# rcedgar/muscle

Measured on AMD Instinct MI355X. Metric: sequence-pairs/sec (fwd+bwd+posterior+relax), higher is better.
Workload: dtype f32

## Files before the change

### include/mpcgpu.h

```cpp
#ifndef MPCGPU_H
#define MPCGPU_H

#include <stdint.h>

#ifdef __cplusplus
extern "C" {
#endif

typedef struct mpcgpu_ctx mpcgpu_ctx;

int mpcgpu_create(mpcgpu_ctx **out, int device_ordinal);
void mpcgpu_destroy(mpcgpu_ctx *ctx);
const char *mpcgpu_last_error(const mpcgpu_ctx *ctx);
const char *mpcgpu_version(void);

int mpcgpu_set_hmm(mpcgpu_ctx *ctx, const float start[5], const float trans[25],
                   const float match[256 * 256], const float ins[256],
                   float min_sparse_score, int expf_variant);

int mpcgpu_set_seqs(mpcgpu_ctx *ctx, uint32_t n, const uint8_t *const *seqs, const uint32_t *lens);

int mpcgpu_set_mega(mpcgpu_ctx *ctx, uint32_t nfeat, const uint32_t *alpha, const float *weight,
                    const float *const *logprobs, const float *const *logprob_mx,
                    const uint8_t *const *profiles);
// ... 10 lines not shown
int mpcgpu_plan_store_segments(uint32_t n, const uint32_t *sizes, uint64_t limit_blocks, uint32_t max_segs, uint32_t *z_first,
                               uint64_t *blocks, uint32_t *nsegs);

int mpcgpu_calc_posteriors(mpcgpu_ctx *ctx, uint64_t k0, uint64_t k1);

int mpcgpu_build_store(mpcgpu_ctx *ctx);

int mpcgpu_shard_info(mpcgpu_ctx *ctx, uint64_t *bytes, void **dev_ptr);
int mpcgpu_shard_entries(mpcgpu_ctx *ctx, uint64_t *entries);
int mpcgpu_shard_export(mpcgpu_ctx *ctx, void *dev_dst);
int mpcgpu_store_import(mpcgpu_ctx *ctx, uint32_t nshards, const uint64_t *k0, const uint64_t *k1,
                        const uint64_t *bytes, void *dev_all);
int mpcgpu_store_import_part(mpcgpu_ctx *ctx, uint32_t nshards, const uint64_t *k0, const uint64_t *k1, const uint64_t *bytes,
                             const uint64_t *offsets, void *dev_all, uint64_t own_k0, uint64_t own_k1);
int mpcgpu_store_complete(mpcgpu_ctx *ctx);
int mpcgpu_values_info(mpcgpu_ctx *ctx, void **dev_ptr, uint64_t *total_count);
int mpcgpu_values_slice(mpcgpu_ctx *ctx, uint64_t k0, uint64_t k1, uint64_t *first, uint64_t *count);
int mpcgpu_values_export(mpcgpu_ctx *ctx, uint64_t first, uint64_t count, void *dev_dst);
int mpcgpu_values_import(mpcgpu_ctx *ctx, uint64_t first, uint64_t count, const void *dev_src);

int mpcgpu_cons_iter(mpcgpu_ctx *ctx, uint64_t k0, uint64_t k1);
int mpcgpu_cons_commit(mpcgpu_ctx *ctx);
int mpcgpu_cons_commit_range(mpcgpu_ctx *ctx, uint64_t first, uint64_t count);

int mpcgpu_get_ea(mpcgpu_ctx *ctx, uint64_t k0, uint64_t k1, float *ea);
int mpcgpu_get_nnz(mpcgpu_ctx *ctx, uint64_t k0, uint64_t k1, uint32_t *nnz);
int mpcgpu_get_sparse(mpcgpu_ctx *ctx, uint64_t k, uint32_t *offsets, void *values);
int mpcgpu_get_sparse_range(mpcgpu_ctx *ctx, uint64_t k0, uint64_t k1, uint32_t *offsets, void *values);

int mpcgpu_post_scores(mpcgpu_ctx *ctx, uint32_t LX, uint32_t LY, uint32_t ncand, const uint32_t *rows,
                       const uint32_t *cols, const float *scores, int kernel, uint32_t batch, float *ea, uint32_t *nnz,
                       uint32_t *offsets, void *values);

int mpcgpu_calc_aln(mpcgpu_ctx *ctx, const float *post, uint32_t LX, uint32_t LY,
                    char *path, uint32_t *pathlen, float *score);

int mpcgpu_align_alns(mpcgpu_ctx *ctx, uint32_t n1, const uint32_t *seq1, uint32_t n2, const uint32_t *seq2,
                      uint32_t C1, uint32_t C2, const uint32_t *pos2col1, const uint32_t *pos2col2,
                      char *path, uint32_t *pathlen, float *score);
int mpcgpu_align_alns_w(mpcgpu_ctx *ctx, uint32_t n1, const uint32_t *seq1, uint32_t n2, const uint32_t *seq2,
                        uint32_t C1, uint32_t C2, const uint32_t *pos2col1, const uint32_t *pos2col2,
                        const float *w1, const float *w2, char *path, uint32_t *pathlen, float *score);

int mpcgpu_align_alns_batch(mpcgpu_ctx *ctx, uint32_t njoins, const uint32_t *n1, const uint32_t *n2, const uint32_t *C1,
                            const uint32_t *C2, const uint32_t *seqs, const uint32_t *pos2col, uint32_t path_stride,
                            char *paths, uint32_t *pathlens, float *scores);

int mpcgpu_build_post(mpcgpu_ctx *ctx, uint32_t n1, const uint32_t *seq1, uint32_t n2, const uint32_t *seq2, uint32_t C1,
                      uint32_t C2, const uint32_t *pos2col1, const uint32_t *pos2col2, const float *w1, const float *w2,
                      float *post);
int mpcgpu_get_last_post(mpcgpu_ctx *ctx, uint32_t C1, uint32_t C2, float *post);

int mpcgpu_set_seqs_registry(mpcgpu_ctx *ctx, uint32_t n, const uint8_t *const *seqs, const uint32_t *lens);
int mpcgpu_align_msas(mpcgpu_ctx *ctx, uint32_t npairs, const uint32_t *seq1, const uint32_t *seq2, uint32_t C1,
                      uint32_t C2, const uint32_t *pos2col1, const uint32_t *pos2col2, char *path, uint32_t *pathlen,
                      float *score, float *ea_out);

int mpcgpu_align_pairs(mpcgpu_ctx *ctx, uint32_t npairs, const uint32_t *seq1, const uint32_t *seq2, uint32_t path_stride,
                       char *paths, uint32_t *pathlens, float *scores, float *ea);
int mpcgpu_get_list_sparse(mpcgpu_ctx *ctx, uint32_t q, uint32_t *nnz, uint32_t *offsets, void *values);

typedef struct mpcgpu_group mpcgpu_group;
int mpcgpu_group_create(mpcgpu_group **out, uint32_t ndev, const int *device_ordinals);
void mpcgpu_group_destroy(mpcgpu_group *g);
const char *mpcgpu_group_last_error(const mpcgpu_group *g);
uint32_t mpcgpu_group_size(const mpcgpu_group *g);
mpcgpu_ctx *mpcgpu_group_ctx(mpcgpu_group *g, uint32_t rank);
const char *mpcgpu_group_transport(const mpcgpu_group *g);
int mpcgpu_group_set_hmm(mpcgpu_group *g, const float start[5], const float trans[25], const float match[256 * 256],
                         const float ins[256], float min_sparse_score, int expf_variant);
int mpcgpu_group_set_seqs(mpcgpu_group *g, uint32_t n, const uint8_t *const *seqs, const uint32_t *lens);
int mpcgpu_group_set_mega(mpcgpu_group *g, uint32_t nfeat, const uint32_t *alpha, const float *weight,
                          const float *const *logprobs, const float *const *logprob_mx, const uint8_t *const *profiles);
int mpcgpu_group_calc_posteriors(mpcgpu_group *g);
int mpcgpu_group_cons_iter(mpcgpu_group *g);

#define MPCGPU_NKERNELS 9
int mpcgpu_timers_reset(mpcgpu_ctx *ctx);
int mpcgpu_timers_enable(mpcgpu_ctx *ctx, int on);
int mpcgpu_timers_get(mpcgpu_ctx *ctx, float ms[MPCGPU_NKERNELS], uint64_t launches[MPCGPU_NKERNELS]);
int mpcgpu_work_get(mpcgpu_ctx *ctx, uint64_t *dp_cells, uint64_t *relax_entry_z, uint64_t *store_entries);
int mpcgpu_stage_a_info(mpcgpu_ctx *ctx, uint64_t *pairs, uint64_t *chained_pairs, uint64_t *chains);
int mpcgpu_stage_a_coop_info(mpcgpu_ctx *ctx, uint64_t *pairs, uint32_t *waves_per_pair);
int mpcgpu_post_info(mpcgpu_ctx *ctx, uint64_t out[4]);
int mpcgpu_store_info(mpcgpu_ctx *ctx, uint64_t out[6]);
int mpcgpu_synchronize(mpcgpu_ctx *ctx);
int mpcgpu_relax_info(mpcgpu_ctx *ctx, char *buf, uint32_t buflen, int *is_fallback);

#ifdef __cplusplus
}
#endif
#endif
```

### muscle_amd/_lib.py

```python
import ctypes as C
import os

import numpy as np

HERE = os.path.dirname(os.path.abspath(__file__))
DEFAULT_LIB = os.path.join(HERE, "csrc", "libmpcgpu.so")
NKERNELS = 9
KERNEL_FAMILIES = ["fb", "post", "store_build", "relax", "commit", "buildpost_gen", "buildpost_sort", "buildpost_reduce", "calc_aln"]

SYMBOLS = [
    "mpcgpu_create", "mpcgpu_destroy", "mpcgpu_last_error", "mpcgpu_version", "mpcgpu_set_hmm",
    "mpcgpu_set_seqs", "mpcgpu_set_mega", "mpcgpu_pair_count", "mpcgpu_calc_posteriors", "mpcgpu_build_store",
    "mpcgpu_shard_info", "mpcgpu_shard_export", "mpcgpu_store_import", "mpcgpu_values_info", "mpcgpu_values_slice", "mpcgpu_values_export", "mpcgpu_values_import",
    "mpcgpu_cons_iter", "mpcgpu_cons_commit", "mpcgpu_cons_commit_range", "mpcgpu_get_ea", "mpcgpu_get_nnz", "mpcgpu_get_sparse",
    "mpcgpu_get_sparse_range", "mpcgpu_post_scores", "mpcgpu_calc_aln", "mpcgpu_align_alns", "mpcgpu_align_alns_w", "mpcgpu_build_post", "mpcgpu_get_last_post", "mpcgpu_align_msas", "mpcgpu_align_pairs", "mpcgpu_get_list_sparse", "mpcgpu_stage_a_info", "mpcgpu_stage_a_coop_info", "mpcgpu_post_info", "mpcgpu_set_seqs_registry", "mpcgpu_timers_reset", "mpcgpu_timers_enable", "mpcgpu_timers_get",
    "mpcgpu_work_get", "mpcgpu_synchronize", "mpcgpu_relax_info", "mpcgpu_shard_entries",
    "mpcgpu_set_pair_order", "mpcgpu_pair_position", "mpcgpu_plan_partition", "mpcgpu_plan_store_segments", "mpcgpu_store_import_part", "mpcgpu_store_complete", "mpcgpu_store_info", "mpcgpu_align_alns_batch", "mpcgpu_store_epoch",
    "mpcgpu_group_create", "mpcgpu_group_destroy", "mpcgpu_group_last_error", "mpcgpu_group_size", "mpcgpu_group_ctx",
    "mpcgpu_group_transport", "mpcgpu_group_set_hmm", "mpcgpu_group_set_seqs", "mpcgpu_group_set_mega",
    "mpcgpu_group_calc_posteriors", "mpcgpu_group_cons_iter",
]


class MpcGpuError(RuntimeError):
    pass


_libs = {}


def load(lib_path=None):
    path = lib_path or os.environ.get("MPCGPU_LIB") or DEFAULT_LIB
    if path in _libs:
        return _libs[path]
    if not os.path.exists(path):
        raise MpcGpuError("HIP library not built: %s (run `python -c 'import __graft_entry__ as g; g.build()'` "
                          "or `make -C muscle_amd/csrc`); there is no CPU fallback" % path)
    L = C.CDLL(path)
    vp, u64, u32, i32 = C.c_void_p, C.c_uint64, C.c_uint32, C.c_int
    L.mpcgpu_create.argtypes = [C.POINTER(vp), i32]
    L.mpcgpu_destroy.argtypes = [vp]
    L.mpcgpu_destroy.restype = None
    L.mpcgpu_last_error.argtypes = [vp]
    L.mpcgpu_last_error.restype = C.c_char_p
    L.mpcgpu_version.restype = C.c_char_p
    L.mpcgpu_set_hmm.argtypes = [vp, vp, vp, vp, vp, C.c_float, i32]
    L.mpcgpu_set_seqs.argtypes = [vp, u32, vp, vp]
    L.mpcgpu_set_mega.argtypes = [vp, u32, vp, vp, vp, vp, vp]
    L.mpcgpu_pair_count.argtypes = [vp]
    L.mpcgpu_pair_count.restype = u64
    L.mpcgpu_calc_posteriors.argtypes = [vp, u64, u64]
    L.mpcgpu_build_store.argtypes = [vp]
    L.mpcgpu_shard_info.argtypes = [vp, C.POINTER(u64), C.POINTER(vp)]
    L.mpcgpu_shard_entries.argtypes = [vp, C.POINTER(u64)]
    L.mpcgpu_shard_export.argtypes = [vp, vp]
    L.mpcgpu_values_export.argtypes = [vp, u64, u64, vp]
    L.mpcgpu_values_import.argtypes = [vp, u64, u64, vp]
    L.mpcgpu_store_import.argtypes = [vp, u32, vp, vp, vp, vp]
    L.mpcgpu_values_info.argtypes = [vp, C.POINTER(vp), C.POINTER(u64)]
    L.mpcgpu_set_pair_order.argtypes = [vp, u32, vp]
    L.mpcgpu_pair_position.argtypes = [vp, u32, u32, C.POINTER(u64)]
    L.mpcgpu_plan_partition.argtypes = [u32, vp, u32, u32, vp, C.POINTER(u32), vp]
    L.mpcgpu_plan_store_segments.argtypes = [u32, vp, u64, u32, vp, vp, C.POINTER(u32)]
    L.mpcgpu_store_import_part.argtypes = [vp, u32, vp, vp, vp, vp, vp, u64, u64]
    L.mpcgpu_store_complete.argtypes = [vp]
    L.mpcgpu_store_info.argtypes = [vp, vp]
    L.mpcgpu_store_epoch.argtypes = [vp, C.POINTER(u64)]
    L.mpcgpu_align_alns_batch.argtypes = [vp, u32, vp, vp, vp, vp, vp, vp, u32, vp, vp, vp]
    L.mpcgpu_values_slice.argtypes = [vp, u64, u64, C.POINTER(u64), C.POINTER(u64)]
    L.mpcgpu_cons_iter.argtypes = [vp, u64, u64]
    L.mpcgpu_cons_commit.argtypes = [vp]
    L.mpcgpu_cons_commit_range.argtypes = [vp, u64, u64]
    L.mpcgpu_get_ea.argtypes = [vp, u64, u64, vp]
    L.mpcgpu_get_nnz.argtypes = [vp, u64, u64, vp]
    L.mpcgpu_get_sparse.argtypes = [vp, u64, vp, vp]
    L.mpcgpu_get_sparse_range.argtypes = [vp, u64, u64, vp, vp]
    L.mpcgpu_post_scores.argtypes = [vp, u32, u32, u32, vp, vp, vp, i32, u32, C.POINTER(C.c_float), C.POINTER(u32), vp, vp]
    L.mpcgpu_calc_aln.argtypes = [vp, vp, u32, u32, vp, C.POINTER(u32), C.POINTER(C.c_float)]
    L.mpcgpu_align_alns.argtypes = [vp, u32, vp, u32, vp, u32, u32, vp, vp, vp, C.POINTER(u32), C.POINTER(C.c_float)]
    L.mpcgpu_align_alns_w.argtypes = [vp, u32, vp, u32, vp, u32, u32, vp, vp, vp, vp, vp, C.POINTER(u32), C.POINTER(C.c_float)]
    L.mpcgpu_build_post.argtypes = [vp, u32, vp, u32, vp, u32, u32, vp, vp, vp, vp, vp]
    L.mpcgpu_get_last_post.argtypes = [vp, u32, u32, vp]
    L.mpcgpu_align_pairs.argtypes = [vp, u32, vp, vp, u32, vp, vp, vp, vp]
    L.mpcgpu_get_list_sparse.argtypes = [vp, u32, C.POINTER(u32), vp, vp]
    L.mpcgpu_set_seqs_registry.argtypes = [vp, u32, vp, vp]
    L.mpcgpu_align_msas.argtypes = [vp, u32, vp, vp, u32, u32, vp, vp, vp, C.POINTER(u32), C.POINTER(C.c_float), vp]
    L.mpcgpu_timers_reset.argtypes = [vp]
    L.mpcgpu_timers_enable.argtypes = [vp, C.c_int]
    L.mpcgpu_timers_get.argtypes = [vp, vp, vp]
    L.mpcgpu_work_get.argtypes = [vp, C.POINTER(u64), C.POINTER(u64), C.POINTER(u64)]
    L.mpcgpu_stage_a_info.argtypes = [vp, C.POINTER(u64), C.POINTER(u64), C.POINTER(u64)]
    L.mpcgpu_stage_a_coop_info.argtypes = [vp, C.POINTER(u64), C.POINTER(u32)]
    L.mpcgpu_post_info.argtypes = [vp, C.POINTER(u64)]
    L.mpcgpu_synchronize.argtypes = [vp]
    L.mpcgpu_relax_info.argtypes = [vp, C.c_char_p, u32, C.POINTER(i32)]
    L.mpcgpu_group_create.argtypes = [C.POINTER(vp), u32, vp]
    L.mpcgpu_group_destroy.argtypes = [vp]
    L.mpcgpu_group_destroy.restype = None
    L.mpcgpu_group_last_error.argtypes = [vp]
    L.mpcgpu_group_last_error.restype = C.c_char_p
    L.mpcgpu_group_size.argtypes = [vp]
    L.mpcgpu_group_size.restype = u32
    L.mpcgpu_group_ctx.argtypes = [vp, u32]
    L.mpcgpu_group_ctx.restype = vp
    L.mpcgpu_group_transport.argtypes = [vp]
    L.mpcgpu_group_transport.restype = C.c_char_p
    L.mpcgpu_group_set_hmm.argtypes = [vp, vp, vp, vp, vp, C.c_float, i32]
    L.mpcgpu_group_set_seqs.argtypes = [vp, u32, vp, vp]
    L.mpcgpu_group_set_mega.argtypes = [vp, u32, vp, vp, vp, vp, vp]
    L.mpcgpu_group_calc_posteriors.argtypes = [vp]
    L.mpcgpu_group_cons_iter.argtypes = [vp]
    _libs[path] = L
    return L


def plan_partition(lens, world, lib_path=None, L=None):
    L = L or load(lib_path)
    lens = np.ascontiguousarray(lens, np.uint32)
    cap = world * (world // 2 + 3) + 4
    rects = np.zeros((cap, 4), np.uint32)
    nr = C.c_uint32()
    pos = np.zeros(world + 1, np.uint64)
    rc = L.mpcgpu_plan_partition(len(lens), lens.ctypes.data, world, cap, rects.ctypes.data, C.byref(nr), pos.ctypes.data)
    if rc != 0:
        raise MpcGpuError("mpcgpu_plan_partition failed (%d)" % rc)
    return rects[:nr.value].copy(), [int(x) for x in pos]


def plan_store_segments(n, sizes, limit_blocks=0, lib_path=None, L=None):
    L = L or load(lib_path)
    sizes = np.ascontiguousarray(sizes, np.uint32).ravel()
    if sizes.size != n * n:
        raise ValueError("plan_store_segments: %d sizes for n = %d" % (sizes.size, n))
    cap = 16
    while True:
        zf, bl, ns = np.zeros(cap + 1, np.uint32), np.zeros(cap, np.uint64), C.c_uint32()
        rc = L.mpcgpu_plan_store_segments(n, sizes.ctypes.data, limit_blocks, cap, zf.ctypes.data, bl.ctypes.data, C.byref(ns))
        if rc == 2:
            cap = ns.value
            continue
        if rc != 0:
            raise MpcGpuError("mpcgpu_plan_store_segments failed (%d)%s" % (rc, ": a Z slab is larger than the segment limit" if rc == 3 else ""))
        return [int(z) for z in zf[:ns.value + 1]], [int(b) for b in bl[:ns.value]]


class MpcGroup:

    def __init__(self, devices, lib_path=None):
        self.L = load(lib_path)
        self.lib_path = lib_path
        devs = np.asarray(devices, np.int32)
        h = C.c_void_p()
        if self.L.mpcgpu_group_create(C.byref(h), len(devs), devs.ctypes.data) != 0:
            raise MpcGpuError(self.L.mpcgpu_group_last_error(None).decode())
        self.h = h
        self.n = 0
        self.lens = None

    def close(self):
        if getattr(self, "h", None):
            self.L.mpcgpu_group_destroy(self.h)
            self.h = None

    __del__ = close

    def _ck(self, rc):
        if rc != 0:
            raise MpcGpuError(self.L.mpcgpu_group_last_error(self.h).decode())

    @property
    def size(self):
        return int(self.L.mpcgpu_group_size(self.h))

    def transport(self):
        return self.L.mpcgpu_group_transport(self.h).decode()
# ... 256 lines not shown
        m2 = np.concatenate([np.asarray(x, np.uint32) for x in p2c2]).astype(np.uint32)
        path = np.empty(C1 + C2, np.uint8)
        n, sc = C.c_uint32(), C.c_float()
        if w1 is not None:
            a1, a2 = np.ascontiguousarray(w1, np.float32), np.ascontiguousarray(w2, np.float32)
            self._ck(self.L.mpcgpu_align_alns_w(self.h, len(s1), s1.ctypes.data, len(s2), s2.ctypes.data, C1, C2, m1.ctypes.data,
                                                 m2.ctypes.data, a1.ctypes.data, a2.ctypes.data, path.ctypes.data, C.byref(n), C.byref(sc)))
            return path[:n.value].tobytes().decode(), float(np.float32(sc.value))
        self._ck(self.L.mpcgpu_align_alns(self.h, len(s1), s1.ctypes.data, len(s2), s2.ctypes.data, C1, C2,
                                           m1.ctypes.data, m2.ctypes.data, path.ctypes.data, C.byref(n), C.byref(sc)))
        return path[:n.value].tobytes().decode(), float(np.float32(sc.value))

    def align_alns_batch(self, joins):
        nj = len(joins)
        n1 = np.array([len(j[0]) for j in joins], np.uint32)
        n2 = np.array([len(j[1]) for j in joins], np.uint32)
        C1 = np.array([j[4] for j in joins], np.uint32)
        C2 = np.array([j[5] for j in joins], np.uint32)
        seqs = np.concatenate([np.concatenate([np.asarray(j[0], np.uint32), np.asarray(j[1], np.uint32)]) for j in joins]).astype(np.uint32)
        maps = np.concatenate([np.asarray(x, np.uint32) for j in joins for x in list(j[2]) + list(j[3])]).astype(np.uint32)
        stride = int((C1 + C2).max())
        paths = np.zeros(nj * stride, np.uint8)
        plen = np.zeros(nj, np.uint32)
        sc = np.zeros(nj, np.float32)
        self._ck(self.L.mpcgpu_align_alns_batch(self.h, nj, n1.ctypes.data, n2.ctypes.data, C1.ctypes.data, C2.ctypes.data, seqs.ctypes.data,
                                                 maps.ctypes.data, stride, paths.ctypes.data, plen.ctypes.data, sc.ctypes.data))
        return [(paths[q * stride:q * stride + int(plen[q])].tobytes().decode(), float(sc[q])) for q in range(nj)]

    def align_pairs(self, seq1, seq2, sparse=False):
        s1, s2 = np.ascontiguousarray(seq1, np.uint32), np.ascontiguousarray(seq2, np.uint32)
        n = len(s1)
        stride = int(max(int(self.lens[a]) + int(self.lens[b]) for a, b in zip(s1, s2))) if n else 1
        paths = np.zeros(max(n, 1) * stride, np.uint8)
        plen = np.zeros(max(n, 1), np.uint32)
        sc = np.zeros(max(n, 1), np.float32)
        ea = np.zeros(max(n, 1), np.float32)
        self._ck(self.L.mpcgpu_align_pairs(self.h, n, s1.ctypes.data, s2.ctypes.data, stride, paths.ctypes.data, plen.ctypes.data,
                                           sc.ctypes.data, ea.ctypes.data))
        out = [(paths[q * stride:q * stride + int(plen[q])].tobytes().decode(), np.float32(sc[q]), np.float32(ea[q])) for q in range(n)]
        if not sparse:
            return out
        sp = []
        for q in range(n):
            nz = C.c_uint32()
            self._ck(self.L.mpcgpu_get_list_sparse(self.h, q, C.byref(nz), None, None))
            off = np.empty(int(self.lens[s1[q]]) + 1, np.uint32)
            val = np.empty(max(nz.value, 1) * 2, np.uint32)
            self._ck(self.L.mpcgpu_get_list_sparse(self.h, q, C.byref(nz), off.ctypes.data, val.ctypes.data))
            sp.append((off, val[:2 * nz.value].copy()))
        return out, sp

    def build_post(self, seq1, seq2, p2c1, p2c2, C1, C2, w1=None, w2=None):
        s1, s2 = np.asarray(seq1, np.uint32), np.asarray(seq2, np.uint32)
        m1 = np.concatenate([np.asarray(x, np.uint32) for x in p2c1]).astype(np.uint32)
        m2 = np.concatenate([np.asarray(x, np.uint32) for x in p2c2]).astype(np.uint32)
        post = np.empty((C1, C2), np.float32)
        a1 = None if w1 is None else np.ascontiguousarray(w1, np.float32)
        a2 = None if w2 is None else np.ascontiguousarray(w2, np.float32)
        self._ck(self.L.mpcgpu_build_post(self.h, len(s1), s1.ctypes.data, len(s2), s2.ctypes.data, C1, C2, m1.ctypes.data, m2.ctypes.data,
                                          None if a1 is None else a1.ctypes.data, None if a2 is None else a2.ctypes.data, post.ctypes.data))
        return post

    def last_post(self, C1, C2):
        post = np.empty((C1, C2), np.float32)
        self._ck(self.L.mpcgpu_get_last_post(self.h, C1, C2, post.ctypes.data))
        return post

    def relax_info(self):
        buf = C.create_string_buffer(1024)
        fb = C.c_int(0)
        self._ck(self.L.mpcgpu_relax_info(self.h, buf, 1024, C.byref(fb)))
        return buf.value.decode(), bool(fb.value)

    def stage_a_info(self):
        a, b, c = C.c_uint64(0), C.c_uint64(0), C.c_uint64(0)
        self._ck(self.L.mpcgpu_stage_a_info(self.h, C.byref(a), C.byref(b), C.byref(c)))
        return a.value, b.value, c.value

    def stage_a_coop_info(self):
        a, w = C.c_uint64(0), C.c_uint32(0)
        self._ck(self.L.mpcgpu_stage_a_coop_info(self.h, C.byref(a), C.byref(w)))
        return a.value, w.value

    def post_info(self):
        out = (C.c_uint64 * 4)()
        self._ck(self.L.mpcgpu_post_info(self.h, out))
        return tuple(int(x) for x in out)

    def timers_reset(self):
        self._ck(self.L.mpcgpu_timers_reset(self.h))

    def timers_enable(self, on=True):
        self._ck(self.L.mpcgpu_timers_enable(self.h, 1 if on else 0))

    def timers_get(self):
        ms = np.zeros(NKERNELS, np.float32)
        ln = np.zeros(NKERNELS, np.uint64)
        self._ck(self.L.mpcgpu_timers_get(self.h, ms.ctypes.data, ln.ctypes.data))
        return {k: (float(ms[i]), int(ln[i])) for i, k in enumerate(KERNEL_FAMILIES)}

    def work_get(self):
        a, b, c = C.c_uint64(), C.c_uint64(), C.c_uint64()
        self._ck(self.L.mpcgpu_work_get(self.h, C.byref(a), C.byref(b), C.byref(c)))
        return {"dp_cells": a.value, "relax_entry_z": b.value, "store_entries": c.value}
```

### muscle_amd/csrc/kernels_fbc.h

```cpp
#pragma once
#include "kernels_fb.h"

#define MPC_CHAIN_MAX 16
#define MPC_CHAIN_TAB_WORDS 8
#define MPC_CHAIN_TAB_BYTES (MPC_CHAIN_MAX * MPC_CHAIN_TAB_WORDS * 4)

struct FbChainParams {
	FbParams f;
	const u32 *chain_first;
	const u32 *chain_cnt;
};

template <int H>
__global__ void __launch_bounds__(256, (H == 8) ? 4 : 1) fb_chain_kernel(FbChainParams cp)
{
	const FbParams &p = cp.f;
	MPC_DYN_SMEM(smem_raw);
	__shared__ MpcCoef s_coef[MPC_COEF_ENTRIES];
	float *s_match = (float *)smem_raw;
	float *s_ins = s_match + p.A * p.A;
	u32 *s_tab_all = (u32 *)(s_ins + p.A);
	if (threadIdx.x < MPC_COEF_ENTRIES)
		mpc_coef_table_init(s_coef, (int)threadIdx.x);
	for (int q = threadIdx.x; q < p.A * p.A; q += blockDim.x)
		s_match[q] = p.match[q];
	for (int q = threadIdx.x; q < p.A; q += blockDim.x)
		s_ins[q] = p.ins[q];
	__syncthreads();

	const int t = threadIdx.x & 63;
	const u32 waves_per_block = blockDim.x >> 6;
	const u32 wave = threadIdx.x >> 6;
	const u32 slot = blockIdx.x * waves_per_block + wave;
	float *fm = p.fm_scratch + (u64)slot * p.fm_stride;
	u32 *s_tab = s_tab_all + wave * (MPC_CHAIN_MAX * MPC_CHAIN_TAB_WORDS);
	const float LZ = MPC_LOG_ZERO;
	const float tSM = p.tSM, tSI = p.tSI, tSJ = p.tSJ, tMM = p.tMM, tMI = p.tMI, tMJ = p.tMJ;
	const float tII = p.tII, tIM = p.tIM, tJJ = p.tJJ, tJM = p.tJM;
	const int A = p.A;
	const int NONE_HI = 0x7fffffff, NONE_LO = -0x40000000;
	auto tabw = [&](int k, int w) -> u32 { return mpc_wave_first(s_tab[k * MPC_CHAIN_TAB_WORDS + w]); };

	for (;;) {
		const u32 qi = mpc_wave_first(atomicAdd(p.queue, t == 0 ? 1u : 0u));
		if (qi >= p.count)
			break;
		const u32 first = cp.chain_first[qi];
		const int C = (int)cp.chain_cnt[qi];
		const u32 pid0 = p.order[first];
		const u32 sx = p.pair_x[pid0];
		const int LX = (int)p.seq_len[sx];
		const u8 *X = p.seq_code + p.seq_off[sx];
		const int T = (LX + H - 1) / H;
		int Vtot;
		{
			const bool mine = t < C;
			const u32 pid = mine ? p.order[first + (u32)t] : 0u;
			const u32 sy = mine ? p.pair_y[pid] : 0u;
			const int ly = mine ? (int)p.seq_len[sy] : -1;
			int incl = ly + 1;
			for (int d = 1; d < MPC_CHAIN_MAX; d <<= 1) {
				const int o = __shfl_up(incl, d);
				if (t >= d) incl += o;
			}
			MPC_WAVE_LDS_ORDER();
			if (mine) {
				u32 *e = s_tab + t * MPC_CHAIN_TAB_WORDS;
				e[0] = (u32)ly; e[1] = (u32)(incl - (ly + 1)); e[2] = pid; e[3] = sy; e[4] = 0u;
			}
			MPC_WAVE_LDS_ORDER();
			Vtot = (int)mpc_wave_first((u32)__shfl(incl, C - 1));
		}
		auto LYof = [&](int k) { return (int)tabw(k, 0); };
		auto baseof = [&](int k) { return (int)tabw(k, 1); };
		auto Yof = [&](int k) { return p.seq_code + p.seq_off[tabw(k, 3)]; };

		float cM[H], cIX[H], cJX[H], cIY[H], cJY[H];
		float insx[H];
		int mrow[H];
#pragma unroll
		for (int r = 0; r < H; ++r) {
			const int i = t * H + r + 1;
			const int xc = (i <= LX) ? (int)X[i - 1] : 0;
			insx[r] = s_ins[xc];
			mrow[r] = xc * A;
			cM[r] = cIX[r] = cJX[r] = cIY[r] = cJY[r] = LZ;
		}
		float uM = LZ, uIX = LZ, uJX = LZ, uIY = LZ, uJY = LZ;
		float gIY = LZ, gJY = LZ;
		int yprev = 0;
		int k0 = 0, base0 = 0, LY0 = LYof(0), next0 = (C > 1) ? baseof(1) : NONE_HI;
		const u8 *Y0 = Yof(0);
		int kb = 1, vb = (C > 1) ? baseof(1) : NONE_HI;
		int ke = 0, ve = LYof(0);
		const int nsteps = Vtot + T - 1;
		for (int s = 0; s < nsteps; ++s) {
			const int V = s - t;
// ... 129 lines not shown
				const int i = t * H + r + 1;
				const float oM = cM[r], oIY = cIY[r], oJY = cJY[r];
				const float xM = dgM + s_match[mrow[r] + yc];
				const float xIX = dnIX + insx[r];
				const float xJX = dnJX + insx[r];
				const float xIY = oIY + insy;
				const float xJY = oJY + insy;
				float vM = mpc_la5t(tMM + xM, tMI + xIX, tMJ + xJX, tMI + xIY, tMJ + xJY, s_coef);
				float vIX = mpc_la2t(tII + xIX, tIM + xM, s_coef);
				float vJX = mpc_la2t(tJJ + xJX, tJM + xM, s_coef);
				float vIY = mpc_la2t(tII + xIY, tIM + xM, s_coef);
				float vJY = mpc_la2t(tJJ + xJY, tJM + xM, s_coef);
				if (i == LX && corner) {
					vM = tSM; vIX = tSI; vIY = tSI; vJX = tSJ; vJY = tSJ;
				}
				const float f = fmrow[r * 64];
				const float score = (f + vM) - total;
				sc[r] = score;
				anyhit = anyhit || ((i <= LX) && incol && score >= p.thr);
				dgM = oM;
				cM[r] = vM; cIX[r] = vIX; cJX[r] = vJX; cIY[r] = vIY; cJY[r] = vJY;
				dnIX = vIX; dnJX = vJX;
			}
			gM = nM;
			ynext_prev = yc;
			if (V == vbB) {
#pragma unroll
				for (int r = 0; r < H; ++r) cM[r] = cIX[r] = cJX[r] = cIY[r] = cJY[r] = LZ;
			}
			if (__ballot(anyhit)) {
				u64 *candA = p.cand + (u64)pidA * p.capc, *candB = p.cand + (u64)pidB * p.capc;
				const u64 below = (1ull << t) - 1ull;
				if (vbB >= Vlead && vbB <= Vlead + (T - 1)) {
#pragma unroll
					for (int r = 0; r < H; ++r) {
						const int i = t * H + r + 1;
						const bool hit = (i <= LX) && incol && (sc[r] >= p.thr);
						const u64 bal = __ballot(hit);
						if (bal) {
							const u64 balB = __ballot(hit && lo), balA = bal & ~balB;
							const u32 pos = lo ? ncB + (u32)__popcll(balB & below) : ncA + (u32)__popcll(balA & below);
							if (hit && pos < p.capc) {
								const u32 idx = ((u32)(i - 1) << MPC_KEY_ROW_SHIFT) | (u32)(j - 1);
								(lo ? candB : candA)[pos] = ((u64)idx << 32) | (u64)__float_as_uint(sc[r]);
							}
							ncA += (u32)__popcll(balA);
							ncB += (u32)__popcll(balB);
						}
					}
				} else {
					const bool allB = Vlead + (T - 1) < vbB;
					u64 *cand1 = allB ? candB : candA;
					u32 nc1 = allB ? ncB : ncA;
#pragma unroll
					for (int r = 0; r < H; ++r) {
						const int i = t * H + r + 1;
						const bool hit = (i <= LX) && incol && (sc[r] >= p.thr);
						const u64 bal = __ballot(hit);
						if (bal) {
							const u32 pos = nc1 + (u32)__popcll(bal & below);
							if (hit && pos < p.capc) {
								const u32 idx = ((u32)(i - 1) << MPC_KEY_ROW_SHIFT) | (u32)(j - 1);
								cand1[pos] = ((u64)idx << 32) | (u64)__float_as_uint(sc[r]);
							}
							nc1 += (u32)__popcll(bal);
						}
					}
					if (allB) ncB = nc1; else ncA = nc1;
				}
			}
			if (Vlead + (T - 1) == vbB) {
				if (t == 0)
					p.cand_cnt[pidA] = ncA;
				--ka;
				pidA = pidB; ncA = ncB; totA = totB; baseA = baseB;
				vbB = (ka >= 1) ? baseA : NONE_LO;
				ncB = 0;
				if (ka >= 1) { baseB = baseof(ka - 1); pidB = tabw(ka - 1, 2); totB = __uint_as_float(tabw(ka - 1, 4)); }
				else baseB = 0;
			}
		}
		if (t == 0)
			p.cand_cnt[pidA] = ncA;
	}
}
```

### muscle_amd/csrc/kernels_post.h

```cpp
#pragma once
#include "device_math.h"
#include "kernels_fb.h"

struct PostParams {
	const u32 *pair_x, *pair_y;
	const u32 *seq_len;
	const u64 *cand;
	u32 capc;
	const u32 *cand_cnt;
	int use_fma;
	u32 sort_cap;
	u32 srow_cap;
	u64 *sort_scratch;
	u64 sort_stride;
	float *srow_scratch;
	u64 srow_stride;
	u32 *res;
	u64 res_stride;
	u32 *nnz;
	float *ea;
	u32 *flags;
	u32 count;
	u32 long_min;
};
// ... 91 lines not shown
				float excl = mpc_lane_up1(incl);
				if (t == 0) excl = 0.0f;
				for (u32 q = 0; q < C; ++q) {
					const u32 j = c0 + q;
					if (j > LY) break;
					Sn[j] = fmaxf(Sn[j], excl);
				}
				__syncthreads();
				float *tmp = Sp; Sp = Sn; Sn = tmp;
			}
			e = e1;
		}
		S = Sp;
		const float score = S[LY];
		const u32 mn = LX < LY ? LX : LY;
		const float ea = score / (float)mn;
		__syncthreads();

		u32 *rowcnt = rec, *colcnt = rec + LX;
		u32 base = 0;
		u32 kept = 0;
		for (u32 q0 = 0; q0 < c; q0 += 64) {
			const u32 q = q0 + t;
			const bool k = q < c && __uint_as_float((u32)buf[q]) >= MPC_MIN_SPARSE_PROB;
			kept += (u32)__popcll(__ballot(k));
		}
		const u32 nnz = kept;
		u32 *ent = rec + LX + LY;
		u32 *rowv = ent + 2 * (u64)nnz;
		u32 *tperm = rowv + nnz;
		for (u32 q0 = 0; q0 < c; q0 += 64) {
			const u32 q = q0 + t;
			const u64 key = q < c ? buf[q] : 0ull;
			const bool k = q < c && __uint_as_float((u32)key) >= MPC_MIN_SPARSE_PROB;
			const u64 bal = __ballot(k);
			if (k) {
				const u32 rank = base + (u32)__popcll(bal & ((1ull << t) - 1ull));
				const u32 idx = (u32)(key >> 32);
				const u32 row = idx >> kshift, col = idx & ((1u << kshift) - 1u);
				ent[2 * (u64)rank] = (u32)key;
				ent[2 * (u64)rank + 1] = col;
				rowv[rank] = row;
				atomicAdd(&rowcnt[row], 1u);
				atomicAdd(&colcnt[col], 1u);
			}
			base += (u32)__popcll(bal);
		}
		__syncthreads();
		const u32 m2 = mpc_next_pow2(nnz < 2 ? 2 : nnz);
		for (u32 q = t; q < m2; q += 64) {
			u64 key = ~0ull;
			if (q < nnz)
				key = ((u64)(ent[2 * (u64)q + 1] * LX + rowv[q]) << 32) | (u64)q;
			buf[q] = key;
		}
		__syncthreads();
		mpc_bitonic_sort(buf, m2);
		for (u32 q = t; q < nnz; q += 64)
			tperm[(u32)buf[q]] = q;
		if (t == 0) { p.nnz[pid] = nnz; p.ea[pid] = ea; }
		__syncthreads();
	}
}

struct PostRowsParams {
	const u32 *pair_x, *pair_y;
	const u32 *seq_len;
	u64 *cand;
	u32 capc;
	const u32 *cand_cnt;
	int use_fma;
	u32 lx_cap, ly_cap;
	u32 sort_cap;
	u32 batch;
	u64 *sort_scratch;
	u64 sort_stride;
	u32 *res;
	u64 res_stride;
	u32 *nnz;
	float *ea;
	u32 *flags;
	u32 count;
	u32 long_min;
};


__global__ void __launch_bounds__(64) post_rows_kernel(PostRowsParams p)
{
	MPC_DYN_SMEM(smem_raw);
	u32 *s_rend = (u32 *)smem_raw;
	u32 *s_cend = s_rend + p.lx_cap;
	float *s_pm = (float *)(s_cend + p.ly_cap);
	u64 *s_sorted = (u64 *)(smem_raw + ((((size_t)p.lx_cap + 2 * (size_t)p.ly_cap) * 4 + 7) & ~(size_t)7));
	const int t = threadIdx.x;

	for (u32 pid = blockIdx.x; pid < p.count; pid += gridDim.x) {
		const u32 LX = p.seq_len[p.pair_x[pid]], LY = p.seq_len[p.pair_y[pid]];
		const u32 kshift = mpc_key_shift(LX, p.long_min);
		u32 *rec = p.res + (u64)pid * p.res_stride;
		const u32 c = p.cand_cnt[pid];
		if (c > p.capc) {
			if (t == 0) { p.flags[pid] = 1u; p.nnz[pid] = 0; p.ea[pid] = 0.0f; }
			continue;
		}
		if (t == 0) p.flags[pid] = 0u;
		u64 *cand = p.cand + (u64)pid * p.capc;
		u64 *sorted = (c <= p.sort_cap) ? s_sorted : (p.sort_scratch + (u64)blockIdx.x * p.sort_stride);
		for (u32 q = t; q <= LX; q += 64) s_rend[q] = 0;
		for (u32 q = t; q <= LY; q += 64) { s_cend[q] = 0; s_pm[q] = 0.0f; }
		for (u32 q = t; q < LX + LY; q += 64) rec[q] = 0;
		__syncthreads();
		for (u32 q = t; q < c; q += 64) {
			const u64 v = cand[q];
			const float pr = mpc_score_to_prob(__uint_as_float((u32)v), p.use_fma);
			cand[q] = (v & 0xffffffff00000000ull) | (u64)__float_as_uint(pr);
			atomicAdd(&s_rend[(u32)(v >> (32 + kshift))], 1u);
		}
		__syncthreads();
		{
			u32 carry = 0;
			for (u32 a0 = 0; a0 <= LX; a0 += 64) {
				const u32 a = a0 + t;
				const u32 v = (a <= LX) ? s_rend[a] : 0;
				u32 incl = v;
				for (int d = 1; d < 64; d <<= 1) {
					const u32 o = __shfl_up(incl, d);
					if (t >= d) incl += o;
				}
				if (a <= LX) s_rend[a] = carry + incl - v;
				carry += __shfl(incl, 63);
			}
		}
		__syncthreads();
		for (u32 q = t; q < c; q += 64) {
			const u64 v = cand[q];
			const u32 at = atomicAdd(&s_rend[(u32)(v >> (32 + kshift))], 1u);
			sorted[at] = ((v >> 32) & (u64)((1u << kshift) - 1u)) << 32 | (v & 0xffffffffull);
		}
		__syncthreads();
		for (u32 i = t; i < LX; i += 64) {
			const u32 b = i ? s_rend[i - 1] : 0u, e = s_rend[i];
			for (u32 x = b + 1; x < e; ++x) {
				const u64 key = sorted[x];
				u32 y = x;
				while (y > b && sorted[y - 1] > key) { sorted[y] = sorted[y - 1]; --y; }
				sorted[y] = key;
			}
		}
		__syncthreads();
		u32 cmax = 0;
		u64 nkey = c ? sorted[(u32)t < c ? (u32)t : c - 1u] : 0ull;
		for (u32 i0 = 0; i0 < LX; i0 += 64) {
			const u32 ri = i0 + (u32)t;
			const u32 rend_v = s_rend[ri < LX ? ri : LX - 1u];
			u32 b = mpc_wave_first(i0 ? s_rend[i0 - 1u] : 0u);
			const u32 nl = LX - i0 < 64u ? LX - i0 : 64u;
			for (u32 rl = 0; rl < nl; ++rl) {
				const u32 e = mpc_read_lane(rend_v, rl);
				if (e == b) continue;
				if (e - b > p.batch) {
					for (u32 x = b + (u32)t; x < e; x += 64) {
						const u64 key = sorted[x];
						const u32 cc = (u32)(key >> 32);
						s_cend[x - b] = __float_as_uint(s_pm[cc < cmax ? cc : cmax] + __uint_as_float((u32)key));
					}
					__syncthreads();
					float vprev = 0.0f;
					for (u32 c0 = b; c0 < e; c0 += p.batch) {
						const u32 me = c0 + (u32)t;
						const bool have = me < e && (u32)t < p.batch;
						const u64 key = have ? sorted[me] : 0ull;
						const u32 col = (u32)(key >> 32);
						const float val = have ? __uint_as_float(s_cend[me - b]) : 0.0f;
						const float suffix = s_pm[cmax];
						const float V = fmaxf(mpc_wave_scan_max_nonneg(val), vprev);
						const u32 k = (e - c0 < p.batch) ? (e - c0) : p.batch;
						const u32 last = mpc_read_lane(col, k - 1) + 1u;
						const u32 hi = last > cmax ? last : cmax;
						const u32 jb0 = mpc_wave_first(col) + 1u;
						for (u32 j0 = jb0 < cmax + 1u ? jb0 : cmax + 1u; j0 <= hi; j0 += 64) {
							const u32 j = j0 + (u32)t;
							float cur = 0.0f;
							for (u32 l = 0; l < k; ++l) {
								const u32 cj = mpc_read_lane(col, l) + 1u;
								const float vj = mpc_read_lane(V, l);
								cur = (j >= cj) ? vj : cur;
							}
							if (j <= hi) s_pm[j] = fmaxf(j <= cmax ? s_pm[j] : suffix, cur);
						}
						cmax = hi;
						vprev = mpc_read_lane(V, k - 1);
						__syncthreads();
					}
					for (u32 x = b + (u32)t; x < e; x += 64) s_cend[x - b] = 0;
					__syncthreads();
					nkey = sorted[e + (u32)t < c ? e + (u32)t : c - 1u];
					b = e;
					continue;
				}
				const u32 k = e - b;
				const bool have = (u32)t < k;
				const u64 key = nkey;
				nkey = sorted[e + (u32)t < c ? e + (u32)t : c - 1u];
				const u32 col = have ? (u32)(key >> 32) : 0u;
				const u32 jfirst = mpc_wave_first(col) + 1u;
				const float val = have ? s_pm[col < cmax ? col : cmax] + __uint_as_float((u32)key) : 0.0f;
				const float suffix = s_pm[cmax];
				const float V = mpc_wave_scan_max_nonneg(val);
				const u32 last = mpc_read_lane(col, k - 1) + 1u;
				const u32 hi = last > cmax ? last : cmax;
				for (u32 j0 = jfirst < cmax + 1u ? jfirst : cmax + 1u; j0 <= hi; j0 += 64) {
					const u32 j = j0 + (u32)t;
					const float old = s_pm[j <= cmax ? j : cmax];
					float cur = 0.0f;
					for (u32 l = 0; l < k; ++l) {
						const u32 cj = mpc_read_lane(col, l) + 1u;
						const float vj = mpc_read_lane(V, l);
						cur = (j >= cj) ? vj : cur;
					}
					if (j <= hi) s_pm[j] = fmaxf(j <= cmax ? old : suffix, cur);
				}
				cmax = hi;
				b = e;
				MPC_WAVE_LDS_ORDER();
			}
		}
		const float score = s_pm[LY < cmax ? LY : cmax];
		const u32 mn = LX < LY ? LX : LY;
		const float ea = score / (float)mn;
		__syncthreads();
		u32 kept = 0;
		for (u32 q0 = 0; q0 < c; q0 += 64) {
			const u32 q = q0 + t;
			const bool k = q < c && __uint_as_float((u32)sorted[q]) >= MPC_MIN_SPARSE_PROB;
			kept += (u32)__popcll(__ballot(k));
		}
		const u32 nnz = kept;
		u32 *rowcnt = rec, *colcnt = rec + LX;
		u32 *ent = rec + LX + LY;
		u32 *rowv = ent + 2 * (u64)nnz;
		u32 *tperm = rowv + nnz;
		u32 base = 0;
		for (u32 i0 = 0; i0 < LX; i0 += 64) {
			const u32 i = i0 + (u32)t;
			u32 mycnt = 0;
			u32 b = 0, e = 0;
			if (i < LX) {
				b = i ? s_rend[i - 1] : 0u; e = s_rend[i];
				for (u32 x = b; x < e; ++x) mycnt += (__uint_as_float((u32)sorted[x]) >= MPC_MIN_SPARSE_PROB) ? 1u : 0u;
			}
			u32 incl = mycnt;
			for (int d = 1; d < 64; d <<= 1) {
				const u32 o = __shfl_up(incl, d);
				if (t >= d) incl += o;
			}
			u32 at = base + incl - mycnt;
			if (i < LX) {
				rowcnt[i] = mycnt;
				for (u32 x = b; x < e; ++x) {
					const u64 key = sorted[x];
					if (__uint_as_float((u32)key) >= MPC_MIN_SPARSE_PROB) {
						const u32 col = (u32)(key >> 32);
						ent[2 * (u64)at] = (u32)key;
						ent[2 * (u64)at + 1] = col;
						rowv[at] = i;
						atomicAdd(&s_cend[col], 1u);
						++at;
					}
				}
			}
			base += __shfl(incl, 63);
		}
		__syncthreads();
		for (u32 q = t; q < LY; q += 64) colcnt[q] = s_cend[q];
		{
			u32 carry = 0;
			for (u32 a0 = 0; a0 <= LY; a0 += 64) {
				const u32 a = a0 + t;
				const u32 v = (a <= LY) ? s_cend[a] : 0;
				u32 incl = v;
				for (int d = 1; d < 64; d <<= 1) {
					const u32 o = __shfl_up(incl, d);
					if (t >= d) incl += o;
				}
				if (a <= LY) s_cend[a] = carry + incl - v;
				carry += __shfl(incl, 63);
			}
		}
		__syncthreads();
		u32 *csorted = (u32 *)sorted;
		__syncthreads();
		for (u32 q = t; q < nnz; q += 64) {
			const u32 at = atomicAdd(&s_cend[ent[2 * (u64)q + 1]], 1u);
			csorted[at] = q;
		}
		__syncthreads();
		for (u32 j = t; j < LY; j += 64) {
			const u32 b = j ? s_cend[j - 1] : 0u, e = s_cend[j];
			for (u32 x = b + 1; x < e; ++x) {
				const u32 key = csorted[x];
				u32 y = x;
				while (y > b && csorted[y - 1] > key) { csorted[y] = csorted[y - 1]; --y; }
				csorted[y] = key;
			}
		}
		__syncthreads();
		for (u32 q = t; q < nnz; q += 64) tperm[csorted[q]] = q;
		if (t == 0) { p.nnz[pid] = nnz; p.ea[pid] = ea; }
		__syncthreads();
	}
}
```

### muscle_amd/csrc/mpc_platform.h

```cpp
#pragma once
#ifdef MPC_EMU
#include "hip_emu.h"
#else
#include <hip/hip_runtime.h>
#include <cstring>
#include <dlfcn.h>
#include <rocprim/device/device_radix_sort.hpp>
#define MPC_VERSION_STRING "mpcgpu 0.2 (HIP gfx950)"
#define MPC_ALN_THREADS 1024
template <class EnsureTmp>
inline hipError_t mpc_sort_pairs(EnsureTmp ensure_tmp, const unsigned *keys_in, unsigned *keys_out, const float *vals_in,
	float *vals_out, size_t n, unsigned end_bit, hipStream_t stream)
{
	size_t tmp_bytes = 0;
	hipError_t e = rocprim::radix_sort_pairs(nullptr, tmp_bytes, keys_in, keys_out, vals_in, vals_out, n, 0u, end_bit, stream);
	if (e != hipSuccess) return e;
	void *tmp = ensure_tmp(tmp_bytes < 16 ? (size_t)16 : tmp_bytes);
	if (!tmp) return hipErrorOutOfMemory;
	return rocprim::radix_sort_pairs(tmp, tmp_bytes, keys_in, keys_out, vals_in, vals_out, n, 0u, end_bit, stream);
}
inline void *mpc_dl_open(const char *name) { return dlopen(name, RTLD_NOW | RTLD_GLOBAL); }
inline void *mpc_dl_sym(void *lib, const char *name) { return dlsym(lib, name); }
inline const char *mpc_dl_error() { const char *e = dlerror(); return e ? e : "unknown error"; }
inline void mpc_enable_peer(int dev, int peer)
{
	(void)hipSetDevice(dev);
	int can = 0;
	if (hipDeviceCanAccessPeer(&can, dev, peer) == hipSuccess && can && hipDeviceEnablePeerAccess(peer, 0) != hipSuccess) (void)hipGetLastError();
}
#define MPC_LAUNCH(kern, grid, block, smem, stream, ...) \
	hipLaunchKernelGGL(kern, dim3(grid), dim3(block), (smem), (stream), __VA_ARGS__)
#define MPC_DYN_SMEM(name) extern __shared__ __attribute__((aligned(16))) unsigned char name[]
__device__ __forceinline__ int mpc_lane_up1(int v) { return __builtin_amdgcn_update_dpp(v, v, 0x138, 0xf, 0xf, false); }
__device__ __forceinline__ int mpc_lane_down1(int v) { return __builtin_amdgcn_update_dpp(v, v, 0x130, 0xf, 0xf, false); }
__device__ __forceinline__ float mpc_lane_up1(float v) { return __builtin_bit_cast(float, mpc_lane_up1(__builtin_bit_cast(int, v))); }
__device__ __forceinline__ float mpc_lane_down1(float v) { return __builtin_bit_cast(float, mpc_lane_down1(__builtin_bit_cast(int, v))); }
__device__ __forceinline__ float mpc_lane_up1_fill(float v, float fill)
{
	return __builtin_bit_cast(float, __builtin_amdgcn_update_dpp(__builtin_bit_cast(int, fill), __builtin_bit_cast(int, v), 0x138, 0xf, 0xf, false));
}
__device__ __forceinline__ float mpc_wave_chain_add(float total, float v)
{
	float acc = total;
	asm volatile(
		"s_nop 1\n\t"
		".irp k,0,1,2,3,4,5,6,7,8,9,10,11,12,13,14,15\n\tv_add_f32_dpp %0, %1, %0 row_newbcast:\\k row_mask:0x1 bank_mask:0xf\n\t.endr\n\t"
		"s_nop 1\n\tv_mov_b32_dpp %0, %0 row_bcast:15 row_mask:0x2 bank_mask:0xf\n\t"
		".irp k,0,1,2,3,4,5,6,7,8,9,10,11,12,13,14,15\n\tv_add_f32_dpp %0, %1, %0 row_newbcast:\\k row_mask:0x2 bank_mask:0xf\n\t.endr\n\t"
		"s_nop 1\n\tv_mov_b32_dpp %0, %0 row_bcast:15 row_mask:0x4 bank_mask:0xf\n\t"
		".irp k,0,1,2,3,4,5,6,7,8,9,10,11,12,13,14,15\n\tv_add_f32_dpp %0, %1, %0 row_newbcast:\\k row_mask:0x4 bank_mask:0xf\n\t.endr\n\t"
		"s_nop 1\n\tv_mov_b32_dpp %0, %0 row_bcast:15 row_mask:0x8 bank_mask:0xf\n\t"
		".irp k,0,1,2,3,4,5,6,7,8,9,10,11,12,13,14,15\n\tv_add_f32_dpp %0, %1, %0 row_newbcast:\\k row_mask:0x8 bank_mask:0xf\n\t.endr"
		: "+v"(acc) : "v"(v));
	return __builtin_bit_cast(float, __builtin_amdgcn_readlane(__builtin_bit_cast(int, acc), 63));
}
__device__ __forceinline__ float mpc_wave_chain_add_shift(float total, float v)
{
	const float w = (threadIdx.x & 63u) == 0u ? total + v : v;
	float p = 0.0f;
	asm volatile(".rept 64\n\ts_nop 1\n\tv_add_f32_dpp %0, %0, %1 wave_shr:1 row_mask:0xf bank_mask:0xf bound_ctrl:0\n\t.endr" : "+v"(p) : "v"(w));
	return __builtin_bit_cast(float, __builtin_amdgcn_readlane(__builtin_bit_cast(int, p), 63));
}
__device__ __forceinline__ float mpc_wave_scan_max_nonneg(float v)
{
#define MPC_DPP_MAX(ctrl, rmask)                                                                              \
	v = fmaxf(v, __builtin_bit_cast(float, __builtin_amdgcn_update_dpp(0, __builtin_bit_cast(int, v), ctrl, rmask, 0xf, false)))
	MPC_DPP_MAX(0x111, 0xf);
	MPC_DPP_MAX(0x112, 0xf);
	MPC_DPP_MAX(0x114, 0xf);
	MPC_DPP_MAX(0x118, 0xf);
	MPC_DPP_MAX(0x142, 0xa);
	MPC_DPP_MAX(0x143, 0xc);
#undef MPC_DPP_MAX
	return v;
}
__device__ __forceinline__ unsigned mpc_row16_scan_add(unsigned v)
{
	v += (unsigned)__builtin_amdgcn_update_dpp(0, (int)v, 0x111, 0xf, 0xf, true);
	v += (unsigned)__builtin_amdgcn_update_dpp(0, (int)v, 0x112, 0xf, 0xf, true);
	v += (unsigned)__builtin_amdgcn_update_dpp(0, (int)v, 0x114, 0xf, 0xf, true);
	v += (unsigned)__builtin_amdgcn_update_dpp(0, (int)v, 0x118, 0xf, 0xf, true);
	return v;
}
__device__ __forceinline__ unsigned mpc_row16_ror8(unsigned v) { return (unsigned)__builtin_amdgcn_update_dpp(0, (int)v, 0x128, 0xf, 0xf, false); }
__device__ __forceinline__ unsigned mpc_lds_load4(unsigned addr) { return *(const __attribute__((address_space(3))) unsigned *)(unsigned long long)addr; }
__device__ __forceinline__ unsigned mpc_read_lane(unsigned v, unsigned l) { return (unsigned)__builtin_amdgcn_readlane((int)v, (int)l); }
__device__ __forceinline__ float mpc_read_lane(float v, unsigned l) { return __builtin_bit_cast(float, __builtin_amdgcn_readlane(__builtin_bit_cast(int, v), (int)l)); }
__device__ __forceinline__ unsigned mpc_lane_gather(unsigned v, unsigned byte_index) { return (unsigned)__builtin_amdgcn_ds_bpermute((int)byte_index, (int)v); }
#define MPC_OPAQUE(v) asm volatile("" : "+v"(v))
#define MPC_OPAQUE_S(v) asm volatile("" : "+s"(v))
template <class T> __device__ __forceinline__ const __attribute__((address_space(4))) T *mpc_kernarg_again(const T &)
{
	unsigned long long k = (unsigned long long)__builtin_amdgcn_kernarg_segment_ptr();
	asm volatile("" : "+s"(k));
	return (const __attribute__((address_space(4))) T *)k;
}
#define MPC_KERNARG_AGAIN(p) mpc_kernarg_again(p)
#define MPC_WAVE_FENCE() __builtin_amdgcn_fence(__ATOMIC_SEQ_CST, "workgroup")
__device__ __forceinline__ unsigned mpc_cvt_u32_sat(float f) { unsigned r; asm("v_cvt_u32_f32 %0, %1" : "=v"(r) : "v"(f)); return r; }
__device__ __forceinline__ unsigned mpc_write_lane(unsigned v, unsigned sv, unsigned l) { return (threadIdx.x & 63u) == l ? sv : v; }
__device__ __forceinline__ void mpc_dma16(const void *gsrc, void *lds_wave_base)
{
	__builtin_amdgcn_global_load_lds((const __attribute__((address_space(1))) void *)gsrc,
		(__attribute__((address_space(3))) void *)lds_wave_base, 16, 0, 0);
}
__device__ __forceinline__ void mpc_dma4(const void *gsrc, void *lds_wave_base)
{
	__builtin_amdgcn_global_load_lds((const __attribute__((address_space(1))) void *)gsrc,
		(__attribute__((address_space(3))) void *)lds_wave_base, 4, 0, 0);
}
__device__ __forceinline__ void mpc_dma_wait() { asm volatile("s_waitcnt vmcnt(0)" ::: "memory"); }
struct __attribute__((aligned(16))) MpcQuad { unsigned x, y, z, w; };
__device__ __forceinline__ unsigned mpc_lds_addr(const void *p) { return (unsigned)(unsigned long long)(const __attribute__((address_space(3))) void *)p; }
typedef unsigned mpc_uint4v __attribute__((ext_vector_type(4)));
__device__ __forceinline__ MpcQuad mpc_lds_load16(unsigned addr)
{
	const mpc_uint4v v = *(const __attribute__((address_space(3))) mpc_uint4v *)(unsigned long long)addr;
	MpcQuad q; q.x = v.x; q.y = v.y; q.z = v.z; q.w = v.w;
	return q;
}
typedef unsigned long long mpc_u64s;
struct MpcRvBlocksAsm {
	mpc_uint4v a0, b0, a1, b1;
	__device__ __forceinline__ void load(int set, unsigned ia, unsigned ib)
	{
		if (set == 0) asm volatile("ds_read_b128 %0, %2\n\tds_read_b128 %1, %3" : "={v[24:27]}"(a0), "={v[28:31]}"(b0) : "v"(ia), "v"(ib) : "memory");
		else asm volatile("ds_read_b128 %0, %2\n\tds_read_b128 %1, %3" : "={v[32:35]}"(a1), "={v[36:39]}"(b1) : "v"(ia), "v"(ib) : "memory");
	}
	__device__ __forceinline__ void drain() { asm volatile("s_waitcnt lgkmcnt(0)" : "+{v[24:27]}"(a0), "+{v[28:31]}"(b0), "+{v[32:35]}"(a1), "+{v[36:39]}"(b1) : : "memory"); }
#define MPC_RV_MERGE_ASM(A0_, A1_, A2_, A3_, B0_, B1_, B2_, B3_, CURA_, CURB_, NXTA_, NXTB_)                           \
	"s_waitcnt lgkmcnt(0)\n\t"                \
	"ds_read_b128 " NXTA_ ", %[nia]\n\t"                                                                                 \
	"ds_read_b128 " NXTB_ ", %[nib]\n\t"                                                                                 \
	"s_mov_b64 %[sv], exec\n"                                                                                            \
	".Lrv_step_%=:\n\t"                                                                                                  \
	"v_cmp_eq_u32_sdwa %[e01], " A2_ ", " B3_ " src0_sel:WORD_0 src1_sel:DWORD\n\t"                                      \
	"v_cmp_eq_u32_sdwa %[e00], " A2_ ", " B2_ " src0_sel:WORD_0 src1_sel:WORD_0\n\t"                                     \
	"v_cmp_eq_u32_e64 %[e11], " A3_ ", " B3_ "\n\t"                                                                      \
	"v_cmp_eq_u32_sdwa %[e10], " A3_ ", " B2_ " src0_sel:DWORD src1_sel:WORD_0\n\t"                                      \
	"v_cmp_le_u32_e64 %[ada], " A3_ ", " B3_ "\n\t"                                                                      \
	"v_cmp_le_u32_e64 %[adb], " B3_ ", " A3_ "\n\t"                                                                      \
	"v_cmp_lt_u32_e64 %[nla], %[kf], " A2_ "\n\t"                                                                        \
	"v_cmp_lt_u32_e64 %[nlb], %[kf], " B2_ "\n\t"                                                                        \
	"v_cndmask_b32_e64 %[t0], 0, " B1_ ", %[e01]\n\t"                                                                    \
	"v_cndmask_b32_e64 %[t1], 0, " B1_ ", %[e11]\n\t"                                                                    \
	"v_cndmask_b32_e64 %[t0], %[t0], " B0_ ", %[e00]\n\t"                  \
	"v_cndmask_b32_e64 %[t1], %[t1], " B0_ ", %[e10]\n\t"                                                                \
	"v_mul_f32_e32 %[t0], " A0_ ", %[t0]\n\t"                                                                            \
	"v_mul_f32_e32 %[t1], " A1_ ", %[t1]\n\t"                                                                            \
	"v_add_f32_e32 %[sum], %[sum], %[t0]\n\t"            \
	"v_add_f32_e32 %[sum], %[sum], %[t1]\n\t"                                                                            \
	"s_orn2_b64 %[nla], %[nla], %[ada]\n\t"                                                                              \
	"s_orn2_b64 %[nlb], %[nlb], %[adb]\n\t"                                                                              \
	"s_and_b64 %[nla], %[nla], %[nlb]\n\t"                                                                               \
	"s_and_b64 exec, exec, %[nla]\n\t"                                              \
	"s_cbranch_scc0 .Lrv_done_%=\n\t"                                                                                    \
	"s_mov_b64 %[nlb], exec\n\t"                                                                                         \
	"s_and_b64 exec, %[nlb], %[ada]\n\t"                                                                                 \
	"v_add_u32_sdwa %[ia], %[ia], " A2_ " dst_sel:DWORD dst_unused:UNUSED_PAD src0_sel:DWORD src1_sel:WORD_1\n\t"        \
	"ds_read_b128 " CURA_ ", %[ia]\n\t"  \
	"s_and_b64 exec, %[nlb], %[adb]\n\t"                                                                                 \
	"v_add_u32_sdwa %[ib], %[ib], " B2_ " dst_sel:DWORD dst_unused:UNUSED_PAD src0_sel:DWORD src1_sel:WORD_1\n\t"        \
	"ds_read_b128 " CURB_ ", %[ib]\n\t"                                                                                  \
	"s_mov_b64 exec, %[nlb]\n\t"                                                                                         \
	"s_waitcnt lgkmcnt(0)\n\t"                                                                                           \
	"s_branch .Lrv_step_%=\n"                                                                                            \
	".Lrv_done_%=:\n\t"                                                                                                  \
	"s_mov_b64 exec, %[sv]"
	template <int SET> __device__ __forceinline__ void merge(float &sum, unsigned ia, unsigned ib, unsigned nia, unsigned nib)
	{
		mpc_u64s sv, e00, e01, e10, e11, ada, adb, nla, nlb;
		float t0, t1;
		const unsigned kf = 0xffffu;
		if (SET == 0)
			asm volatile(MPC_RV_MERGE_ASM("v24", "v25", "v26", "v27", "v28", "v29", "v30", "v31", "v[24:27]", "v[28:31]", "v[32:35]", "v[36:39]")
				: [sum] "+v"(sum), [ia] "+v"(ia), [ib] "+v"(ib), "+{v[24:27]}"(a0), "+{v[28:31]}"(b0), "=&{v[32:35]}"(a1), "=&{v[36:39]}"(b1),
				  [t0] "=&v"(t0), [t1] "=&v"(t1), [sv] "=&s"(sv), [e00] "=&s"(e00), [e01] "=&s"(e01), [e10] "=&s"(e10), [e11] "=&s"(e11),
				  [ada] "=&s"(ada), [adb] "=&s"(adb), [nla] "=&s"(nla), [nlb] "=&s"(nlb)
				: [nia] "v"(nia), [nib] "v"(nib), [kf] "s"(kf)
				: "vcc", "scc", "memory");
		else
// ... 199 lines not shown
```

### muscle_amd/csrc/mpcgpu.cpp

```cpp
#include "../../include/mpcgpu.h"
#include "kernels_fb.h"
#include "kernels_fbc.h"
#include "kernels_fbcoop.h"
#include "kernels_post.h"
#include "kernels_postw.h"
#include "kernels_store.h"
#include "kernels_relaxv.h"
#include "kernels_relaxb.h"
#include "kernels_aln.h"
#include "kernels_prog.h"

#include <algorithm>
#include <chrono>
#include <climits>
#include <cstdarg>
#include <cstdio>
#include <cstdlib>
#include <cstring>
#include <functional>
#include <map>
#include <mutex>
#include <string>
#include <vector>

// ... 104 lines not shown
	std::vector<std::pair<u64, u64> > lazy_ranges;
	std::vector<u8> need;
	DevBuf d_need;
	u64 own_k0 = 0, own_k1 = 0;

	bool have_shard = false;
	bool shard_is_list = false;
	u64 sh_k0 = 0, sh_k1 = 0;
	DevBuf d_shard;
	u64 shard_bytes = 0;
	std::vector<u32> sh_nnz;
	std::vector<float> sh_ea;

	bool have_store = false;
	const u32 *st_packed = nullptr;
	std::vector<u64> h_pbase, h_vbase;
	std::vector<u32> all_nnz;
	std::vector<float> all_ea;
	DevBuf d_pbase, d_vbase, d_rp, d_rp_base, d_ent, d_ent_base, d_mbase, d_vnext, d_own_packed;
	u64 total_entries = 0;
	u32 max_nnz = 0, max_len = 0;
	HostBuf h_bp_in, h_aln_res;
	size_t aln_smem_set[5] = {0, 0, 0, 0, 0};
	DevBuf d_tile_next, d_bp_in, d_aln_res, d_bp_seq, d_bp_map, d_bp_off, d_bp_coff, d_bp_keys, d_bp_vals, d_bp_tmp, d_bp_runs;
	DevBuf d_tiles, d_pad, d_pos, d_aln_post, d_aln_tb, d_aln_rev, d_aln_bnd;
	bool have_pad = false;
	u32 pad_lcap1 = 0;
	DevBuf d_rec_off, d_sizes, d_tilefit;
	u32 var_max_rec_blocks = 0;
	u64 var_total_blocks = 0;
	SegStore pad_seg, win_seg;
	std::string store_desc, tiles_desc, relax_kernel_name;
	bool relax_fallback = false;
	std::vector<u32> h_tiles;
	std::vector<u32> h_tiles2;
	DevBuf d_tiles2;
	bool var_mixed = false;
	u64 tiles_k0 = ~0ull, tiles_k1 = ~0ull;
	u32 tiles_bx = 0, tiles_by = 0;
	bool band_ok = false;
	bool var_pairs_ok = true;
	u32 band_nb1 = 0;
	DevBuf d_ovf_off, d_cell_off, d_yr, d_ovf_sum, d_ovf_maxc, d_btiles, d_bt_out, d_bt_count, d_bt_list;
	std::vector<u32> h_btiles;
	u64 btiles_k0 = ~0ull, btiles_k1 = ~0ull;
	bool win_ok = false;
	DevBuf d_win, d_wrec_off, d_wv_off, d_pos_w, d_wsum, d_wmaxc, d_wflag;
	u64 win_total_blocks = 0;
	const void *band_fn = nullptr;
	size_t band_smem = 0;
	int band_occ = 0;

	DevBuf d_bnd;
	DevBuf d_queue, d_order, d_bx, d_by, d_fm, d_cand, d_cand_cnt, d_total, d_res, d_nnz, d_ea, d_flags,
		d_sort_scratch, d_srow_scratch, d_dstbase, d_recwords, d_exp_off, d_exp_val, d_exp_offbase, d_exp_klist, d_exp_valbase;

	std::vector<TimedSpan> spans;
	bool timing = true;
	float ms[MPCGPU_NKERNELS] = {0};
	u64 launches[MPCGPU_NKERNELS] = {0};
	u64 work_cells = 0, work_entry_z = 0;
	u64 last_post_cells = 0;
	u64 sa_b0 = 0, sa_B = 0;
	u32 sa_capc = 0, sa_long_min = 0;
	bool sa_post_rows = false;
	u32 pi_kernel = 0, pi_threads = 0, pi_grid = 0;
	u64 pi_pairs = 0;
	DevBuf d_pw_rs, d_pw_info;
	std::vector<u32> list_x, list_y;
	std::vector<u32> ap_x, ap_y;
	u32 list_q0 = 0;
	bool ap_keep = false;
	HostBuf h_ap;
	std::vector<u32> v_flags;
	std::vector<u64> v_dstbase, v_recw;
	std::vector<u8> v_shdr;
	std::vector<u8> v_hdr;
	std::vector<u32> v_off, v_woff;
	std::vector<u32> v_words, v_out, v_w2, v_o2, v_okw;
	HostBuf h_bt;
	DevBuf d_ap_off;
	DevBuf d_chain_first, d_chain_cnt;
	DevBuf d_bx_n, d_by_n, d_order_n, d_chain_first_n, d_chain_cnt_n;
	hipStream_t stream2 = nullptr;
	hipEvent_t ev_post = nullptr;
	u64 sa_pairs = 0, sa_chained = 0, sa_chains = 0;
	u64 sa_coop_pairs = 0; u32 sa_coop_waves = 0;
	double aa_trace_t[5] = {0, 0, 0, 0, 0};
	u64 aa_trace_n = 0;
};

namespace {

int fail(mpcgpu_ctx *c, const char *fmt, ...)
{
	char buf[1024];
	va_list ap;
	va_start(ap, fmt);
	vsnprintf(buf, sizeof(buf), fmt, ap);
	va_end(ap);
	if (c) c->err = buf; else g_create_err = buf;
	return 1;
}

#define HIPCHK(c, call)                                                                          \
	do {                                                                                         \
		hipError_t e_ = (call);                                                                  \
		if (e_ != hipSuccess)                                                                    \
			return fail((c), "%s failed: %s (%s:%d)", #call, hipGetErrorString(e_), __FILE__, __LINE__); \
	} while (0)

int trace_level()
{
	static int lv = -1;
	if (lv < 0) { const char *s = getenv("MPCGPU_TRACE"); lv = (s && *s) ? atoi(s) : 0; if (lv < 0) lv = 0; }
	return lv;
}
bool trace_on() { return (trace_level() & 1) != 0; }
bool trace_host() { return (trace_level() & 4) != 0; }

int span_begin(mpcgpu_ctx *c, int fam, TimedSpan *sp)
{
	sp->fam = (c->timing || trace_on()) ? fam : -1;
	if (sp->fam < 0) return 0;
	if (trace_on()) { fprintf(stderr, "[mpcgpu] launch family %d ...\n", fam); fflush(stderr); }
	HIPCHK(c, hipEventCreate(&sp->a));
	HIPCHK(c, hipEventCreate(&sp->b));
	HIPCHK(c, hipEventRecord(sp->a, c->stream));
	return 0;
}
int span_end(mpcgpu_ctx *c, TimedSpan *sp)
{
	if (sp->fam < 0) return 0;
	HIPCHK(c, hipEventRecord(sp->b, c->stream));
	if (trace_on()) {
		HIPCHK(c, hipStreamSynchronize(c->stream));
		float t = 0;
		HIPCHK(c, hipEventElapsedTime(&t, sp->a, sp->b));
		fprintf(stderr, "[mpcgpu] family %d done: %.3f ms\n", sp->fam, t);
		fflush(stderr);
	}
	c->spans.push_back(*sp);
	c->launches[sp->fam] += 1;
	if (c->spans.size() >= 64) {
		size_t keep = 0;
		for (size_t q = 0; q < c->spans.size(); ++q) {
			TimedSpan &t = c->spans[q];
			float ms = 0;
			if (hipEventQuery(t.b) == hipSuccess && hipEventElapsedTime(&ms, t.a, t.b) == hipSuccess) {
				c->ms[t.fam] += ms;
				(void)hipEventDestroy(t.a);
				(void)hipEventDestroy(t.b);
			} else c->spans[keep++] = t;
		}
		(void)hipGetLastError();
		c->spans.resize(keep);
	}
	return 0;
}
int spans_collect(mpcgpu_ctx *c)
{
	HIPCHK(c, hipStreamSynchronize(c->stream));
	for (auto &sp : c->spans) {
		float t = 0;
		HIPCHK(c, hipEventElapsedTime(&t, sp.a, sp.b));
		c->ms[sp.fam] += t;
// ... 82 lines not shown
template <int H, bool MEGA> int occ_fb_coop_t(u32 block, size_t smem)
{
	int nb = 0;
	ensure_dyn_smem((const void *)fb_coop_kernel<H, MEGA>, smem);
	if (hipOccupancyMaxActiveBlocksPerMultiprocessor(&nb, (const void *)fb_coop_kernel<H, MEGA>, (int)block, smem) != hipSuccess) { (void)hipGetLastError(); nb = 0; }
	return nb;
}

int occ_fb_coop(int H, bool mega, u32 block, size_t smem)
{
	if (H == 1) return mega ? occ_fb_coop_t<1, true>(block, smem) : occ_fb_coop_t<1, false>(block, smem);
	if (H == MPC_LONG_H_SMALL) return mega ? occ_fb_coop_t<MPC_LONG_H_SMALL, true>(block, smem) : occ_fb_coop_t<MPC_LONG_H_SMALL, false>(block, smem);
	return mega ? occ_fb_coop_t<MPC_LONG_H, true>(block, smem) : occ_fb_coop_t<MPC_LONG_H, false>(block, smem);
}

u32 fb_coop_wave_limit(int H, bool mega)
{
	if (H == 1) return (u32)(mega ? FbCoopBounds<1, true>::threads : FbCoopBounds<1, false>::threads) / 64;
	if (H == MPC_LONG_H_SMALL) return (u32)(mega ? FbCoopBounds<MPC_LONG_H_SMALL, true>::threads : FbCoopBounds<MPC_LONG_H_SMALL, false>::threads) / 64;
	return (u32)(mega ? FbCoopBounds<MPC_LONG_H, true>::threads : FbCoopBounds<MPC_LONG_H, false>::threads) / 64;
}

void launch_fb_coop(int H, bool mega, const FbParams &p, u32 grid, u32 block, size_t smem, hipStream_t st)
{
	if (H == 1) { if (mega) launch_fb_coop_t<1, true>(p, grid, block, smem, st); else launch_fb_coop_t<1, false>(p, grid, block, smem, st); }
	else if (H == MPC_LONG_H_SMALL) { if (mega) launch_fb_coop_t<MPC_LONG_H_SMALL, true>(p, grid, block, smem, st); else launch_fb_coop_t<MPC_LONG_H_SMALL, false>(p, grid, block, smem, st); }
	else if (mega) launch_fb_coop_t<MPC_LONG_H, true>(p, grid, block, smem, st);
	else launch_fb_coop_t<MPC_LONG_H, false>(p, grid, block, smem, st);
}

int occ_fb_h(int H, bool mega, u32 block, size_t smem)
{
	switch (H) {
#define MPC_CASE(h) case h: return mega ? occ_fb<h, true>(block, smem) : occ_fb<h, false>(block, smem);
	MPC_CASE(1) MPC_CASE(2) MPC_CASE(3) MPC_CASE(4) MPC_CASE(5) MPC_CASE(6) MPC_CASE(7) MPC_CASE(8)
	MPC_CASE(9) MPC_CASE(10) MPC_CASE(11) MPC_CASE(12) MPC_CASE(13) MPC_CASE(14) MPC_CASE(15) MPC_CASE(16)
#undef MPC_CASE
	default: return 1;
	}
}

void launch_fb_h(int H, bool mega, const FbParams &p, u32 grid, u32 block, size_t smem, hipStream_t st)
{
	switch (H) {
#define MPC_CASE(h) case h: if (mega) launch_fb<h, true>(p, grid, block, smem, st); else launch_fb<h, false>(p, grid, block, smem, st); break;
	MPC_CASE(1) MPC_CASE(2) MPC_CASE(3) MPC_CASE(4) MPC_CASE(5) MPC_CASE(6) MPC_CASE(7) MPC_CASE(8)
	MPC_CASE(9) MPC_CASE(10) MPC_CASE(11) MPC_CASE(12) MPC_CASE(13) MPC_CASE(14) MPC_CASE(15) MPC_CASE(16)
#undef MPC_CASE
	default: break;
	}
}

template <int H> void launch_fbc(const FbChainParams &p, u32 grid, u32 block, size_t smem, hipStream_t st)
{
	auto kern = fb_chain_kernel<H>;
	ensure_dyn_smem((const void *)kern, smem);
	MPC_LAUNCH(kern, grid, block, smem, st, p);
}

template <int H> int occ_fbc(u32 block, size_t smem)
{
	int nb = 0;
	ensure_dyn_smem((const void *)fb_chain_kernel<H>, smem);
	if (hipOccupancyMaxActiveBlocksPerMultiprocessor(&nb, (const void *)fb_chain_kernel<H>, (int)block, smem) != hipSuccess || nb < 1)
		nb = 1;
	return nb;
}

int occ_fbc_h(int H, u32 block, size_t smem)
{
	switch (H) {
#define MPC_CASE(h) case h: return occ_fbc<h>(block, smem);
	MPC_CASE(1) MPC_CASE(2) MPC_CASE(3) MPC_CASE(4) MPC_CASE(5) MPC_CASE(6) MPC_CASE(7) MPC_CASE(8)
	MPC_CASE(9) MPC_CASE(10) MPC_CASE(11) MPC_CASE(12) MPC_CASE(13) MPC_CASE(14) MPC_CASE(15) MPC_CASE(16)
#undef MPC_CASE
	default: return 1;
	}
}

void launch_fbc_h(int H, const FbChainParams &p, u32 grid, u32 block, size_t smem, hipStream_t st)
{
	switch (H) {
#define MPC_CASE(h) case h: launch_fbc<h>(p, grid, block, smem, st); break;
	MPC_CASE(1) MPC_CASE(2) MPC_CASE(3) MPC_CASE(4) MPC_CASE(5) MPC_CASE(6) MPC_CASE(7) MPC_CASE(8)
	MPC_CASE(9) MPC_CASE(10) MPC_CASE(11) MPC_CASE(12) MPC_CASE(13) MPC_CASE(14) MPC_CASE(15) MPC_CASE(16)
#undef MPC_CASE
	default: break;
	}
}

u64 shard_header_bytes(u64 np) { return ((16 + np * 8 + 7) / 8) * 8; }
u64 rec_words(u32 LX, u32 LY, u32 nnz) { return (u64)LX + LY + 4 * (u64)nnz; }

void fill_store_params(mpcgpu_ctx *c, StoreParams &s)
{
	s.n = c->n;
	s.seq_len = c->d_seq_len.as<u32>();
	s.npairs = c->npairs;
	s.pair_x = c->d_pair_x.as<u32>();
	s.pair_y = c->d_pair_y.as<u32>();
	s.packed = (u32 *)c->st_packed;
	s.pbase = c->d_pbase.as<u64>();
	s.vbase = c->d_vbase.as<u64>();
	s.rp = c->d_rp.as<u32>();
	s.rp_base = c->d_rp_base.as<u64>();
	s.ent = c->d_ent.as<MpcEnt>();
	s.ent_base = c->d_ent_base.as<u64>();
	s.mbase = c->d_mbase.as<u32>();
	s.vnext = c->d_vnext.as<float>();
	s.pad = c->d_pad.as<u32>();
	s.lcap1 = c->pad_lcap1;
	s.pos_f = c->d_pos.as<unsigned short>();
	s.pos_t = c->d_pos.as<unsigned short>() + c->total_entries;
	s.rec_off = c->d_rec_off.as<u32>();
	s.ovf_off = c->band_ok ? c->d_ovf_off.as<u32>() : nullptr;
	s.nb1 = c->band_nb1;
	s.win = c->win_ok ? c->d_win.as<u32>() : nullptr;
	s.wrec_off = c->d_wrec_off.as<u32>();
	s.wv_off = c->win_ok ? c->d_wv_off.as<u32>() : nullptr;
	s.pos_wf = c->d_pos_w.as<unsigned short>();
	s.pos_wt = c->d_pos_w.as<unsigned short>() + c->total_entries;
	s.nrect = (u32)(c->order_rects.size() / 4);
	s.rects = s.nrect ? c->d_rects.as<u32>() : nullptr;
	s.need = c->partial ? c->d_need.as<u8>() : nullptr;
	const bool pseg = !c->pad_seg.seg.empty(), wseg = c->win_ok && !c->win_seg.seg.empty();
	s.pad_zbase = pseg ? c->pad_seg.zbase.as<u64>() : nullptr;
	s.pad_zend = pseg ? c->pad_seg.zend.as<u32>() : nullptr;
	s.win_zbase = wseg ? c->win_seg.zbase.as<u64>() : nullptr;
	s.win_zend = wseg ? c->win_seg.zend.as<u32>() : nullptr;
	if (pseg) s.pad = nullptr;
	if (wseg) s.win = nullptr;
}

void release_windows(mpcgpu_ctx *c)
{
	c->win_ok = false;
	c->d_win.release(); c->win_seg.release();
	c->d_pos_w.release(); c->d_wv_off.release(); c->d_wsum.release(); c->d_wmaxc.release(); c->d_wrec_off.release();
}

u64 pair_pos(const mpcgpu_ctx *c, u32 X, u32 Y)
{
	const u32 n = c->n;
	auto tri = [](u32 m, u32 i, u32 j) { return (u64)i * m - ((u64)i * (i + 1)) / 2 + (j - i - 1); };
	if (c->order_rects.empty()) return tri(n, X, Y);
	for (size_t r = 0; r < c->order_rects.size() / 4; ++r) {
		const u32 *q = &c->order_rects[4 * r];
		if (X < q[0] || X >= q[1] || Y < q[2] || Y >= q[3]) continue;
		return q[2] >= q[1] ? c->order_base[r] + (u64)(X - q[0]) * (q[3] - q[2]) + (Y - q[2]) : c->order_base[r] + tri(q[1] - q[0], X - q[0], Y - q[0]);
	}
	return ~0ull;
}

#include "mpcgpu_relax.inc"
#include "mpcgpu_store.inc"
}

static int refresh_packed(mpcgpu_ctx *c)
{
	if (!c->packed_stale) return 0;
	StoreParams sp;
	fill_store_params(c, sp);
	for (const std::pair<u64, u64> &r : c->lazy_ranges) {
		const u64 ka = (u64)(std::upper_bound(c->h_vbase.begin(), c->h_vbase.end(), r.first) - c->h_vbase.begin()) - 1;
		const u64 kb = std::min<u64>((u64)(std::lower_bound(c->h_vbase.begin(), c->h_vbase.end(), r.second) - c->h_vbase.begin()), c->npairs);
		if (kb <= ka) continue;
// ... 37 lines not shown
			for (u32 Z = 0; Z < n; ++Z) {
				if (run > 0xffffffffull) return fail(c, "mpcgpu_store_import: slab of sequence %u exceeds 2^32 entries", A);
				mbase[(size_t)A * (n + 1) + Z] = (u32)run;
				if (Z != A) {
					const u64 k = A < Z ? pair_pos(c, A, Z) : pair_pos(c, Z, A);
					run += c->all_nnz[k];
				}
			}
			if (run > 0xffffffffull) return fail(c, "mpcgpu_store_import: slab of sequence %u exceeds 2^32 entries", A);
			mbase[(size_t)A * (n + 1) + n] = (u32)run;
			slab[A] = run;
		}
		for (u32 A = 0; A < n; ++A) {
			ent_base[A + 1] = ent_base[A] + slab[A];
			rp_base[A + 1] = rp_base[A] + (u64)n * (c->len[A] + 1);
		}
	}
	HIPCHK(c, c->d_rp.ensure(rp_base[n] * 4));
	HIPCHK(c, c->d_ent.ensure(std::max<u64>(ent_base[n], 1) * 8));
	if (upload(c, c->d_mbase, mbase) || upload(c, c->d_ent_base, ent_base) || upload(c, c->d_rp_base, rp_base)) return 1;
	StoreParams sp;
	fill_store_params(c, sp);
	if (span_begin(c, 2, &ts)) return 1;
	const u64 blocks = (u64)n * n;
	MPC_LAUNCH(slab_build_kernel, (u32)std::min<u64>(blocks, (u64)c->prop.multiProcessorCount * 32), 64, 0, c->stream, sp);
	HIPCHK(c, hipGetLastError());
	if (span_end(c, &ts)) return 1;
	HIPCHK(c, hipStreamSynchronize(c->stream));
	c->have_store = true;
	return 0;
}

extern "C" {

const char *mpcgpu_version(void) { return MPC_VERSION_STRING; }

const char *mpcgpu_last_error(const mpcgpu_ctx *ctx) { return ctx ? ctx->err.c_str() : g_create_err.c_str(); }

int mpcgpu_create(mpcgpu_ctx **out, int device_ordinal)
{
	if (!out) return fail(nullptr, "mpcgpu_create: out is NULL");
	*out = nullptr;
	int ndev = 0;
	hipError_t e = hipGetDeviceCount(&ndev);
	if (e != hipSuccess || ndev <= 0)
		return fail(nullptr, "mpcgpu_create: no HIP device available (%s); this library has no CPU path",
			e == hipSuccess ? "device count 0" : hipGetErrorString(e));
	if (device_ordinal < 0 || device_ordinal >= ndev)
		return fail(nullptr, "mpcgpu_create: device %d out of range (have %d)", device_ordinal, ndev);
	mpcgpu_ctx *c = new mpcgpu_ctx;
	c->device = device_ordinal;
	if (hipSetDevice(device_ordinal) != hipSuccess || hipGetDeviceProperties(&c->prop, device_ordinal) != hipSuccess ||
		hipStreamCreate(&c->stream) != hipSuccess) {
		delete c;
		return fail(nullptr, "mpcgpu_create: cannot initialise device %d", device_ordinal);
	}
	for (int i = 0; i < 256; ++i) c->code_of[i] = -1;
	*out = c;
	return 0;
}

void mpcgpu_destroy(mpcgpu_ctx *c)
{
	if (!c) return;
	(void)hipSetDevice(c->device);
	(void)hipStreamSynchronize(c->stream);
	for (auto &sp : c->spans) { (void)hipEventDestroy(sp.a); (void)hipEventDestroy(sp.b); }
	DevBuf *all[] = {&c->d_seq_code, &c->d_seq_off, &c->d_seq_len, &c->d_match, &c->d_ins, &c->d_pair_x, &c->d_pair_y,
		&c->d_mg_prof, &c->d_mg_ins, &c->d_mg_tab, &c->d_mg_in, &c->d_bnd,
		&c->d_shard, &c->d_pbase, &c->d_vbase, &c->d_rp, &c->d_rp_base, &c->d_ent, &c->d_ent_base, &c->d_mbase,
		&c->d_vnext, &c->d_own_packed, &c->d_queue, &c->d_order, &c->d_bx, &c->d_by, &c->d_fm, &c->d_cand,
		&c->d_cand_cnt, &c->d_total, &c->d_res, &c->d_nnz, &c->d_ea, &c->d_flags, &c->d_sort_scratch,
		&c->d_srow_scratch, &c->d_dstbase, &c->d_recwords, &c->d_exp_off, &c->d_exp_val, &c->d_exp_offbase, &c->d_tiles, &c->d_pad, &c->d_pos, &c->d_bp_seq, &c->d_bp_map, &c->d_bp_off, &c->d_bp_coff,
		&c->d_tile_next, &c->d_bp_in, &c->d_aln_res, &c->d_bp_keys, &c->d_bp_vals, &c->d_bp_tmp, &c->d_bp_runs, &c->d_aln_post, &c->d_aln_tb, &c->d_aln_rev,
		&c->d_rec_off, &c->d_sizes, &c->d_tilefit};
	for (DevBuf *b : all) b->release();
	c->h_bp_in.release();
	c->h_aln_res.release();
	c->h_ap.release();
	c->d_ap_off.release(); c->d_aln_bnd.release();
	c->d_pw_rs.release(); c->d_pw_info.release();
	c->d_chain_first.release(); c->d_chain_cnt.release();
	c->d_bx_n.release(); c->d_by_n.release(); c->d_order_n.release(); c->d_chain_first_n.release(); c->d_chain_cnt_n.release();
	c->d_rects.release(); c->d_need.release(); c->d_exp_klist.release(); c->d_exp_valbase.release();
	c->d_tiles2.release();
	c->pad_seg.release(); release_windows(c);
	if (c->ev_post) (void)hipEventDestroy(c->ev_post);
	if (c->stream2) (void)hipStreamDestroy(c->stream2);
	(void)hipStreamDestroy(c->stream);
	delete c;
}

int mpcgpu_store_epoch(mpcgpu_ctx *c, uint64_t *epoch)
{
	if (!c) return 1;
	if (!epoch) return fail(c, "mpcgpu_store_epoch: NULL argument");
	*epoch = c->epoch;
	return 0;
}

int mpcgpu_synchronize(mpcgpu_ctx *c)
{
	if (!c) return 1;
	HIPCHK(c, hipSetDevice(c->device));
	HIPCHK(c, hipStreamSynchronize(c->stream));
	return 0;
}

int mpcgpu_set_hmm(mpcgpu_ctx *c, const float start[5], const float trans[25], const float match[65536],
	const float ins[256], float min_sparse_score, int expf_variant)
{
	if (!c) return 1;
	if (!start || !trans || !match || !ins) return fail(c, "mpcgpu_set_hmm: NULL table");
	++c->epoch;
	memcpy(c->start, start, sizeof(c->start));
	memcpy(c->trans, trans, sizeof(c->trans));
	c->match256.assign(match, match + 65536);
	c->ins256.assign(ins, ins + 256);
	c->thr = min_sparse_score;
	if (expf_variant < 0) {
#if defined(__x86_64__) && !defined(__HIP_DEVICE_COMPILE__)
		__builtin_cpu_init();
		c->use_fma = (__builtin_cpu_supports("fma") && __builtin_cpu_supports("avx2")) ? 1 : 0;
#else
		c->use_fma = 0;
#endif
	} else
		c->use_fma = expf_variant ? 1 : 0;
	c->have_hmm = true;
	c->have_shard = c->have_store = false;
	return 0;
}

static int set_seqs_impl(mpcgpu_ctx *c, uint32_t n, const uint8_t *const *seqs, const uint32_t *lens, bool with_pairs)
{
	if (!c) return 1;
	if (!c->have_hmm) return fail(c, "mpcgpu_set_seqs: call mpcgpu_set_hmm first");
	if (n < 2) return fail(c, "mpcgpu_set_seqs: need at least 2 sequences (got %u)", n);
	if (with_pairs && (u64)n * n > 0xffffffffull) return fail(c, "mpcgpu_set_seqs: too many sequences (%u)", n);
	HIPCHK(c, hipSetDevice(c->device));
	++c->epoch;
	c->have_shard = c->have_store = false;
	c->have_mega = false;
	c->n = n;
	c->raw.assign(n, {});
	c->len.assign(lens, lens + n);
	for (int i = 0; i < 256; ++i) c->code_of[i] = -1;
	c->A = 0;
	u32 maxl = 0, max2 = 0;
	for (u32 i = 0; i < n; ++i) {
		if (lens[i] == 0) return fail(c, "mpcgpu_set_seqs: sequence %u is empty", i);
		if (lens[i] > MPC_KEY_COL_MASK) return fail(c, "mpcgpu_set_seqs: sequence %u is longer than %u", i, MPC_KEY_COL_MASK);
		c->raw[i].assign(seqs[i], seqs[i] + lens[i]);
		for (u32 at = 0; at < lens[i]; ++at) {
			const u8 b = c->raw[i][at];
			if (b >= 128) return fail(c, "mpcgpu_set_seqs: sequence %u holds non-ASCII byte %u at position %u", i, (unsigned)b, at);
			if (c->code_of[b] < 0) {
				c->code_of[b] = c->A++;
			}
		}
		if (lens[i] > maxl) { max2 = maxl; maxl = lens[i]; } else if (lens[i] > max2) max2 = lens[i];
	}
	if (with_pairs && double(maxl) * double(max2) * 5 + 100 > double(INT_MAX))
		return fail(c, "HMM overflow, sequence lengths %u, %u (max ~21k)", maxl, max2);
	std::vector<u8> code;
	std::vector<u64> off(n + 1, 0);
// ... 172 lines not shown
	HIPCHK(c, c->d_mg_tab.ensure(((u64)nmx + 1) * 4));
	MegaPrepParams mp;
	const u8 *base = c->d_mg_in.as<u8>();
	mp.nfeat = nfeat;
	mp.alpha = (const u32 *)(base + o_alpha); mp.weight = (const float *)(base + o_weight);
	mp.lp = (const float *)(base + o_lp); mp.lp_off = (const u32 *)(base + o_lpoff);
	mp.mx = (const float *)(base + o_mx); mp.mx_off = (const u32 *)(base + o_mxoff);
	mp.letters = base + o_let; mp.npos = npos;
	mp.prof = c->d_mg_prof.as<u64>(); mp.ins = c->d_mg_ins.as<float>(); mp.tab = c->d_mg_tab.as<float>();
	const u32 grid = (u32)std::min<u64>((std::max<u64>(npos, nmx + 1) + 255) / 256, 4096);
	MPC_LAUNCH(mega_prepare_kernel, grid, 256, 0, c->stream, mp);
	HIPCHK(c, hipGetLastError());
	HIPCHK(c, hipStreamSynchronize(c->stream));
	c->mg_nfeat = nfeat;
	c->mg_tab_floats = nmx + 1;
	for (u32 f = 0; f < MPC_MEGA_FMAX; ++f) {
		c->mg_base[f] = f < nfeat ? mx_off[f] : nmx;
		c->mg_alpha[f] = f < nfeat ? alpha[f] : 0;
	}
	c->have_mega = true;
	return 0;
}

uint64_t mpcgpu_pair_count(const mpcgpu_ctx *c) { return c ? c->npairs : 0; }

#include "mpcgpu_stage_a.inc"
#include "mpcgpu_exchange.inc"
#include "mpcgpu_joins.inc"
int mpcgpu_relax_info(mpcgpu_ctx *c, char *buf, uint32_t buflen, int *is_fallback)
{
	if (!c) return 1;
	if (!c->have_store) return fail(c, "mpcgpu_relax_info: no store");
	if (buf && buflen) {
		std::string d = c->store_desc;
		if (!c->tiles_desc.empty()) d += "; " + c->tiles_desc;
		if (!c->relax_kernel_name.empty()) d += "; kernel=" + c->relax_kernel_name;
		snprintf(buf, buflen, "%s", d.c_str());
	}
	if (is_fallback) *is_fallback = c->relax_fallback ? 1 : 0;
	return 0;
}

int mpcgpu_store_info(mpcgpu_ctx *c, uint64_t out[6])
{
	if (!c) return 1;
	if (!c->have_store) return fail(c, "mpcgpu_store_info: no store");
	u64 packed_words = 0;
	for (u64 k = 0; k < c->npairs; ++k) packed_words += rec_words(c->len[c->h_pair_x[k]], c->len[c->h_pair_y[k]], c->all_nnz[k]);
	out[0] = c->have_pad ? c->var_total_blocks * 16 : 0;
	out[1] = (c->have_pad && c->win_ok) ? c->win_total_blocks * 16 : 0;
	out[2] = packed_words * 4;
	out[3] = c->total_entries;
	out[4] = c->h_vbase[c->own_k1] - c->h_vbase[c->own_k0];
	u32 held = 0;
	for (u32 i = 0; i < c->n; ++i) held += (!c->partial || c->need[i]) ? 1u : 0u;
	out[5] = held;
	return 0;
}

int mpcgpu_plan_store_segments(uint32_t n, const uint32_t *sizes, uint64_t limit_blocks, uint32_t max_segs, uint32_t *z_first, uint64_t *blocks,
	uint32_t *nsegs)
{
	if (!sizes || !nsegs || n == 0) return 1;
	std::vector<u32> zf;
	std::vector<u64> bl;
	const u64 limit = (limit_blocks == 0 || limit_blocks > kStoreSegBlocksMax) ? kStoreSegBlocksMax : limit_blocks;
	if (!plan_store_segments(n, sizes, limit, zf, bl)) return 3;
	*nsegs = (uint32_t)bl.size();
	if (bl.size() > max_segs || !z_first || !blocks) return 2;
	for (size_t g = 0; g < bl.size(); ++g) { z_first[g] = zf[g]; blocks[g] = bl[g]; }
	z_first[bl.size()] = n;
	return 0;
}

int mpcgpu_stage_a_info(mpcgpu_ctx *c, uint64_t *pairs, uint64_t *chained_pairs, uint64_t *chains)
{
	if (!c) return 1;
	if (pairs) *pairs = c->sa_pairs;
	if (chained_pairs) *chained_pairs = c->sa_chained;
	if (chains) *chains = c->sa_chains;
	return 0;
}

int mpcgpu_stage_a_coop_info(mpcgpu_ctx *c, uint64_t *pairs, uint32_t *waves_per_pair)
{
	if (!c) return 1;
	if (pairs) *pairs = c->sa_coop_pairs;
	if (waves_per_pair) *waves_per_pair = c->sa_coop_pairs ? c->sa_coop_waves : 0;
	return 0;
}

int mpcgpu_post_info(mpcgpu_ctx *c, uint64_t out[4])
{
	if (!c) return 1;
	if (!out) return fail(c, "mpcgpu_post_info: NULL argument");
	out[0] = c->pi_kernel; out[1] = c->pi_threads; out[2] = c->pi_pairs; out[3] = 0;
	if (c->pi_kernel == 2 && c->pi_grid) {
		HIPCHK(c, hipSetDevice(c->device));
		std::vector<u64> best(c->pi_grid, 0);
		HIPCHK(c, hipStreamSynchronize(c->stream));
		HIPCHK(c, hipMemcpy(best.data(), c->d_pw_info.p, (size_t)c->pi_grid * 8, hipMemcpyDeviceToHost));
		out[3] = *std::max_element(best.begin(), best.end()) & 0xffu;
	}
	return 0;
}

int mpcgpu_timers_reset(mpcgpu_ctx *c)
{
	if (!c) return 1;
	if (spans_collect(c)) return 1;
	for (int i = 0; i < MPCGPU_NKERNELS; ++i) { c->ms[i] = 0; c->launches[i] = 0; }
	return 0;
}

int mpcgpu_timers_enable(mpcgpu_ctx *c, int on)
{
	if (!c) return 1;
	c->timing = on != 0;
	return 0;
}

int mpcgpu_timers_get(mpcgpu_ctx *c, float ms[MPCGPU_NKERNELS], uint64_t launches[MPCGPU_NKERNELS])
{
	if (!c) return 1;
	if (spans_collect(c)) return 1;
	for (int i = 0; i < MPCGPU_NKERNELS; ++i) { ms[i] = c->ms[i]; launches[i] = c->launches[i]; }
	return 0;
}

int mpcgpu_work_get(mpcgpu_ctx *c, uint64_t *dp_cells, uint64_t *relax_entry_z, uint64_t *store_entries)
{
	if (!c) return 1;
	if (dp_cells) *dp_cells = c->work_cells;
	if (relax_entry_z) *relax_entry_z = c->work_entry_z;
	if (store_entries) *store_entries = c->total_entries;
	return 0;
}

}
```

### muscle_amd/csrc/mpcgpu_stage_a.inc

```
static void fill_fb_params(mpcgpu_ctx *c, FbParams &fp, const u32 *pair_x, const u32 *pair_y, u32 capc, bool mega)
{
	fp.seq_code = c->d_seq_code.as<u8>(); fp.seq_off = c->d_seq_off.as<u64>(); fp.seq_len = c->d_seq_len.as<u32>();
	fp.tSM = c->start[0]; fp.tSI = c->start[1]; fp.tSJ = c->start[3];
	fp.tMM = c->trans[0 * 5 + 0]; fp.tMI = c->trans[0 * 5 + 1]; fp.tMJ = c->trans[0 * 5 + 3];
	fp.tII = c->trans[1 * 5 + 1]; fp.tIM = c->trans[1 * 5 + 0];
	fp.tJJ = c->trans[3 * 5 + 3]; fp.tJM = c->trans[3 * 5 + 0];
	fp.thr = c->thr; fp.A = c->A; fp.match = c->d_match.as<float>(); fp.ins = c->d_ins.as<float>();
	fp.pair_x = pair_x; fp.pair_y = pair_y;
	fp.cand = c->d_cand.as<u64>(); fp.capc = capc; fp.cand_cnt = c->d_cand_cnt.as<u32>();
	fp.total = c->d_total.as<float>();
	fp.mg_prof = mega ? c->d_mg_prof.as<u64>() : nullptr; fp.mg_ins = mega ? c->d_mg_ins.as<float>() : nullptr;
	fp.mg_tab = mega ? c->d_mg_tab.as<float>() : nullptr; fp.mg_tab_floats = mega ? c->mg_tab_floats : 0;
	for (u32 f = 0; f < MPC_MEGA_FMAX; ++f) { fp.mg_base[f] = mega ? c->mg_base[f] : 0; fp.mg_alpha[f] = mega ? c->mg_alpha[f] : 0; }
	fp.order = nullptr; fp.count = 0; fp.queue = nullptr; fp.fm_scratch = nullptr; fp.fm_stride = 0;
	fp.bnd = nullptr; fp.bnd_stride = 0; fp.bnd_ld = 0; fp.fm_block = 0;
}

static const int SA_WAVES = 4, SA_BLOCK = 64 * SA_WAVES;
struct StageAGeom {
	u32 LXmax = 0, LYmax = 0;
	u32 LXlong = 0, LYlong = 0;
	u32 long_min = 0;
	u32 capc = 0;
	bool mega = false; size_t fb_smem = 0; u64 work_cells = 0;
	u64 res_stride() const { return (u64)LXmax + LYmax + 4 * (u64)capc; }
};
static StageAGeom stage_a_geom(const mpcgpu_ctx *c, u64 np, const u32 *px, const u32 *py)
{
	StageAGeom g;
	g.long_min = (u32)std::min(std::max(env_int("MPCGPU_FB_LONG_MIN", 64 * 12 + 1), 2), 64 * MPC_HMAX + 1);
	for (u64 k = 0; k < np; ++k) {
		const u32 LX = c->len[px[k]], LY = c->len[py[k]];
		g.LXmax = std::max(g.LXmax, LX); g.LYmax = std::max(g.LYmax, LY);
		g.work_cells += (u64)(LX + 1) * (LY + 1);
		if (LX >= g.long_min) { g.LXlong = std::max(g.LXlong, LX); g.LYlong = std::max(g.LYlong, LY); }
	}
	g.capc = std::max((u32)std::max(env_int("MPCGPU_CAND_PER_ROW", 12), 1) * std::max(g.LXmax, g.LYmax), 1024u);
	g.mega = c->have_mega;
	g.fb_smem = (g.mega ? (size_t)c->mg_tab_floats : (size_t)c->A * c->A + c->A) * sizeof(float);
	return g;
}
static bool post_rows_fits(u32 LXmax, u32 LYmax, u32 sort_cap)
{
	return ((size_t)LXmax + 2 + 2 * ((size_t)LYmax + 2)) * 4 + 8 + 8 * (size_t)sort_cap <= 150 * 1024;
}

struct ScratchBudget { u64 batch, planes; };
static ScratchBudget scratch_budget()
{
	const char *s = getenv("MPCGPU_SCRATCH_GB");
	const bool set = s && *s;
	return {(u64)(set ? atoi(s) : 32) << 30, set ? (u64)std::max(atoi(s), 1) << 30 : ~0ull};
}

struct BatchPrep {
	bool valid = false;
	u64 B = 0;
	std::vector<u32> bx, by, order;
	u32 hcount[MPC_HMAX + 2];
	std::vector<u32> chain_first, chain_cnt;
	u32 ccount[MPC_HMAX + 1];
	u32 cvmax[MPC_HMAX + 1];
	u32 coop_pairs = 0, coop_waves = 0;
};

struct ChainPlan {
	bool on = false, grade = true;
	u32 max = 0; size_t smem = 0;
	u32 vcap[MPC_HMAX + 1] = {0};
};
static int chain_plan(mpcgpu_ctx *c, const StageAGeom &g, u64 planes_budget, ChainPlan &cp)
{
	cp.on = !g.mega && env_int("MPCGPU_FB_CHAIN", 1) != 0;
	cp.max = (u32)std::min(std::max(env_int("MPCGPU_FB_CHAIN_MAX", 16), 2), MPC_CHAIN_MAX);
	cp.grade = env_int("MPCGPU_FB_CHAIN_GRADE", 1) != 0;
	cp.smem = ((size_t)c->A * c->A + c->A) * sizeof(float) + (size_t)SA_WAVES * MPC_CHAIN_TAB_BYTES;
	if (!cp.on) return 0;
	size_t freeb = 0, totb = 0;
	HIPCHK(c, hipMemGetInfo(&freeb, &totb));
	const u64 fm_budget = std::min<u64>(std::min<u64>((u64)32 << 30, planes_budget), (u64)((freeb + c->d_fm.cap) * 0.25));
	for (u32 H = 1; H <= MPC_HMAX; ++H) {
		const u64 waves = (u64)c->prop.multiProcessorCount * (u32)occ_fbc_h((int)H, SA_BLOCK, cp.smem) * SA_WAVES;
		const u64 steps = fm_budget / (waves * H * 64 * 4);
		cp.vcap[H] = steps > 64 + 2 ? (u32)std::min<u64>(steps - 64, 1u << 24) : 0;
	}
	return 0;
}

struct Chain { u32 q0, cnt, H; u64 work; };
static void build_chains(const mpcgpu_ctx *c, const ChainPlan &cp, u32 long_min, BatchPrep &P, std::vector<Chain> &chains, std::vector<unsigned char> &chained)
{
	const u64 B = P.B;
	auto work_of = [c, &P](u32 q0, u32 cnt, u32 H, u32 T) {
		u64 V = 0;
		for (u32 k = 0; k < cnt; ++k) V += c->len[P.by[q0 + k]] + 1;
		return (V + T) * H;
	};
	u64 q = 0;
	while (q < B) {
		const u32 LX = c->len[P.bx[q]];
		const u32 H = (LX + 63) / 64;
		if (LX >= long_min || H < 1 || H > MPC_HMAX || c->len[P.by[q]] + 1 > cp.vcap[H]) { ++q; continue; }
		const u32 T = (LX + H - 1) / H;
		u64 e = q;
		u64 V = 0;
		while (e < B && P.bx[e] == P.bx[q] && e - q < cp.max) {
			const u32 LY = c->len[P.by[e]];
			if (LY + 1 < T || V + LY + 1 > cp.vcap[H]) break;
			V += LY + 1;
			++e;
		}
		if (e == q) e = q + 1;
		chains.push_back({(u32)q, (u32)(e - q), H, 0});
		for (u64 k = q; k < e; ++k) chained[k] = 1;
		q = e;
	}
	for (Chain &ch : chains) { const u32 LX = c->len[P.bx[ch.q0]]; ch.work = work_of(ch.q0, ch.cnt, ch.H, (LX + ch.H - 1) / ch.H); }
	auto by_bin_and_work = [](const Chain &a, const Chain &b) { return a.H != b.H ? a.H < b.H : a.work != b.work ? a.work > b.work : a.q0 < b.q0; };
	std::sort(chains.begin(), chains.end(), by_bin_and_work);
	std::vector<Chain> graded;
	graded.reserve(chains.size() * 2);
	size_t lo = 0;
	while (lo < chains.size()) {
		size_t hi = lo;
		while (hi < chains.size() && chains[hi].H == chains[lo].H) ++hi;
		const u32 H = chains[lo].H;
		const u64 waves = (u64)c->prop.multiProcessorCount * (u32)occ_fbc_h((int)H, SA_BLOCK, cp.smem) * SA_WAVES;
		const u64 gw = std::max<u64>(waves, 1);
		u64 seen = 0;
		for (size_t k = hi; k-- > lo;) {
			const Chain &ch = chains[k];
			const u32 piece = !cp.grade ? ch.cnt : seen < gw ? 1u : seen < 3 * gw ? 2u : seen < 7 * gw ? 4u : ch.cnt;
			seen += ch.cnt;
			const u32 LX = c->len[P.bx[ch.q0]];
			for (u32 o = 0; o < ch.cnt; o += piece) {
				const u32 n = std::min(piece, ch.cnt - o);
				graded.push_back({ch.q0 + o, n, H, work_of(ch.q0 + o, n, H, (LX + H - 1) / H)});
			}
		}
		lo = hi;
	}
	std::sort(graded.begin(), graded.end(), by_bin_and_work);
	chains.swap(graded);
	for (const Chain &ch : chains) {
		u64 V = 0;
		for (u32 k = 0; k < ch.cnt; ++k) V += c->len[P.by[ch.q0 + k]] + 1;
		P.cvmax[ch.H] = std::max<u32>(P.cvmax[ch.H], (u32)V);
	}
}

static int prepare_batch(mpcgpu_ctx *c, const StageAGeom &g, const ChainPlan &cp, u64 batch_budget, u64 np, const u32 *px, const u32 *py, u64 b0, BatchPrep &P)
{
	const u64 per_pair = (u64)g.capc * 8 + g.res_stride() * 4 + 64;
	size_t freeb = 0, totb = 0;
	HIPCHK(c, hipMemGetInfo(&freeb, &totb));
	const u64 owned = (u64)c->d_cand.cap + c->d_res.cap + c->d_fm.cap;
	const u64 budget = std::min<u64>(batch_budget, (u64)((freeb + owned) * 0.4));
	const u64 bmax = std::min<u64>(std::max<u64>(1, budget / per_pair), 1u << 22);
	const u64 left = np - b0, nbat = (left + bmax - 1) / bmax;
	const u64 B = (left + nbat - 1) / nbat;
	P.B = B;
	P.bx.resize(B); P.by.resize(B); P.order.resize(B);
	std::vector<u64> keys;
	keys.reserve(B);
	for (u32 h = 0; h < MPC_HMAX + 2; ++h) P.hcount[h] = 0;
	for (u32 h = 0; h <= MPC_HMAX; ++h) P.ccount[h] = P.cvmax[h] = 0;
	P.chain_first.clear(); P.chain_cnt.clear();
	for (u64 q = 0; q < B; ++q) { P.bx[q] = px[b0 + q]; P.by[q] = py[b0 + q]; }
	std::vector<Chain> chains;
	std::vector<unsigned char> chained(B, 0);
	if (cp.on) build_chains(c, cp, g.long_min, P, chains, chained);
	for (u64 q = 0; q < B; ++q) {
		if (chained[q]) continue;
		const u32 LX = c->len[P.bx[q]], LY = c->len[P.by[q]];
		const bool lng = LX >= g.long_min;
		const u32 H = lng ? MPC_HMAX + 1 : (LX + 63) / 64;
		P.hcount[H]++;
		const u64 wk = lng ? (u64)LX * LY : (u64)(LY + (LX + H - 1) / H) * H;
		keys.push_back(((u64)H << 59) | ((((u64)1 << 37) - 1 - wk) << 22) | q);
	}
	std::sort(keys.begin(), keys.end());
	u64 at = 0;
	for (; at < keys.size(); ++at) P.order[at] = (u32)(keys[at] & (((u64)1 << 22) - 1));
	for (const Chain &ch : chains) {
		P.ccount[ch.H]++;
		P.chain_first.push_back((u32)at);
		P.chain_cnt.push_back(ch.cnt);
		for (u32 k = 0; k < ch.cnt; ++k) P.order[at++] = ch.q0 + k;
	}
	P.valid = true;
	return 0;
}

static int ensure_pair_scratch(mpcgpu_ctx *c, const StageAGeom &g, u64 B)
{
	HIPCHK(c, c->d_cand.ensure(B * g.capc * 8));
	HIPCHK(c, c->d_cand_cnt.ensure(B * 4));
	HIPCHK(c, c->d_total.ensure(B * 4));
	HIPCHK(c, c->d_res.ensure(B * g.res_stride() * 4));
	HIPCHK(c, c->d_queue.ensure(4 * (2 * MPC_HMAX + 4)));
	HIPCHK(c, hipMemsetAsync(c->d_queue.p, 0, 4 * (2 * MPC_HMAX + 4), c->stream));
	return 0;
}

struct RowBlockPlan { u32 long_h = 0, nbmax = 0, ld = 0, occ = 0; u64 fm_block = 0, fm_stride = 0, fm_budget = 0; };
static int row_block_plan(mpcgpu_ctx *c, const StageAGeom &g, u32 cnt, u64 planes_budget, RowBlockPlan &rp)
{
	const u32 cus = (u32)c->prop.multiProcessorCount;
	const int long_h_env = env_int("MPCGPU_FB_LONG_H", 0);
	const u32 LXlong = g.LXlong, LYlong = g.LYlong;
	rp.ld = (LYlong + 2 + 63) & ~63u;
	auto planes = [LXlong, LYlong](u32 h, u32 *nb, u64 *blk) { *nb = (LXlong + 64 * h - 1) / (64 * h); *blk = (u64)(LYlong + 64) * h * 64; return *blk * *nb; };
	size_t freeb = 0, totb = 0;
	HIPCHK(c, hipMemGetInfo(&freeb, &totb));
	rp.fm_budget = std::min<u64>(planes_budget, (u64)((freeb + c->d_fm.cap) * 0.45));
	rp.long_h = long_h_env == 1 ? 1u : long_h_env == MPC_LONG_H_SMALL ? (u32)MPC_LONG_H_SMALL : (u32)MPC_LONG_H;
	if (long_h_env == 0) {
		const u64 stride_small = planes(MPC_LONG_H_SMALL, &rp.nbmax, &rp.fm_block);
		const u64 waves_small = std::min<u64>(cnt, rp.fm_budget / (stride_small * 4 + 16ull * rp.ld * 4));
		if (waves_small > (u64)cus * 4 * 2) rp.long_h = MPC_LONG_H_SMALL;
	}
	rp.fm_stride = planes(rp.long_h, &rp.nbmax, &rp.fm_block);
	rp.occ = (u32)occ_fb_long((int)rp.long_h, g.mega, SA_BLOCK, g.fb_smem);
	return 0;
}

static int launch_fb_row_blocks(mpcgpu_ctx *c, const StageAGeom &g, const RowBlockPlan &rp, FbParams fp, const u32 *order, u32 cnt)
{
	const u32 cus = (u32)c->prop.multiProcessorCount;
	const u32 ld = rp.ld, occ = rp.occ;
	const u64 max_waves = rp.fm_budget / (rp.fm_stride * 4 + 16ull * ld * 4);
	if (max_waves < 1)
		return fail(c, "mpcgpu_calc_posteriors: not enough device memory for the forward plane of a %u x %u pair", g.LXlong, g.LYlong);
	u32 grid = std::min<u32>((cnt + SA_WAVES - 1) / SA_WAVES, cus * occ);
	grid = (u32)std::max<u64>(std::min<u64>(grid, max_waves / SA_WAVES), 1);
	const u32 wpb = max_waves < (u64)SA_WAVES ? (u32)max_waves : (u32)SA_WAVES;
	HIPCHK(c, c->d_fm.ensure((u64)grid * wpb * rp.fm_stride * 4));
	HIPCHK(c, c->d_bnd.ensure((u64)grid * wpb * 16 * ld * 4));
	if (trace_on()) {
		fprintf(stderr, "[mpcgpu] fb row blocks: H=%u pairs=%u blocks<=%u grid=%u x %u waves occ=%u fm=%.1f MB\n", rp.long_h, cnt, rp.nbmax,
			grid, wpb, occ, (double)grid * wpb * rp.fm_stride * 4 / 1048576.0);
		fflush(stderr);
	}
	fp.order = order; fp.count = cnt;
	fp.queue = c->d_queue.as<u32>() + MPC_HMAX + 1;
	fp.fm_scratch = c->d_fm.as<float>(); fp.fm_stride = rp.fm_stride; fp.fm_block = rp.fm_block;
	fp.bnd = c->d_bnd.as<float>(); fp.bnd_stride = 16ull * ld; fp.bnd_ld = ld;
	TimedSpan sp;
	if (span_begin(c, 0, &sp)) return 1;
	launch_fb_long((int)rp.long_h, g.mega, fp, grid, 64 * wpb, g.fb_smem, c->stream);
	HIPCHK(c, hipGetLastError());
	return span_end(c, &sp);
}

static int launch_fb_row_blocks_coop(mpcgpu_ctx *c, const StageAGeom &g, const RowBlockPlan &rp, FbParams fp, const u32 *order, u32 cnt, u32 W)
{
	const u32 cus = (u32)c->prop.multiProcessorCount;
	const u32 ld = rp.ld;
	const size_t smem = g.fb_smem + MPC_FB_COOP_LDS_BYTES;
	const u64 bnd_stride = (u64)rp.nbmax * 8 * ld;
	const u64 max_wgs = rp.fm_budget / (rp.fm_stride * 4 + bnd_stride * 4);
	if (max_wgs < 1)
		return fail(c, "mpcgpu_calc_posteriors: not enough device memory for the forward plane of a %u x %u pair", g.LXlong, g.LYlong);
	const u32 occ = (u32)std::max(occ_fb_coop((int)rp.long_h, g.mega, 64 * W, smem), 1);
	const u32 grid = (u32)std::max<u64>(std::min<u64>(std::min<u32>(cnt, cus * occ), max_wgs), 1);
	HIPCHK(c, c->d_fm.ensure((u64)grid * rp.fm_stride * 4));
	HIPCHK(c, c->d_bnd.ensure((u64)grid * bnd_stride * 4));
	if (trace_on()) {
		fprintf(stderr, "[mpcgpu] fb row blocks: H=%u pairs=%u blocks<=%u grid=%u x %u waves occ=%u fm=%.1f MB\n", rp.long_h, cnt, rp.nbmax,
			grid, W, occ, (double)grid * rp.fm_stride * 4 / 1048576.0);
		fprintf(stderr, "[mpcgpu] fb coop: W=%u waves per pair (fb_coop_kernel), line buffers %.1f MB\n", W, (double)grid * bnd_stride * 4 / 1048576.0);
		fflush(stderr);
	}
	fp.order = order; fp.count = cnt;
	fp.queue = c->d_queue.as<u32>() + MPC_HMAX + 1;
	fp.fm_scratch = c->d_fm.as<float>(); fp.fm_stride = rp.fm_stride; fp.fm_block = rp.fm_block;
	fp.bnd = c->d_bnd.as<float>(); fp.bnd_stride = bnd_stride; fp.bnd_ld = ld;
	TimedSpan sp;
	if (span_begin(c, 0, &sp)) return 1;
	launch_fb_coop((int)rp.long_h, g.mega, fp, grid, 64 * W, smem, c->stream);
	HIPCHK(c, hipGetLastError());
	return span_end(c, &sp);
}

static const int kFbCoopDefault = 0;
static u32 fb_coop_waves(const mpcgpu_ctx *c, const StageAGeom &g, const RowBlockPlan &rp, u32 cnt)
{
	const int env = env_int("MPCGPU_FB_COOP", kFbCoopDefault);
	if (env <= 0) return 0;
	const u32 wmax = std::min<u32>(std::min<u32>(rp.occ * SA_WAVES, fb_coop_wave_limit((int)rp.long_h, g.mega)), 16u);
	u32 W;
	if (env >= 2) W = std::min<u32>((u32)env, wmax);
	else {
		const u64 resident = (u64)c->prop.multiProcessorCount * rp.occ * SA_WAVES;
		if (rp.nbmax < 2 || cnt >= resident) return 0;
		W = (u32)std::min<u64>(std::min<u32>(wmax, rp.nbmax), resident / cnt);
	}
	return W >= 2 ? W : 0;
}

static int launch_fb_row_block_pairs(mpcgpu_ctx *c, const StageAGeom &g, const FbParams &fp, const u32 *order, u32 cnt, u64 planes_budget, BatchPrep &P)
{
	RowBlockPlan rp;
	if (row_block_plan(c, g, cnt, planes_budget, rp)) return 1;
	const u32 W = fb_coop_waves(c, g, rp, cnt);
	P.coop_pairs = W ? cnt : 0; P.coop_waves = W;
	return W ? launch_fb_row_blocks_coop(c, g, rp, fp, order, cnt, W) : launch_fb_row_blocks(c, g, rp, fp, order, cnt);
}

static int launch_fb_bins(mpcgpu_ctx *c, const StageAGeom &g, FbParams fp, const u32 *order, const u32 *hcount, u64 batch)
{
	TimedSpan sp;
	u32 pos = 0;
	for (u32 H = 1; H <= MPC_HMAX; ++H) {
		if (!hcount[H]) continue;
		const u32 cnt = hcount[H];
		u32 grid = (cnt + SA_WAVES - 1) / SA_WAVES, occ = 0;
		if (batch) {
			occ = (u32)occ_fb_h((int)H, g.mega, SA_BLOCK, g.fb_smem);
			grid = std::max(std::min<u32>(grid, (u32)c->prop.multiProcessorCount * occ), 1u);
		}
		const u64 fm_stride = (u64)(g.LYmax + 64) * H * 64;
		HIPCHK(c, c->d_fm.ensure((u64)grid * SA_WAVES * fm_stride * 4));
		if (trace_on()) {
			if (batch) fprintf(stderr, "[mpcgpu] fb H=%u pairs=%u grid=%u block=%d occ=%u capc=%u batch=%llu fm=%.1f MB\n", H, cnt, grid,
				SA_BLOCK, occ, g.capc, batch, (double)grid * SA_WAVES * fm_stride * 4 / 1048576.0);
			else fprintf(stderr, "[mpcgpu] align_pairs short list: fb H=%u pairs=%u\n", H, cnt);
			fflush(stderr);
		}
		fp.order = order + pos; fp.count = cnt;
		fp.queue = c->d_queue.as<u32>() + H;
		fp.fm_scratch = c->d_fm.as<float>(); fp.fm_stride = fm_stride;
		if (span_begin(c, 0, &sp)) return 1;
		launch_fb_h((int)H, g.mega, fp, grid, SA_BLOCK, g.fb_smem, c->stream);
		HIPCHK(c, hipGetLastError());
		if (span_end(c, &sp)) return 1;
		pos += cnt;
	}
	return 0;
}

static int launch_fb_chains(mpcgpu_ctx *c, const StageAGeom &g, const ChainPlan &plan, const FbParams &fp, const BatchPrep &P, const u32 *order, const u32 *first, const u32 *cnts)
{
	const u32 cus = (u32)c->prop.multiProcessorCount;
	TimedSpan sp;
	u32 cpos = 0;
	for (u32 H = 1; H <= MPC_HMAX; ++H) {
		if (!P.ccount[H]) continue;
		const u32 cnt = P.ccount[H];
		const u32 occ = (u32)occ_fbc_h((int)H, SA_BLOCK, plan.smem);
		const u32 grid = std::max(std::min<u32>((cnt + SA_WAVES - 1) / SA_WAVES, cus * occ), 1u);
		const u64 fm_stride = (u64)(P.cvmax[H] + 64) * H * 64;
		HIPCHK(c, c->d_fm.ensure((u64)grid * SA_WAVES * fm_stride * 4));
		if (trace_on()) {
			fprintf(stderr, "[mpcgpu] fb chains H=%u chains=%u grid=%u occ=%u longest axis=%u fm=%.1f MB\n", H, cnt, grid, occ, P.cvmax[H],
				(double)grid * SA_WAVES * fm_stride * 4 / 1048576.0);
			u64 members = 0;
			for (u32 k = 0; k < cnt; ++k) members += P.chain_cnt[cpos + k];
			fprintf(stderr, "[mpcgpu] fb chain members H=%u pairs=%llu capc=%u batch=%llu\n", H, members, g.capc, P.B);
			fflush(stderr);
		}
		FbChainParams cp;
		cp.f = fp;
		cp.f.order = order; cp.f.count = cnt;
		cp.f.queue = c->d_queue.as<u32>() + (MPC_HMAX + 2) + H;
		cp.f.fm_scratch = c->d_fm.as<float>(); cp.f.fm_stride = fm_stride;
		cp.chain_first = first + cpos; cp.chain_cnt = cnts + cpos;
		if (span_begin(c, 0, &sp)) return 1;
		launch_fbc_h((int)H, cp, grid, SA_BLOCK, plan.smem, c->stream);
		HIPCHK(c, hipGetLastError());
		if (span_end(c, &sp)) return 1;
		cpos += cnt;
	}
	return 0;
}

static int launch_fb_batch(mpcgpu_ctx *c, const StageAGeom &g, const ChainPlan &plan, u64 planes_budget, BatchPrep &P, bool into_next)
{
	DevBuf &dbx = into_next ? c->d_bx_n : c->d_bx, &dby = into_next ? c->d_by_n : c->d_by, &dord = into_next ? c->d_order_n : c->d_order;
	DevBuf &dcf = into_next ? c->d_chain_first_n : c->d_chain_first, &dcc = into_next ? c->d_chain_cnt_n : c->d_chain_cnt;
	const u64 B = P.B;
	if (upload(c, dbx, P.bx) || upload(c, dby, P.by) || upload(c, dord, P.order)) return 1;
	if (!P.chain_first.empty() && (upload(c, dcf, P.chain_first) || upload(c, dcc, P.chain_cnt))) return 1;
	if (ensure_pair_scratch(c, g, B)) return 1;
	HIPCHK(c, c->d_nnz.ensure(B * 4));
	HIPCHK(c, c->d_ea.ensure(B * 4));
	HIPCHK(c, c->d_flags.ensure(B * 4));
	FbParams fp;
	fill_fb_params(c, fp, dbx.as<u32>(), dby.as<u32>(), g.capc, g.mega);
	P.coop_pairs = P.coop_waves = 0;
	if (P.hcount[MPC_HMAX + 1]) {
		u32 first = 0;
		for (u32 H = 1; H <= MPC_HMAX; ++H) first += P.hcount[H];
		if (launch_fb_row_block_pairs(c, g, fp, dord.as<u32>() + first, P.hcount[MPC_HMAX + 1], planes_budget, P)) return 1;
	}
	return launch_fb_bins(c, g, fp, dord.as<u32>(), P.hcount, B) || launch_fb_chains(c, g, plan, fp, P, dord.as<u32>(), dcf.as<u32>(), dcc.as<u32>());
}

struct PostIO { const u32 *pair_x, *pair_y, *seq_len; u64 *cand; const u32 *cand_cnt; u32 *res, *nnz; float *ea; u32 *flags; u32 count; };

static void post_info_set(mpcgpu_ctx *c, u32 kernel, u32 threads, u32 grid, u64 pairs) { c->pi_kernel = kernel; c->pi_threads = threads; c->pi_grid = grid; c->pi_pairs = pairs; }

static int launch_post_rows(mpcgpu_ctx *c, const StageAGeom &g, const PostIO &io, u32 sort_cap, u32 batch, u32 grid, DevBuf &scratch, bool timed)
{
	PostRowsParams pr;
	pr.pair_x = io.pair_x; pr.pair_y = io.pair_y; pr.seq_len = io.seq_len;
	pr.cand = io.cand; pr.capc = g.capc; pr.cand_cnt = io.cand_cnt;
	pr.use_fma = c->use_fma;
	pr.lx_cap = g.LXmax + 2; pr.ly_cap = g.LYmax + 2;
	pr.sort_cap = std::min<u32>(g.capc, sort_cap); pr.sort_stride = g.capc;
	pr.batch = std::min<u32>(std::max<u32>(batch, 1u), 64u);
	const size_t fixed_lds = ((((size_t)pr.lx_cap + 2 * (size_t)pr.ly_cap) * 4 + 7) & ~(size_t)7);
	if (fixed_lds + (size_t)pr.sort_cap * 8 > 150 * 1024) pr.sort_cap = (u32)((150 * 1024 - fixed_lds) / 8);
	const size_t smem = fixed_lds + (size_t)pr.sort_cap * 8;
	if (smem > 64 * 1024) HIPCHK(c, hipFuncSetAttribute((const void *)post_rows_kernel, hipFuncAttributeMaxDynamicSharedMemorySize, (int)smem));
	if (!grid) {
		int pocc = 0;
		if (hipOccupancyMaxActiveBlocksPerMultiprocessor(&pocc, (const void *)post_rows_kernel, 64, smem) != hipSuccess || pocc < 1) pocc = 1;
		pocc = std::max(1, std::min(pocc, (int)((152 * 1024) / smem)));
		grid = (u32)std::min<u64>(io.count, (u64)c->prop.multiProcessorCount * (u32)pocc);
		if (trace_on()) { fprintf(stderr, "[mpcgpu] post rows: list of %u candidates in LDS, lds=%zu B blocks/CU=%d grid=%u\n", pr.sort_cap, smem, pocc, grid); fflush(stderr); }
	}
	HIPCHK(c, scratch.ensure(g.capc > pr.sort_cap ? (u64)grid * pr.sort_stride * 8 : 8));
	pr.sort_scratch = scratch.as<u64>();
	pr.res = io.res; pr.res_stride = g.res_stride();
	pr.nnz = io.nnz; pr.ea = io.ea; pr.flags = io.flags;
	pr.count = io.count; pr.long_min = g.long_min;
	post_info_set(c, 0, 64, grid, io.count);
	TimedSpan sp;
	if (timed && span_begin(c, 1, &sp)) return 1;
	MPC_LAUNCH(post_rows_kernel, grid, 64, smem, c->stream, pr);
	HIPCHK(c, hipGetLastError());
	return timed ? span_end(c, &sp) : 0;
}

static size_t fill_post(const mpcgpu_ctx *c, const StageAGeom &g, const PostIO &io, u32 sort_cap, PostParams &pp)
{
	pp.pair_x = io.pair_x; pp.pair_y = io.pair_y; pp.seq_len = io.seq_len;
	pp.cand = io.cand; pp.capc = g.capc; pp.cand_cnt = io.cand_cnt;
	pp.use_fma = c->use_fma;
	pp.sort_stride = next_pow2(std::max<u32>(g.capc, 2));
	pp.sort_cap = std::min<u32>((u32)pp.sort_stride, next_pow2(sort_cap));
	pp.srow_cap = std::min<u32>(g.LYmax + 1, 2048u);
	pp.srow_stride = 2 * ((u64)g.LYmax + 1);
	pp.res = io.res; pp.res_stride = g.res_stride();
	pp.nnz = io.nnz; pp.ea = io.ea; pp.flags = io.flags;
	pp.count = io.count; pp.long_min = g.long_min;
	return (size_t)pp.sort_cap * 8 + (size_t)pp.srow_cap * 2 * 4;
}

static const int kPostWideDefault = 0;
static int post_wide_env() { return env_int("MPCGPU_POST_WIDE", -1); }

static int launch_post_wide(mpcgpu_ctx *c, const StageAGeom &g, const PostIO &io, u32 grid, bool timed)
{
	const u32 T = MPC_POSTW_THREADS;
	const int lds_env = env_int("MPCGPU_POSTW_LDS", -1);
	PostWideParams pw;
	pw.pair_x = io.pair_x; pw.pair_y = io.pair_y; pw.seq_len = io.seq_len;
	pw.cand = io.cand; pw.capc = g.capc; pw.cand_cnt = io.cand_cnt;
	pw.use_fma = c->use_fma;
	pw.lds_cap = std::min<u32>(g.capc, lds_env >= 0 ? std::min<u32>((u32)lds_env, 4096u) : 4096u);
	pw.srow_cap = std::min<u32>(g.LYmax + 1, lds_env >= 0 ? std::min<u32>((u32)lds_env, 4096u) : 4096u);
	const size_t smem = mpc_postw_smem(T, pw.lds_cap, pw.srow_cap);
	ensure_dyn_smem((const void *)post_wide_kernel, smem);
	if (!grid) {
		int pocc = 0;
		if (hipOccupancyMaxActiveBlocksPerMultiprocessor(&pocc, (const void *)post_wide_kernel, (int)T, smem) != hipSuccess || pocc < 1) pocc = 1;
		grid = (u32)std::min<u64>(io.count, (u64)c->prop.multiProcessorCount * (u32)pocc);
	}
	pw.key_stride = g.capc; pw.rs_stride = (u64)g.LXmax + 1; pw.srow_stride = 2 * ((u64)g.LYmax + 1);
	HIPCHK(c, c->d_sort_scratch.ensure(g.capc > pw.lds_cap ? (u64)grid * 2 * pw.key_stride * 8 : 8));
	HIPCHK(c, c->d_pw_rs.ensure((u64)grid * pw.rs_stride * 4));
	HIPCHK(c, c->d_srow_scratch.ensure(g.LYmax + 1 > pw.srow_cap ? (u64)grid * pw.srow_stride * 4 : 8));
	HIPCHK(c, c->d_pw_info.ensure((u64)grid * 8));
	pw.key_scratch = c->d_sort_scratch.as<u64>(); pw.rs_scratch = c->d_pw_rs.as<u32>(); pw.srow_scratch = c->d_srow_scratch.as<float>();
	pw.info = c->d_pw_info.as<u64>();
	pw.res = io.res; pw.res_stride = g.res_stride();
	pw.nnz = io.nnz; pw.ea = io.ea; pw.flags = io.flags;
	pw.count = io.count; pw.long_min = g.long_min;
	if (trace_on()) { fprintf(stderr, "[mpcgpu] post wide: %u threads per pair, lists of %u candidates and rows of %u floats in LDS, lds=%zu B grid=%u\n", T, pw.lds_cap, pw.srow_cap, smem, grid); fflush(stderr); }
	post_info_set(c, 2, T, grid, io.count);
	TimedSpan sp;
	if (timed && span_begin(c, 1, &sp)) return 1;
	MPC_LAUNCH(post_wide_kernel, grid, T, smem, c->stream, pw);
	HIPCHK(c, hipGetLastError());
	return timed ? span_end(c, &sp) : 0;
}

static int launch_post_batch(mpcgpu_ctx *c, const StageAGeom &g, bool post_rows, bool post_wide, u32 sort_cap, u64 B)
{
	const PostIO io = {c->d_bx.as<u32>(), c->d_by.as<u32>(), c->d_seq_len.as<u32>(), c->d_cand.as<u64>(), c->d_cand_cnt.as<u32>(), c->d_res.as<u32>(), c->d_nnz.as<u32>(), c->d_ea.as<float>(), c->d_flags.as<u32>(), (u32)B};
	if (post_rows) {
		if (launch_post_rows(c, g, io, sort_cap, (u32)std::max(env_int("MPCGPU_POST_BATCH", 64), 1), 0, c->d_sort_scratch, true)) return 1;
	} else if (post_wide) {
		if (launch_post_wide(c, g, io, 0, true)) return 1;
	} else {
		PostParams pp;
		const size_t psmem = fill_post(c, g, io, sort_cap, pp);
		ensure_dyn_smem((const void *)post_kernel, psmem);
		int pocc = 0;
		if (hipOccupancyMaxActiveBlocksPerMultiprocessor(&pocc, (const void *)post_kernel, 64, psmem) != hipSuccess || pocc < 1) pocc = 8;
		if (psmem) pocc = std::max(1, std::min(pocc, (int)((152 * 1024) / psmem)));
		const u32 pgrid = (u32)std::min<u64>(B, (u64)c->prop.multiProcessorCount * (u32)pocc);
		if (trace_on()) { fprintf(stderr, "[mpcgpu] post: sort_cap=%u lds=%zu B blocks/CU=%d grid=%u\n", pp.sort_cap, psmem, pocc, pgrid); fflush(stderr); }
		HIPCHK(c, c->d_sort_scratch.ensure(pp.sort_stride > pp.sort_cap ? (u64)pgrid * pp.sort_stride * 8 : 8));
		HIPCHK(c, c->d_srow_scratch.ensure(g.LYmax + 1 > pp.srow_cap ? (u64)pgrid * pp.srow_stride * 4 : 8));
		pp.sort_scratch = c->d_sort_scratch.as<u64>(); pp.srow_scratch = c->d_srow_scratch.as<float>();
		post_info_set(c, 1, 64, pgrid, B);
		TimedSpan sp;
		if (span_begin(c, 1, &sp)) return 1;
		MPC_LAUNCH(post_kernel, pgrid, 64, psmem, c->stream, pp);
		HIPCHK(c, hipGetLastError());
		if (span_end(c, &sp)) return 1;
	}
	HIPCHK(c, hipEventRecord(c->ev_post, c->stream));
	return 0;
}

static int read_batch_sizes(mpcgpu_ctx *c, u64 done, u64 B, bool *overflow)
{
	std::vector<u32> &flags = c->v_flags;
	flags.resize(B);
	HIPCHK(c, hipStreamWaitEvent(c->stream2, c->ev_post, 0));
	HIPCHK(c, hipMemcpyAsync(&c->sh_nnz[done], c->d_nnz.p, B * 4, hipMemcpyDeviceToHost, c->stream2));
	HIPCHK(c, hipMemcpyAsync(&c->sh_ea[done], c->d_ea.p, B * 4, hipMemcpyDeviceToHost, c->stream2));
	HIPCHK(c, hipMemcpyAsync(flags.data(), c->d_flags.p, B * 4, hipMemcpyDeviceToHost, c->stream2));
	HIPCHK(c, hipStreamSynchronize(c->stream2));
	*overflow = false;
	for (u64 q = 0; q < B; ++q) *overflow = *overflow || (flags[q] & 1u);
	return 0;
}

static int pack_batch(mpcgpu_ctx *c, const StageAGeom &g, const BatchPrep &P, u64 done, u64 np, u64 hdr, u64 *words)
{
	const u64 B = P.B;
	std::vector<u64> &dstbase = c->v_dstbase, &recw = c->v_recw;
	dstbase.resize(B); recw.resize(B);
	u64 w = *words;
	for (u64 q = 0; q < B; ++q) {
		recw[q] = rec_words(c->len[P.bx[q]], c->len[P.by[q]], c->sh_nnz[done + q]);
		dstbase[q] = hdr / 4 + w;
		w += recw[q];
	}
	const double per = double(w) / double(done + B);
	const u64 est = hdr + (u64)(per * 1.05 * double(np) + 1024) * 4;
	if (std::max<u64>(est, hdr + w * 4) > c->d_shard.cap) {
		const size_t cap0 = c->d_shard.cap;
		HIPCHK(c, c->d_shard.ensure(std::max<u64>(hdr + (u64)(per * 1.15 * double(np) + 1024) * 4, hdr + w * 4), true, c->stream));
		if (trace_on()) {
			fprintf(stderr, "[mpcgpu] stage A shard: buffer %s at pair %llu, %zu -> %zu B, %llu record words kept\n", cap0 ? "replaced" : "allocated", done, cap0, c->d_shard.cap, *words);
			fflush(stderr);
		}
	}
	if (upload(c, c->d_dstbase, dstbase) || upload(c, c->d_recwords, recw)) return 1;
	TimedSpan sp;
	if (span_begin(c, 1, &sp)) return 1;
	MPC_LAUNCH(pack_kernel, (u32)std::min<u64>(B, (u64)c->prop.multiProcessorCount * 8), 256, 0, c->stream, c->d_res.as<u32>(), g.res_stride(),
		c->d_dstbase.as<u64>(), c->d_recwords.as<u64>(), c->d_shard.as<u32>(), (u32)B);
	HIPCHK(c, hipGetLastError());
	if (span_end(c, &sp)) return 1;
	*words = w;
	return 0;
}

static int stage_a(mpcgpu_ctx *c, u64 np, const u32 *px, const u32 *py)
{
	HIPCHK(c, hipSetDevice(c->device));
	c->have_shard = c->have_store = false;
	c->shard_is_list = true;
	c->list_x.assign(px, px + np); c->list_y.assign(py, py + np);
	c->list_q0 = 0;
	if (!c->ap_keep) { c->ap_x.clear(); c->ap_y.clear(); }
	c->sh_k0 = 0; c->sh_k1 = np;
	c->sh_nnz.assign(np, 0);
	c->sh_ea.assign(np, 0.0f);
	StageAGeom g = stage_a_geom(c, np, px, py);
	c->work_cells = g.work_cells;
	c->sa_pairs = np; c->sa_chained = c->sa_chains = 0;
	c->sa_coop_pairs = 0; c->sa_coop_waves = 0;
	const u64 hdr = shard_header_bytes(np);
	if (np == 0) {
		HIPCHK(c, c->d_shard.ensure(hdr));
		u64 h2[2] = {0, 0};
		HIPCHK(c, hipMemcpyAsync(c->d_shard.p, h2, 16, hipMemcpyHostToDevice, c->stream));
		HIPCHK(c, hipStreamSynchronize(c->stream));
		c->shard_bytes = hdr;
		c->have_shard = true;
		return 0;
	}
	for (u64 k = 0; k < np; ++k)
		if (double(c->len[px[k]]) * double(c->len[py[k]]) * 5 + 100 > double(INT_MAX))
			return fail(c, "mpcgpu_calc_posteriors: HMM overflow, sequence lengths %u, %u (max ~21k)", c->len[px[k]], c->len[py[k]]);
	if (g.LXlong > MPC_KEY_COL_MASK_LONG || g.LYlong > MPC_KEY_COL_MASK_LONG)
		return fail(c, "mpcgpu_calc_posteriors: a pair of %u x %u positions is beyond this build's limit of %u per sequence "
			"once the row sequence is longer than %u", g.LXlong, g.LYlong, MPC_KEY_COL_MASK_LONG, g.long_min - 1);
	const ScratchBudget budget = scratch_budget();
	ChainPlan chain;
	if (chain_plan(c, g, budget.planes, chain)) return 1;
	const char *post_mode = getenv("MPCGPU_POST");
	const u32 sort_cap = (u32)std::max(env_int("MPCGPU_POST_SORT_CAP", 1024), 2);
	const bool post_sort = post_mode && !strcmp(post_mode, "sort");
	const int wide_env = post_wide_env();
	const bool fits = post_rows_fits(g.LXmax, g.LYmax, sort_cap);
	const bool post_rows = wide_env != 1 && !post_sort && fits;
	const bool post_wide = wide_env == 1 || (wide_env < 0 && kPostWideDefault && !post_sort && !fits);
	const bool host_trace = trace_host();
	auto now = []() { return std::chrono::duration<double>(std::chrono::steady_clock::now().time_since_epoch()).count(); };
	double lap_t[6] = {0, 0, 0, 0, 0, 0}, t_prev = host_trace ? now() : 0.0;
	auto lap = [&](int k) { if (host_trace) { const double t = now(); lap_t[k] += t - t_prev; t_prev = t; } };

	if (!c->stream2) HIPCHK(c, hipStreamCreateWithFlags(&c->stream2, hipStreamNonBlocking));
	if (!c->ev_post) HIPCHK(c, hipEventCreateWithFlags(&c->ev_post, hipEventDisableTiming));
	BatchPrep cur, nxt;
	u64 words_done = 0, done = 0;
	if (prepare_batch(c, g, chain, budget.batch, np, px, py, 0, cur) || launch_fb_batch(c, g, chain, budget.planes, cur, false)) return 1;
	lap(0);
	while (done < np) {
		const u64 B = cur.B;
		if (launch_post_batch(c, g, post_rows, post_wide, sort_cap, B)) return 1;
		lap(1);
		nxt.valid = false;
		if (done + B < np && (prepare_batch(c, g, chain, budget.batch, np, px, py, done + B, nxt) || launch_fb_batch(c, g, chain, budget.planes, nxt, true))) return 1;
		lap(2);
		bool overflow = false;
		if (read_batch_sizes(c, done, B, &overflow)) return 1;
		lap(3);
		if (overflow) {
			const u64 room = (u64)g.LXmax * g.LYmax;
			if (g.capc >= room) return fail(c, "mpcgpu_calc_posteriors: candidate overflow at full capacity (internal error)");
			if (trace_on()) {
				fprintf(stderr, "[mpcgpu] stage A overflow: batch at pair %llu (%llu pairs) redone, capc %u -> %llu, next batch %s\n", done, B, g.capc,
					std::min<u64>((u64)g.capc * 2, room), nxt.valid ? "queued and dropped" : "not queued");
				fflush(stderr);
			}
			g.capc = (u32)std::min<u64>((u64)g.capc * 2, room);
			HIPCHK(c, hipStreamSynchronize(c->stream));
			if (prepare_batch(c, g, chain, budget.batch, np, px, py, done, cur) || launch_fb_batch(c, g, chain, budget.planes, cur, false)) return 1;
			continue;
		}
		if (pack_batch(c, g, cur, done, np, hdr, &words_done)) return 1;
		c->sa_b0 = done; c->sa_B = B; c->sa_capc = g.capc; c->sa_post_rows = post_rows; c->sa_long_min = g.long_min;
		done += B;
		for (u32 c2 : cur.chain_cnt) if (c2 >= 2) { c->sa_chains += 1; c->sa_chained += c2; }
		if (cur.coop_pairs) { c->sa_coop_pairs += cur.coop_pairs; c->sa_coop_waves = cur.coop_waves; }
		std::swap(cur, nxt);
		if (cur.valid) {
			std::swap(c->d_bx, c->d_bx_n); std::swap(c->d_by, c->d_by_n); std::swap(c->d_order, c->d_order_n);
			std::swap(c->d_chain_first, c->d_chain_first_n); std::swap(c->d_chain_cnt, c->d_chain_cnt_n);
		}
		lap(4);
	}
	HIPCHK(c, hipStreamSynchronize(c->stream));
	if (host_trace)
		fprintf(stderr, "[mpcgpu] stage A host seconds: prepare (first batch / retries) %.4f, uploads + launches %.4f, next batch prepared %.4f, "
			"waiting for the device %.4f, sizes -> pack -> wait %.4f\n", lap_t[0], lap_t[1], lap_t[2], lap_t[3], lap_t[4]);
	std::vector<u8> &h = c->v_shdr;
	h.assign(hdr, 0);
	u64 h2[2] = {np, words_done};
	memcpy(h.data(), h2, 16);
	memcpy(h.data() + 16, c->sh_nnz.data(), np * 4);
	memcpy(h.data() + 16 + np * 4, c->sh_ea.data(), np * 4);
	HIPCHK(c, hipMemcpyAsync(c->d_shard.p, h.data(), hdr, hipMemcpyHostToDevice, c->stream));
	HIPCHK(c, hipStreamSynchronize(c->stream));
	c->shard_bytes = hdr + words_done * 4;
	c->have_shard = true;
	return 0;
}

int mpcgpu_calc_posteriors(mpcgpu_ctx *c, uint64_t k0, uint64_t k1)
{
	if (!c) return 1;
	if (c->n == 0) return fail(c, "mpcgpu_calc_posteriors: call mpcgpu_set_seqs first");
	if (k0 > k1 || k1 > c->npairs) return fail(c, "mpcgpu_calc_posteriors: bad pair range [%llu,%llu)", (u64)k0, (u64)k1);
	++c->epoch;
	const int rc = stage_a(c, k1 - k0, c->h_pair_x.data() + k0, c->h_pair_y.data() + k0);
	c->shard_is_list = false;
	c->sh_k0 = k0; c->sh_k1 = k1;
	return rc;
}
```

Baseline: 345,700.

## Fuse posterior row processing into chained forward-backward kernel sweeps

Adds a fused variant of the chained forward-backward kernel that runs the per-pair posterior-rows pass (sort, max-path relax, sparse extraction) inside the same wave right after the sweeps, using extra per-wave LDS. The standalone post kernel then only handles the remaining pairs through a selection list. Result, nnz, ea and flags buffers are double-buffered so the next batch's fused kernel can write while the current batch is packed. The aim is to remove a separate launch and a global re-read of candidates for chained pairs. The cost is higher LDS use per workgroup, which may lower occupancy.

```diff
diff --git a/include/mpcgpu.h b/include/mpcgpu.h
--- a/include/mpcgpu.h
+++ b/include/mpcgpu.h
@@ -116,6 +116,7 @@
 int mpcgpu_work_get(mpcgpu_ctx *ctx, uint64_t *dp_cells, uint64_t *relax_entry_z, uint64_t *store_entries);
 int mpcgpu_stage_a_info(mpcgpu_ctx *ctx, uint64_t *pairs, uint64_t *chained_pairs, uint64_t *chains);
 int mpcgpu_stage_a_coop_info(mpcgpu_ctx *ctx, uint64_t *pairs, uint32_t *waves_per_pair);
+int mpcgpu_stage_a_fuse_info(mpcgpu_ctx *ctx, uint64_t *pairs, uint32_t *bins);
 int mpcgpu_post_info(mpcgpu_ctx *ctx, uint64_t out[4]);
 int mpcgpu_store_info(mpcgpu_ctx *ctx, uint64_t out[6]);
 int mpcgpu_synchronize(mpcgpu_ctx *ctx);
diff --git a/muscle_amd/_lib.py b/muscle_amd/_lib.py
--- a/muscle_amd/_lib.py
+++ b/muscle_amd/_lib.py
@@ -13,7 +13,7 @@
     "mpcgpu_set_seqs", "mpcgpu_set_mega", "mpcgpu_pair_count", "mpcgpu_calc_posteriors", "mpcgpu_build_store",
     "mpcgpu_shard_info", "mpcgpu_shard_export", "mpcgpu_store_import", "mpcgpu_values_info", "mpcgpu_values_slice", "mpcgpu_values_export", "mpcgpu_values_import",
     "mpcgpu_cons_iter", "mpcgpu_cons_commit", "mpcgpu_cons_commit_range", "mpcgpu_get_ea", "mpcgpu_get_nnz", "mpcgpu_get_sparse",
-    "mpcgpu_get_sparse_range", "mpcgpu_post_scores", "mpcgpu_calc_aln", "mpcgpu_align_alns", "mpcgpu_align_alns_w", "mpcgpu_build_post", "mpcgpu_get_last_post", "mpcgpu_align_msas", "mpcgpu_align_pairs", "mpcgpu_get_list_sparse", "mpcgpu_stage_a_info", "mpcgpu_stage_a_coop_info", "mpcgpu_post_info", "mpcgpu_set_seqs_registry", "mpcgpu_timers_reset", "mpcgpu_timers_enable", "mpcgpu_timers_get",
+    "mpcgpu_get_sparse_range", "mpcgpu_post_scores", "mpcgpu_calc_aln", "mpcgpu_align_alns", "mpcgpu_align_alns_w", "mpcgpu_build_post", "mpcgpu_get_last_post", "mpcgpu_align_msas", "mpcgpu_align_pairs", "mpcgpu_get_list_sparse", "mpcgpu_stage_a_info", "mpcgpu_stage_a_coop_info", "mpcgpu_stage_a_fuse_info", "mpcgpu_post_info", "mpcgpu_set_seqs_registry", "mpcgpu_timers_reset", "mpcgpu_timers_enable", "mpcgpu_timers_get",
     "mpcgpu_work_get", "mpcgpu_synchronize", "mpcgpu_relax_info", "mpcgpu_shard_entries",
     "mpcgpu_set_pair_order", "mpcgpu_pair_position", "mpcgpu_plan_partition", "mpcgpu_plan_store_segments", "mpcgpu_store_import_part", "mpcgpu_store_complete", "mpcgpu_store_info", "mpcgpu_align_alns_batch", "mpcgpu_store_epoch",
     "mpcgpu_group_create", "mpcgpu_group_destroy", "mpcgpu_group_last_error", "mpcgpu_group_size", "mpcgpu_group_ctx",
@@ -91,6 +91,7 @@
     L.mpcgpu_work_get.argtypes = [vp, C.POINTER(u64), C.POINTER(u64), C.POINTER(u64)]
     L.mpcgpu_stage_a_info.argtypes = [vp, C.POINTER(u64), C.POINTER(u64), C.POINTER(u64)]
     L.mpcgpu_stage_a_coop_info.argtypes = [vp, C.POINTER(u64), C.POINTER(u32)]
+    L.mpcgpu_stage_a_fuse_info.argtypes = [vp, C.POINTER(u64), C.POINTER(u32)]
     L.mpcgpu_post_info.argtypes = [vp, C.POINTER(u64)]
     L.mpcgpu_synchronize.argtypes = [vp]
     L.mpcgpu_relax_info.argtypes = [vp, C.c_char_p, u32, C.POINTER(i32)]
@@ -513,6 +514,16 @@
         self._ck(self.L.mpcgpu_stage_a_coop_info(self.h, C.byref(a), C.byref(w)))
         return a.value, w.value
 
+    def stage_a_fuse_info(self):
+        a = C.c_uint64(0)
+        self._ck(self.L.mpcgpu_stage_a_fuse_info(self.h, C.byref(a), None))
+        return a.value
+
+    def stage_a_fuse_bins(self):
+        a, b = C.c_uint64(0), C.c_uint32(0)
+        self._ck(self.L.mpcgpu_stage_a_fuse_info(self.h, C.byref(a), C.byref(b)))
+        return {H for H in range(32) if b.value >> H & 1}
+
     def post_info(self):
         out = (C.c_uint64 * 4)()
         self._ck(self.L.mpcgpu_post_info(self.h, out))
diff --git a/muscle_amd/csrc/kernels_fbc.h b/muscle_amd/csrc/kernels_fbc.h
--- a/muscle_amd/csrc/kernels_fbc.h
+++ b/muscle_amd/csrc/kernels_fbc.h
@@ -1,5 +1,6 @@
 #pragma once
 #include "kernels_fb.h"
+#include "kernels_post.h"
 
 #define MPC_CHAIN_MAX 16
 #define MPC_CHAIN_TAB_WORDS 8
@@ -11,8 +12,27 @@
 	const u32 *chain_cnt;
 };
 
-template <int H>
-__global__ void __launch_bounds__(256, (H == 8) ? 4 : 1) fb_chain_kernel(FbChainParams cp)
+struct FbChainPost {
+	u32 lx_cap, ly_cap;
+	u32 sort_cap;
+	u32 wave_lds;
+	u32 batch;
+	int use_fma;
+	u64 *sort_scratch;
+	u64 sort_stride;
+	u32 *res;
+	u64 res_stride;
+	u32 *nnz;
+	float *ea;
+	u32 *flags;
+};
+struct FbChainPostParams { FbChainParams c; FbChainPost post; };
+#ifndef MPC_DEVICE_FENCE
+#define MPC_DEVICE_FENCE() ((void)0)
+#endif
+
+template <int H, bool POST>
+__device__ __forceinline__ void fb_chain_body(const FbChainParams &cp, const FbChainPost *pp)
 {
 	const FbParams &p = cp.f;
 	MPC_DYN_SMEM(smem_raw);
@@ -308,5 +328,32 @@
 		}
 		if (t == 0)
 			p.cand_cnt[pidA] = ncA;
+		if (POST) {
+			MPC_DEVICE_FENCE();
+			MPC_WAVE_LDS_ORDER();
+			u32 *s_rend = (u32 *)((unsigned char *)(s_tab_all + waves_per_block * (MPC_CHAIN_MAX * MPC_CHAIN_TAB_WORDS)) + (size_t)wave * pp->wave_lds);
+			u32 *s_cend = s_rend + pp->lx_cap;
+			float *s_pm = (float *)(s_cend + pp->ly_cap);
+			u64 *s_sorted = (u64 *)((unsigned char *)s_rend + ((((size_t)pp->lx_cap + 2 * (size_t)pp->ly_cap) * 4 + 7) & ~(size_t)7));
+			for (int k = 0; k < C; ++k) {
+				const u32 pid = tabw(k, 2);
+				const u32 c = mpc_wave_first(p.cand_cnt[pid]);
+				u64 *sorted = (c <= pp->sort_cap) ? s_sorted : (pp->sort_scratch + (u64)slot * pp->sort_stride);
+				mpc_post_rows_pair<false>(t, (u32)LX, tabw(k, 0), MPC_KEY_ROW_SHIFT, p.cand + (u64)pid * p.capc, c, p.capc, sorted,
+					pp->res + (u64)pid * pp->res_stride, pp->nnz + pid, pp->ea + pid, pp->flags + pid, pp->use_fma, pp->batch, s_rend, s_cend, s_pm);
+			}
+		}
 	}
 }
+
+template <int H>
+__global__ void __launch_bounds__(256, (H == 8) ? 4 : 1) fb_chain_kernel(FbChainParams cp)
+{
+	fb_chain_body<H, false>(cp, nullptr);
+}
+
+template <int H>
+__global__ void __launch_bounds__(256, (H <= 8) ? 4 : 1) fb_chain_post_kernel(FbChainPostParams cp)
+{
+	fb_chain_body<H, true>(cp.c, &cp.post);
+}
diff --git a/muscle_amd/csrc/kernels_post.h b/muscle_amd/csrc/kernels_post.h
--- a/muscle_amd/csrc/kernels_post.h
+++ b/muscle_amd/csrc/kernels_post.h
@@ -197,8 +197,227 @@
 	u32 *flags;
 	u32 count;
 	u32 long_min;
+	const u32 *sel;
 };
 
+template <bool WG> __device__ __forceinline__ void mpc_post_sync()
+{
+	if (WG) __syncthreads();
+	else { MPC_WAVE_FENCE(); MPC_WAVE_LDS_ORDER(); }
+}
+
+template <bool WG>
+__device__ __forceinline__ void mpc_post_rows_pair(const int t, const u32 LX, const u32 LY, const u32 kshift, u64 *cand, const u32 c, const u32 capc,
+	u64 *sorted, u32 *rec, u32 *nnz_out, float *ea_out, u32 *flags_out, const int use_fma, const u32 batch, u32 *s_rend, u32 *s_cend, float *s_pm)
+{
+	if (c > capc) {
+		if (t == 0) { *flags_out = 1u; *nnz_out = 0; *ea_out = 0.0f; }
+		return;
+	}
+	if (t == 0) *flags_out = 0u;
+	for (u32 q = t; q <= LX; q += 64) s_rend[q] = 0;
+	for (u32 q = t; q <= LY; q += 64) { s_cend[q] = 0; s_pm[q] = 0.0f; }
+	for (u32 q = t; q < LX + LY; q += 64) rec[q] = 0;
+	mpc_post_sync<WG>();
+	for (u32 q = t; q < c; q += 64) {
+		const u64 v = cand[q];
+		const float pr = mpc_score_to_prob(__uint_as_float((u32)v), use_fma);
+		cand[q] = (v & 0xffffffff00000000ull) | (u64)__float_as_uint(pr);
+		atomicAdd(&s_rend[(u32)(v >> (32 + kshift))], 1u);
+	}
+	mpc_post_sync<WG>();
+	{
+		u32 carry = 0;
+		for (u32 a0 = 0; a0 <= LX; a0 += 64) {
+			const u32 a = a0 + t;
+			const u32 v = (a <= LX) ? s_rend[a] : 0;
+			u32 incl = v;
+			for (int d = 1; d < 64; d <<= 1) {
+				const u32 o = __shfl_up(incl, d);
+				if (t >= d) incl += o;
+			}
+			if (a <= LX) s_rend[a] = carry + incl - v;
+			carry += __shfl(incl, 63);
+		}
+	}
+	mpc_post_sync<WG>();
+	for (u32 q = t; q < c; q += 64) {
+		const u64 v = cand[q];
+		const u32 at = atomicAdd(&s_rend[(u32)(v >> (32 + kshift))], 1u);
+		sorted[at] = ((v >> 32) & (u64)((1u << kshift) - 1u)) << 32 | (v & 0xffffffffull);
+	}
+	mpc_post_sync<WG>();
+	for (u32 i = t; i < LX; i += 64) {
+		const u32 b = i ? s_rend[i - 1] : 0u, e = s_rend[i];
+		for (u32 x = b + 1; x < e; ++x) {
+			const u64 key = sorted[x];
+			u32 y = x;
+			while (y > b && sorted[y - 1] > key) { sorted[y] = sorted[y - 1]; --y; }
+			sorted[y] = key;
+		}
+	}
+	mpc_post_sync<WG>();
+	u32 cmax = 0;
+	u64 nkey = c ? sorted[(u32)t < c ? (u32)t : c - 1u] : 0ull;
+	for (u32 i0 = 0; i0 < LX; i0 += 64) {
+		const u32 ri = i0 + (u32)t;
+		const u32 rend_v = s_rend[ri < LX ? ri : LX - 1u];
+		u32 b = mpc_wave_first(i0 ? s_rend[i0 - 1u] : 0u);
+		const u32 nl = LX - i0 < 64u ? LX - i0 : 64u;
+		for (u32 rl = 0; rl < nl; ++rl) {
+			const u32 e = mpc_read_lane(rend_v, rl);
+			if (e == b) continue;
+			if (e - b > batch) {
+				for (u32 x = b + (u32)t; x < e; x += 64) {
+					const u64 key = sorted[x];
+					const u32 cc = (u32)(key >> 32);
+					s_cend[x - b] = __float_as_uint(s_pm[cc < cmax ? cc : cmax] + __uint_as_float((u32)key));
+				}
+				mpc_post_sync<WG>();
+				float vprev = 0.0f;
+				for (u32 c0 = b; c0 < e; c0 += batch) {
+					const u32 me = c0 + (u32)t;
+					const bool have = me < e && (u32)t < batch;
+					const u64 key = have ? sorted[me] : 0ull;
+					const u32 col = (u32)(key >> 32);
+					const float val = have ? __uint_as_float(s_cend[me - b]) : 0.0f;
+					const float suffix = s_pm[cmax];
+					const float V = fmaxf(mpc_wave_scan_max_nonneg(val), vprev);
+					const u32 k = (e - c0 < batch) ? (e - c0) : batch;
+					const u32 last = mpc_read_lane(col, k - 1) + 1u;
+					const u32 hi = last > cmax ? last : cmax;
+					const u32 jb0 = mpc_wave_first(col) + 1u;
+					for (u32 j0 = jb0 < cmax + 1u ? jb0 : cmax + 1u; j0 <= hi; j0 += 64) {
+						const u32 j = j0 + (u32)t;
+						float cur = 0.0f;
+						for (u32 l = 0; l < k; ++l) {
+							const u32 cj = mpc_read_lane(col, l) + 1u;
+							const float vj = mpc_read_lane(V, l);
+							cur = (j >= cj) ? vj : cur;
+						}
+						if (j <= hi) s_pm[j] = fmaxf(j <= cmax ? s_pm[j] : suffix, cur);
+					}
+					cmax = hi;
+					vprev = mpc_read_lane(V, k - 1);
+					mpc_post_sync<WG>();
+				}
+				for (u32 x = b + (u32)t; x < e; x += 64) s_cend[x - b] = 0;
+				mpc_post_sync<WG>();
+				nkey = sorted[e + (u32)t < c ? e + (u32)t : c - 1u];
+				b = e;
+				continue;
+			}
+			const u32 k = e - b;
+			const bool have = (u32)t < k;
+			const u64 key = nkey;
+			nkey = sorted[e + (u32)t < c ? e + (u32)t : c - 1u];
+			const u32 col = have ? (u32)(key >> 32) : 0u;
+			const u32 jfirst = mpc_wave_first(col) + 1u;
+			const float val = have ? s_pm[col < cmax ? col : cmax] + __uint_as_float((u32)key) : 0.0f;
+			const float suffix = s_pm[cmax];
+			const float V = mpc_wave_scan_max_nonneg(val);
+			const u32 last = mpc_read_lane(col, k - 1) + 1u;
+			const u32 hi = last > cmax ? last : cmax;
+			for (u32 j0 = jfirst < cmax + 1u ? jfirst : cmax + 1u; j0 <= hi; j0 += 64) {
+				const u32 j = j0 + (u32)t;
+				const float old = s_pm[j <= cmax ? j : cmax];
+				float cur = 0.0f;
+				for (u32 l = 0; l < k; ++l) {
+					const u32 cj = mpc_read_lane(col, l) + 1u;
+					const float vj = mpc_read_lane(V, l);
+					cur = (j >= cj) ? vj : cur;
+				}
+				if (j <= hi) s_pm[j] = fmaxf(j <= cmax ? old : suffix, cur);
+			}
+			cmax = hi;
+			b = e;
+			MPC_WAVE_LDS_ORDER();
+		}
+	}
+	const float score = s_pm[LY < cmax ? LY : cmax];
+	const u32 mn = LX < LY ? LX : LY;
+	const float ea = score / (float)mn;
+	mpc_post_sync<WG>();
+	u32 kept = 0;
+	for (u32 q0 = 0; q0 < c; q0 += 64) {
+		const u32 q = q0 + t;
+		const bool k = q < c && __uint_as_float((u32)sorted[q]) >= MPC_MIN_SPARSE_PROB;
+		kept += (u32)__popcll(__ballot(k));
+	}
+	const u32 nnz = kept;
+	u32 *rowcnt = rec, *colcnt = rec + LX;
+	u32 *ent = rec + LX + LY;
+	u32 *rowv = ent + 2 * (u64)nnz;
+	u32 *tperm = rowv + nnz;
+	u32 base = 0;
+	for (u32 i0 = 0; i0 < LX; i0 += 64) {
+		const u32 i = i0 + (u32)t;
+		u32 mycnt = 0;
+		u32 b = 0, e = 0;
+		if (i < LX) {
+			b = i ? s_rend[i - 1] : 0u; e = s_rend[i];
+			for (u32 x = b; x < e; ++x) mycnt += (__uint_as_float((u32)sorted[x]) >= MPC_MIN_SPARSE_PROB) ? 1u : 0u;
+		}
+		u32 incl = mycnt;
+		for (int d = 1; d < 64; d <<= 1) {
+			const u32 o = __shfl_up(incl, d);
+			if (t >= d) incl += o;
+		}
+		u32 at = base + incl - mycnt;
+		if (i < LX) {
+			rowcnt[i] = mycnt;
+			for (u32 x = b; x < e; ++x) {
+				const u64 key = sorted[x];
+				if (__uint_as_float((u32)key) >= MPC_MIN_SPARSE_PROB) {
+					const u32 col = (u32)(key >> 32);
+					ent[2 * (u64)at] = (u32)key;
+					ent[2 * (u64)at + 1] = col;
+					rowv[at] = i;
+					atomicAdd(&s_cend[col], 1u);
+					++at;
+				}
+			}
+		}
+		base += __shfl(incl, 63);
+	}
+	mpc_post_sync<WG>();
+	for (u32 q = t; q < LY; q += 64) colcnt[q] = s_cend[q];
+	{
+		u32 carry = 0;
+		for (u32 a0 = 0; a0 <= LY; a0 += 64) {
+			const u32 a = a0 + t;
+			const u32 v = (a <= LY) ? s_cend[a] : 0;
+			u32 incl = v;
+			for (int d = 1; d < 64; d <<= 1) {
+				const u32 o = __shfl_up(incl, d);
+				if (t >= d) incl += o;
+			}
+			if (a <= LY) s_cend[a] = carry + incl - v;
+			carry += __shfl(incl, 63);
+		}
+	}
+	mpc_post_sync<WG>();
+	u32 *csorted = (u32 *)sorted;
+	mpc_post_sync<WG>();
+	for (u32 q = t; q < nnz; q += 64) {
+		const u32 at = atomicAdd(&s_cend[ent[2 * (u64)q + 1]], 1u);
+		csorted[at] = q;
+	}
+	mpc_post_sync<WG>();
+	for (u32 j = t; j < LY; j += 64) {
+		const u32 b = j ? s_cend[j - 1] : 0u, e = s_cend[j];
+		for (u32 x = b + 1; x < e; ++x) {
+			const u32 key = csorted[x];
+			u32 y = x;
+			while (y > b && csorted[y - 1] > key) { csorted[y] = csorted[y - 1]; --y; }
+			csorted[y] = key;
+		}
+	}
+	mpc_post_sync<WG>();
+	for (u32 q = t; q < nnz; q += 64) tperm[csorted[q]] = q;
+	if (t == 0) { *nnz_out = nnz; *ea_out = ea; }
+	mpc_post_sync<WG>();
+}
 
 __global__ void __launch_bounds__(64) post_rows_kernel(PostRowsParams p)
 {
@@ -209,219 +428,12 @@
 	u64 *s_sorted = (u64 *)(smem_raw + ((((size_t)p.lx_cap + 2 * (size_t)p.ly_cap) * 4 + 7) & ~(size_t)7));
 	const int t = threadIdx.x;
 
-	for (u32 pid = blockIdx.x; pid < p.count; pid += gridDim.x) {
+	for (u32 k = blockIdx.x; k < p.count; k += gridDim.x) {
+		const u32 pid = p.sel ? p.sel[k] : k;
 		const u32 LX = p.seq_len[p.pair_x[pid]], LY = p.seq_len[p.pair_y[pid]];
-		const u32 kshift = mpc_key_shift(LX, p.long_min);
-		u32 *rec = p.res + (u64)pid * p.res_stride;
 		const u32 c = p.cand_cnt[pid];
-		if (c > p.capc) {
-			if (t == 0) { p.flags[pid] = 1u; p.nnz[pid] = 0; p.ea[pid] = 0.0f; }
-			continue;
-		}
-		if (t == 0) p.flags[pid] = 0u;
-		u64 *cand = p.cand + (u64)pid * p.capc;
 		u64 *sorted = (c <= p.sort_cap) ? s_sorted : (p.sort_scratch + (u64)blockIdx.x * p.sort_stride);
-		for (u32 q = t; q <= LX; q += 64) s_rend[q] = 0;
-		for (u32 q = t; q <= LY; q += 64) { s_cend[q] = 0; s_pm[q] = 0.0f; }
-		for (u32 q = t; q < LX + LY; q += 64) rec[q] = 0;
-		__syncthreads();
-		for (u32 q = t; q < c; q += 64) {
-			const u64 v = cand[q];
-			const float pr = mpc_score_to_prob(__uint_as_float((u32)v), p.use_fma);
-			cand[q] = (v & 0xffffffff00000000ull) | (u64)__float_as_uint(pr);
-			atomicAdd(&s_rend[(u32)(v >> (32 + kshift))], 1u);
-		}
-		__syncthreads();
-		{
-			u32 carry = 0;
-			for (u32 a0 = 0; a0 <= LX; a0 += 64) {
-				const u32 a = a0 + t;
-				const u32 v = (a <= LX) ? s_rend[a] : 0;
-				u32 incl = v;
-				for (int d = 1; d < 64; d <<= 1) {
-					const u32 o = __shfl_up(incl, d);
-					if (t >= d) incl += o;
-				}
-				if (a <= LX) s_rend[a] = carry + incl - v;
-				carry += __shfl(incl, 63);
-			}
-		}
-		__syncthreads();
-		for (u32 q = t; q < c; q += 64) {
-			const u64 v = cand[q];
-			const u32 at = atomicAdd(&s_rend[(u32)(v >> (32 + kshift))], 1u);
-			sorted[at] = ((v >> 32) & (u64)((1u << kshift) - 1u)) << 32 | (v & 0xffffffffull);
-		}
-		__syncthreads();
-		for (u32 i = t; i < LX; i += 64) {
-			const u32 b = i ? s_rend[i - 1] : 0u, e = s_rend[i];
-			for (u32 x = b + 1; x < e; ++x) {
-				const u64 key = sorted[x];
-				u32 y = x;
-				while (y > b && sorted[y - 1] > key) { sorted[y] = sorted[y - 1]; --y; }
-				sorted[y] = key;
-			}
-		}
-		__syncthreads();
-		u32 cmax = 0;
-		u64 nkey = c ? sorted[(u32)t < c ? (u32)t : c - 1u] : 0ull;
-		for (u32 i0 = 0; i0 < LX; i0 += 64) {
-			const u32 ri = i0 + (u32)t;
-			const u32 rend_v = s_rend[ri < LX ? ri : LX - 1u];
-			u32 b = mpc_wave_first(i0 ? s_rend[i0 - 1u] : 0u);
-			const u32 nl = LX - i0 < 64u ? LX - i0 : 64u;
-			for (u32 rl = 0; rl < nl; ++rl) {
-				const u32 e = mpc_read_lane(rend_v, rl);
-				if (e == b) continue;
-				if (e - b > p.batch) {
-					for (u32 x = b + (u32)t; x < e; x += 64) {
-						const u64 key = sorted[x];
-						const u32 cc = (u32)(key >> 32);
-						s_cend[x - b] = __float_as_uint(s_pm[cc < cmax ? cc : cmax] + __uint_as_float((u32)key));
-					}
-					__syncthreads();
-					float vprev = 0.0f;
-					for (u32 c0 = b; c0 < e; c0 += p.batch) {
-						const u32 me = c0 + (u32)t;
-						const bool have = me < e && (u32)t < p.batch;
-						const u64 key = have ? sorted[me] : 0ull;
-						const u32 col = (u32)(key >> 32);
-						const float val = have ? __uint_as_float(s_cend[me - b]) : 0.0f;
-						const float suffix = s_pm[cmax];
-						const float V = fmaxf(mpc_wave_scan_max_nonneg(val), vprev);
-						const u32 k = (e - c0 < p.batch) ? (e - c0) : p.batch;
-						const u32 last = mpc_read_lane(col, k - 1) + 1u;
-						const u32 hi = last > cmax ? last : cmax;
-						const u32 jb0 = mpc_wave_first(col) + 1u;
-						for (u32 j0 = jb0 < cmax + 1u ? jb0 : cmax + 1u; j0 <= hi; j0 += 64) {
-							const u32 j = j0 + (u32)t;
-							float cur = 0.0f;
-							for (u32 l = 0; l < k; ++l) {
-								const u32 cj = mpc_read_lane(col, l) + 1u;
-								const float vj = mpc_read_lane(V, l);
-								cur = (j >= cj) ? vj : cur;
-							}
-							if (j <= hi) s_pm[j] = fmaxf(j <= cmax ? s_pm[j] : suffix, cur);
-						}
-						cmax = hi;
-						vprev = mpc_read_lane(V, k - 1);
-						__syncthreads();
-					}
-					for (u32 x = b + (u32)t; x < e; x += 64) s_cend[x - b] = 0;
-					__syncthreads();
-					nkey = sorted[e + (u32)t < c ? e + (u32)t : c - 1u];
-					b = e;
-					continue;
-				}
-				const u32 k = e - b;
-				const bool have = (u32)t < k;
-				const u64 key = nkey;
-				nkey = sorted[e + (u32)t < c ? e + (u32)t : c - 1u];
-				const u32 col = have ? (u32)(key >> 32) : 0u;
-				const u32 jfirst = mpc_wave_first(col) + 1u;
-				const float val = have ? s_pm[col < cmax ? col : cmax] + __uint_as_float((u32)key) : 0.0f;
-				const float suffix = s_pm[cmax];
-				const float V = mpc_wave_scan_max_nonneg(val);
-				const u32 last = mpc_read_lane(col, k - 1) + 1u;
-				const u32 hi = last > cmax ? last : cmax;
-				for (u32 j0 = jfirst < cmax + 1u ? jfirst : cmax + 1u; j0 <= hi; j0 += 64) {
-					const u32 j = j0 + (u32)t;
-					const float old = s_pm[j <= cmax ? j : cmax];
-					float cur = 0.0f;
-					for (u32 l = 0; l < k; ++l) {
-						const u32 cj = mpc_read_lane(col, l) + 1u;
-						const float vj = mpc_read_lane(V, l);
-						cur = (j >= cj) ? vj : cur;
-					}
-					if (j <= hi) s_pm[j] = fmaxf(j <= cmax ? old : suffix, cur);
-				}
-				cmax = hi;
-				b = e;
-				MPC_WAVE_LDS_ORDER();
-			}
-		}
-		const float score = s_pm[LY < cmax ? LY : cmax];
-		const u32 mn = LX < LY ? LX : LY;
-		const float ea = score / (float)mn;
-		__syncthreads();
-		u32 kept = 0;
-		for (u32 q0 = 0; q0 < c; q0 += 64) {
-			const u32 q = q0 + t;
-			const bool k = q < c && __uint_as_float((u32)sorted[q]) >= MPC_MIN_SPARSE_PROB;
-			kept += (u32)__popcll(__ballot(k));
-		}
-		const u32 nnz = kept;
-		u32 *rowcnt = rec, *colcnt = rec + LX;
-		u32 *ent = rec + LX + LY;
-		u32 *rowv = ent + 2 * (u64)nnz;
-		u32 *tperm = rowv + nnz;
-		u32 base = 0;
-		for (u32 i0 = 0; i0 < LX; i0 += 64) {
-			const u32 i = i0 + (u32)t;
-			u32 mycnt = 0;
-			u32 b = 0, e = 0;
-			if (i < LX) {
-				b = i ? s_rend[i - 1] : 0u; e = s_rend[i];
-				for (u32 x = b; x < e; ++x) mycnt += (__uint_as_float((u32)sorted[x]) >= MPC_MIN_SPARSE_PROB) ? 1u : 0u;
-			}
-			u32 incl = mycnt;
-			for (int d = 1; d < 64; d <<= 1) {
-				const u32 o = __shfl_up(incl, d);
-				if (t >= d) incl += o;
-			}
-			u32 at = base + incl - mycnt;
-			if (i < LX) {
-				rowcnt[i] = mycnt;
-				for (u32 x = b; x < e; ++x) {
-					const u64 key = sorted[x];
-					if (__uint_as_float((u32)key) >= MPC_MIN_SPARSE_PROB) {
-						const u32 col = (u32)(key >> 32);
-						ent[2 * (u64)at] = (u32)key;
-						ent[2 * (u64)at + 1] = col;
-						rowv[at] = i;
-						atomicAdd(&s_cend[col], 1u);
-						++at;
-					}
-				}
-			}
-			base += __shfl(incl, 63);
-		}
-		__syncthreads();
-		for (u32 q = t; q < LY; q += 64) colcnt[q] = s_cend[q];
-		{
-			u32 carry = 0;
-			for (u32 a0 = 0; a0 <= LY; a0 += 64) {
-				const u32 a = a0 + t;
-				const u32 v = (a <= LY) ? s_cend[a] : 0;
-				u32 incl = v;
-				for (int d = 1; d < 64; d <<= 1) {
-					const u32 o = __shfl_up(incl, d);
-					if (t >= d) incl += o;
-				}
-				if (a <= LY) s_cend[a] = carry + incl - v;
-				carry += __shfl(incl, 63);
-			}
-		}
-		__syncthreads();
-		u32 *csorted = (u32 *)sorted;
-		__syncthreads();
-		for (u32 q = t; q < nnz; q += 64) {
-			const u32 at = atomicAdd(&s_cend[ent[2 * (u64)q + 1]], 1u);
-			csorted[at] = q;
-		}
-		__syncthreads();
-		for (u32 j = t; j < LY; j += 64) {
-			const u32 b = j ? s_cend[j - 1] : 0u, e = s_cend[j];
-			for (u32 x = b + 1; x < e; ++x) {
-				const u32 key = csorted[x];
-				u32 y = x;
-				while (y > b && csorted[y - 1] > key) { csorted[y] = csorted[y - 1]; --y; }
-				csorted[y] = key;
-			}
-		}
-		__syncthreads();
-		for (u32 q = t; q < nnz; q += 64) tperm[csorted[q]] = q;
-		if (t == 0) { p.nnz[pid] = nnz; p.ea[pid] = ea; }
-		__syncthreads();
-	}
-}
+		mpc_post_rows_pair<true>(t, LX, LY, mpc_key_shift(LX, p.long_min), p.cand + (u64)pid * p.capc, c, p.capc, sorted, p.res + (u64)pid * p.res_stride,
+			p.nnz + pid, p.ea + pid, p.flags + pid, p.use_fma, p.batch, s_rend, s_cend, s_pm);
+	}
+}
diff --git a/muscle_amd/csrc/mpc_platform.h b/muscle_amd/csrc/mpc_platform.h
--- a/muscle_amd/csrc/mpc_platform.h
+++ b/muscle_amd/csrc/mpc_platform.h
@@ -97,6 +97,7 @@
 }
 #define MPC_KERNARG_AGAIN(p) mpc_kernarg_again(p)
 #define MPC_WAVE_FENCE() __builtin_amdgcn_fence(__ATOMIC_SEQ_CST, "workgroup")
+#define MPC_DEVICE_FENCE() __builtin_amdgcn_fence(__ATOMIC_SEQ_CST, "agent")
 __device__ __forceinline__ unsigned mpc_cvt_u32_sat(float f) { unsigned r; asm("v_cvt_u32_f32 %0, %1" : "=v"(r) : "v"(f)); return r; }
 __device__ __forceinline__ unsigned mpc_write_lane(unsigned v, unsigned sv, unsigned l) { return (threadIdx.x & 63u) == l ? sv : v; }
 __device__ __forceinline__ void mpc_dma16(const void *gsrc, void *lds_wave_base)
diff --git a/muscle_amd/csrc/mpcgpu.cpp b/muscle_amd/csrc/mpcgpu.cpp
--- a/muscle_amd/csrc/mpcgpu.cpp
+++ b/muscle_amd/csrc/mpcgpu.cpp
@@ -210,6 +210,9 @@
 	DevBuf d_ap_off;
 	DevBuf d_chain_first, d_chain_cnt;
 	DevBuf d_bx_n, d_by_n, d_order_n, d_chain_first_n, d_chain_cnt_n;
+	DevBuf d_rest, d_rest_n, d_res_n, d_nnz_n, d_ea_n, d_flags_n, d_fuse_sort;
+	u64 sa_fused = 0;
+	u32 sa_fuse_bins = 0;
 	hipStream_t stream2 = nullptr;
 	hipEvent_t ev_post = nullptr;
 	u64 sa_pairs = 0, sa_chained = 0, sa_chains = 0;
@@ -458,6 +461,65 @@
 {
 	switch (H) {
 #define MPC_CASE(h) case h: launch_fbc<h>(p, grid, block, smem, st); break;
+	MPC_CASE(1) MPC_CASE(2) MPC_CASE(3) MPC_CASE(4) MPC_CASE(5) MPC_CASE(6) MPC_CASE(7) MPC_CASE(8)
+	MPC_CASE(9) MPC_CASE(10) MPC_CASE(11) MPC_CASE(12) MPC_CASE(13) MPC_CASE(14) MPC_CASE(15) MPC_CASE(16)
+#undef MPC_CASE
+	default: break;
+	}
+}
+
+template <int H> void launch_fbcp(const FbChainPostParams &p, u32 grid, u32 block, size_t smem, hipStream_t st)
+{
+	auto kern = fb_chain_post_kernel<H>;
+	ensure_dyn_smem((const void *)kern, smem);
+	MPC_LAUNCH(kern, grid, block, smem, st, p);
+}
+
+template <int H> int occ_fbcp(u32 block, size_t smem)
+{
+	int nb = 0;
+	ensure_dyn_smem((const void *)fb_chain_post_kernel<H>, smem);
+	if (hipOccupancyMaxActiveBlocksPerMultiprocessor(&nb, (const void *)fb_chain_post_kernel<H>, (int)block, smem) != hipSuccess) { (void)hipGetLastError(); nb = 0; }
+	return nb;
+}
+
+template <int H> bool fbcp_spills()
+{
+#ifdef MPC_EMU
+	return false;
+#else
+	hipFuncAttributes a;
+	if (hipFuncGetAttributes(&a, (const void *)fb_chain_post_kernel<H>) != hipSuccess) { (void)hipGetLastError(); return true; }
+	return a.localSizeBytes != 0;
+#endif
+}
+
+bool fbcp_spills_h(int H)
+{
+	switch (H) {
+#define MPC_CASE(h) case h: return fbcp_spills<h>();
+	MPC_CASE(1) MPC_CASE(2) MPC_CASE(3) MPC_CASE(4) MPC_CASE(5) MPC_CASE(6) MPC_CASE(7) MPC_CASE(8)
+	MPC_CASE(9) MPC_CASE(10) MPC_CASE(11) MPC_CASE(12) MPC_CASE(13) MPC_CASE(14) MPC_CASE(15) MPC_CASE(16)
+#undef MPC_CASE
+	default: return true;
+	}
+}
+
+int occ_fbcp_h(int H, u32 block, size_t smem)
+{
+	switch (H) {
+#define MPC_CASE(h) case h: return occ_fbcp<h>(block, smem);
+	MPC_CASE(1) MPC_CASE(2) MPC_CASE(3) MPC_CASE(4) MPC_CASE(5) MPC_CASE(6) MPC_CASE(7) MPC_CASE(8)
+	MPC_CASE(9) MPC_CASE(10) MPC_CASE(11) MPC_CASE(12) MPC_CASE(13) MPC_CASE(14) MPC_CASE(15) MPC_CASE(16)
+#undef MPC_CASE
+	default: return 0;
+	}
+}
+
+void launch_fbcp_h(int H, const FbChainPostParams &p, u32 grid, u32 block, size_t smem, hipStream_t st)
+{
+	switch (H) {
+#define MPC_CASE(h) case h: launch_fbcp<h>(p, grid, block, smem, st); break;
 	MPC_CASE(1) MPC_CASE(2) MPC_CASE(3) MPC_CASE(4) MPC_CASE(5) MPC_CASE(6) MPC_CASE(7) MPC_CASE(8)
 	MPC_CASE(9) MPC_CASE(10) MPC_CASE(11) MPC_CASE(12) MPC_CASE(13) MPC_CASE(14) MPC_CASE(15) MPC_CASE(16)
 #undef MPC_CASE
@@ -661,6 +723,7 @@
 	c->d_pw_rs.release(); c->d_pw_info.release();
 	c->d_chain_first.release(); c->d_chain_cnt.release();
 	c->d_bx_n.release(); c->d_by_n.release(); c->d_order_n.release(); c->d_chain_first_n.release(); c->d_chain_cnt_n.release();
+	for (DevBuf *b : {&c->d_rest, &c->d_rest_n, &c->d_res_n, &c->d_nnz_n, &c->d_ea_n, &c->d_flags_n, &c->d_fuse_sort}) b->release();
 	c->d_rects.release(); c->d_need.release(); c->d_exp_klist.release(); c->d_exp_valbase.release();
 	c->d_tiles2.release();
 	c->pad_seg.release(); release_windows(c);
@@ -999,6 +1062,14 @@
 	return 0;
 }
 
+int mpcgpu_stage_a_fuse_info(mpcgpu_ctx *c, uint64_t *pairs, uint32_t *bins)
+{
+	if (!c) return 1;
+	if (pairs) *pairs = c->sa_fused;
+	if (bins) *bins = c->sa_fuse_bins;
+	return 0;
+}
+
 int mpcgpu_stage_a_coop_info(mpcgpu_ctx *c, uint64_t *pairs, uint32_t *waves_per_pair)
 {
 	if (!c) return 1;
diff --git a/muscle_amd/csrc/mpcgpu_stage_a.inc b/muscle_amd/csrc/mpcgpu_stage_a.inc
--- a/muscle_amd/csrc/mpcgpu_stage_a.inc
+++ b/muscle_amd/csrc/mpcgpu_stage_a.inc
@@ -62,13 +62,52 @@
 	u32 ccount[MPC_HMAX + 1];
 	u32 cvmax[MPC_HMAX + 1];
 	u32 coop_pairs = 0, coop_waves = 0;
+	u64 fused = 0;
+	std::vector<u32> rest;
 };
 
 struct ChainPlan {
 	bool on = false, grade = true;
 	u32 max = 0; size_t smem = 0;
 	u32 vcap[MPC_HMAX + 1] = {0};
+	bool fuse[MPC_HMAX + 1] = {false}, fuse_any = false;
+	u32 fuse_sort_cap[MPC_HMAX + 1] = {0};
+	u32 post_batch = 64;
 };
+static size_t post_rows_fixed_lds(const StageAGeom &g) { return ((((size_t)g.LXmax + 2 + 2 * ((size_t)g.LYmax + 2)) * 4 + 7) & ~(size_t)7); }
+static size_t fuse_smem(const ChainPlan &cp, const StageAGeom &g, u32 sort_cap) { return cp.smem + (size_t)SA_WAVES * (post_rows_fixed_lds(g) + 8 * (size_t)sort_cap); }
+
+static const int kFbPostFuseDefault = 0;
+static int fuse_plan(mpcgpu_ctx *c, const StageAGeom &g, u64 np, u64 batch_budget, bool post_rows, u32 sort_cap, ChainPlan &cp)
+{
+	const int env = env_int("MPCGPU_FB_POST_FUSE", kFbPostFuseDefault);
+	cp.post_batch = (u32)std::min(std::max(env_int("MPCGPU_POST_BATCH", 64), 1), 64);
+	if (!cp.on || !post_rows || env == 0) return 0;
+	size_t freeb = 0, totb = 0;
+	HIPCHK(c, hipMemGetInfo(&freeb, &totb));
+	const u64 owned = (u64)c->d_cand.cap + c->d_res.cap + c->d_res_n.cap + c->d_fm.cap;
+	const u64 second = std::min<u64>(np * g.res_stride() * 4, std::min<u64>(batch_budget, (u64)((freeb + owned) * 0.4)));
+	if (second > (freeb + c->d_res_n.cap) / 4) {
+		if (trace_on()) { fprintf(stderr, "[mpcgpu] fb chain post: not fused, a second set of records (%llu B) is more than a quarter of the free memory (%zu B)\n", second, freeb + c->d_res_n.cap); fflush(stderr); }
+		return 0;
+	}
+	const u32 top = std::max(std::min<u32>(g.capc, sort_cap), 2u);
+	for (u32 H = 1; H <= MPC_HMAX; ++H) {
+		if (!cp.vcap[H]) continue;
+		const int occ0 = occ_fbc_h((int)H, SA_BLOCK, cp.smem);
+		if (env != 1 && fbcp_spills_h((int)H)) continue;
+		const int occ2 = occ_fbcp_h((int)H, SA_BLOCK, fuse_smem(cp, g, 2));
+		const int need = occ2 >= occ0 ? occ0 : env == 1 ? 1 : occ0;
+		if (occ2 < need) continue;
+		u32 lo = 2, hi = top;
+		while (lo < hi) {
+			const u32 mid = lo + (hi - lo + 1) / 2;
+			if (occ_fbcp_h((int)H, SA_BLOCK, fuse_smem(cp, g, mid)) >= need) lo = mid; else hi = mid - 1;
+		}
+		cp.fuse[H] = true; cp.fuse_sort_cap[H] = lo; cp.fuse_any = true;
+	}
+	return 0;
+}
 static int chain_plan(mpcgpu_ctx *c, const StageAGeom &g, u64 planes_budget, ChainPlan &cp)
 {
 	cp.on = !g.mega && env_int("MPCGPU_FB_CHAIN", 1) != 0;
@@ -154,7 +193,7 @@
 	const u64 per_pair = (u64)g.capc * 8 + g.res_stride() * 4 + 64;
 	size_t freeb = 0, totb = 0;
 	HIPCHK(c, hipMemGetInfo(&freeb, &totb));
-	const u64 owned = (u64)c->d_cand.cap + c->d_res.cap + c->d_fm.cap;
+	const u64 owned = (u64)c->d_cand.cap + c->d_res.cap + c->d_res_n.cap + c->d_fm.cap;
 	const u64 budget = std::min<u64>(batch_budget, (u64)((freeb + owned) * 0.4));
 	const u64 bmax = std::min<u64>(std::max<u64>(1, budget / per_pair), 1u << 22);
 	const u64 left = np - b0, nbat = (left + bmax - 1) / bmax;
@@ -188,6 +227,14 @@
 		P.chain_cnt.push_back(ch.cnt);
 		for (u32 k = 0; k < ch.cnt; ++k) P.order[at++] = ch.q0 + k;
 	}
+	P.fused = 0; P.rest.clear();
+	if (cp.fuse_any) {
+		P.rest.assign(P.order.begin(), P.order.begin() + keys.size());
+		for (const Chain &ch : chains) {
+			if (cp.fuse[ch.H]) { P.fused += ch.cnt; continue; }
+			for (u32 k = 0; k < ch.cnt; ++k) P.rest.push_back(ch.q0 + k);
+		}
+	}
 	P.valid = true;
 	return 0;
 }
@@ -340,7 +387,7 @@
 	return 0;
 }
 
-static int launch_fb_chains(mpcgpu_ctx *c, const StageAGeom &g, const ChainPlan &plan, const FbParams &fp, const BatchPrep &P, const u32 *order, const u32 *first, const u32 *cnts)
+static int launch_fb_chains(mpcgpu_ctx *c, const StageAGeom &g, const ChainPlan &plan, const FbParams &fp, const BatchPrep &P, const u32 *order, const u32 *first, const u32 *cnts, const FbChainPost &post)
 {
 	const u32 cus = (u32)c->prop.multiProcessorCount;
 	TimedSpan sp;
@@ -348,7 +395,9 @@
 	for (u32 H = 1; H <= MPC_HMAX; ++H) {
 		if (!P.ccount[H]) continue;
 		const u32 cnt = P.ccount[H];
-		const u32 occ = (u32)occ_fbc_h((int)H, SA_BLOCK, plan.smem);
+		const bool fuse = plan.fuse[H];
+		const size_t smem = fuse ? fuse_smem(plan, g, plan.fuse_sort_cap[H]) : plan.smem;
+		const u32 occ = (u32)std::max(fuse ? occ_fbcp_h((int)H, SA_BLOCK, smem) : occ_fbc_h((int)H, SA_BLOCK, plan.smem), 1);
 		const u32 grid = std::max(std::min<u32>((cnt + SA_WAVES - 1) / SA_WAVES, cus * occ), 1u);
 		const u64 fm_stride = (u64)(P.cvmax[H] + 64) * H * 64;
 		HIPCHK(c, c->d_fm.ensure((u64)grid * SA_WAVES * fm_stride * 4));
@@ -358,6 +407,7 @@
 			u64 members = 0;
 			for (u32 k = 0; k < cnt; ++k) members += P.chain_cnt[cpos + k];
 			fprintf(stderr, "[mpcgpu] fb chain members H=%u pairs=%llu capc=%u batch=%llu\n", H, members, g.capc, P.B);
+			if (fuse) fprintf(stderr, "[mpcgpu] fb chain post: H=%u finishes its %llu pairs in the sweeps, list of %u candidates in LDS, lds=%zu B per workgroup\n", H, members, plan.fuse_sort_cap[H], smem);
 			fflush(stderr);
 		}
 		FbChainParams cp;
@@ -366,8 +416,20 @@
 		cp.f.queue = c->d_queue.as<u32>() + (MPC_HMAX + 2) + H;
 		cp.f.fm_scratch = c->d_fm.as<float>(); cp.f.fm_stride = fm_stride;
 		cp.chain_first = first + cpos; cp.chain_cnt = cnts + cpos;
-		if (span_begin(c, 0, &sp)) return 1;
-		launch_fbc_h((int)H, cp, grid, SA_BLOCK, plan.smem, c->stream);
+		if (fuse) {
+			FbChainPostParams fpp;
+			fpp.c = cp; fpp.post = post;
+			fpp.post.sort_cap = plan.fuse_sort_cap[H];
+			fpp.post.wave_lds = (u32)(post_rows_fixed_lds(g) + 8 * (size_t)fpp.post.sort_cap);
+			fpp.post.sort_stride = g.capc;
+			HIPCHK(c, c->d_fuse_sort.ensure(g.capc > fpp.post.sort_cap ? (u64)grid * SA_WAVES * g.capc * 8 : 8));
+			fpp.post.sort_scratch = c->d_fuse_sort.as<u64>();
+			if (span_begin(c, 0, &sp)) return 1;
+			launch_fbcp_h((int)H, fpp, grid, SA_BLOCK, smem, c->stream);
+		} else {
+			if (span_begin(c, 0, &sp)) return 1;
+			launch_fbc_h((int)H, cp, grid, SA_BLOCK, plan.smem, c->stream);
+		}
 		HIPCHK(c, hipGetLastError());
 		if (span_end(c, &sp)) return 1;
 		cpos += cnt;
@@ -379,13 +441,23 @@
 {
 	DevBuf &dbx = into_next ? c->d_bx_n : c->d_bx, &dby = into_next ? c->d_by_n : c->d_by, &dord = into_next ? c->d_order_n : c->d_order;
 	DevBuf &dcf = into_next ? c->d_chain_first_n : c->d_chain_first, &dcc = into_next ? c->d_chain_cnt_n : c->d_chain_cnt;
+	const bool alt = into_next && plan.fuse_any;
+	DevBuf &dres = alt ? c->d_res_n : c->d_res, &dnnz = alt ? c->d_nnz_n : c->d_nnz, &dea = alt ? c->d_ea_n : c->d_ea, &dflags = alt ? c->d_flags_n : c->d_flags;
 	const u64 B = P.B;
 	if (upload(c, dbx, P.bx) || upload(c, dby, P.by) || upload(c, dord, P.order)) return 1;
 	if (!P.chain_first.empty() && (upload(c, dcf, P.chain_first) || upload(c, dcc, P.chain_cnt))) return 1;
+	if (plan.fuse_any && upload(c, into_next ? c->d_rest_n : c->d_rest, P.rest)) return 1;
 	if (ensure_pair_scratch(c, g, B)) return 1;
-	HIPCHK(c, c->d_nnz.ensure(B * 4));
-	HIPCHK(c, c->d_ea.ensure(B * 4));
-	HIPCHK(c, c->d_flags.ensure(B * 4));
+	HIPCHK(c, dres.ensure(B * g.res_stride() * 4));
+	HIPCHK(c, dnnz.ensure(B * 4));
+	HIPCHK(c, dea.ensure(B * 4));
+	HIPCHK(c, dflags.ensure(B * 4));
+	FbChainPost post;
+	post.lx_cap = g.LXmax + 2; post.ly_cap = g.LYmax + 2; post.sort_cap = 0; post.wave_lds = 0;
+	post.batch = plan.post_batch; post.use_fma = c->use_fma;
+	post.sort_scratch = nullptr; post.sort_stride = 0;
+	post.res = dres.as<u32>(); post.res_stride = g.res_stride();
+	post.nnz = dnnz.as<u32>(); post.ea = dea.as<float>(); post.flags = dflags.as<u32>();
 	FbParams fp;
 	fill_fb_params(c, fp, dbx.as<u32>(), dby.as<u32>(), g.capc, g.mega);
 	P.coop_pairs = P.coop_waves = 0;
@@ -394,10 +466,10 @@
 		for (u32 H = 1; H <= MPC_HMAX; ++H) first += P.hcount[H];
 		if (launch_fb_row_block_pairs(c, g, fp, dord.as<u32>() + first, P.hcount[MPC_HMAX + 1], planes_budget, P)) return 1;
 	}
-	return launch_fb_bins(c, g, fp, dord.as<u32>(), P.hcount, B) || launch_fb_chains(c, g, plan, fp, P, dord.as<u32>(), dcf.as<u32>(), dcc.as<u32>());
-}
-
-struct PostIO { const u32 *pair_x, *pair_y, *seq_len; u64 *cand; const u32 *cand_cnt; u32 *res, *nnz; float *ea; u32 *flags; u32 count; };
+	return launch_fb_bins(c, g, fp, dord.as<u32>(), P.hcount, B) || launch_fb_chains(c, g, plan, fp, P, dord.as<u32>(), dcf.as<u32>(), dcc.as<u32>(), post);
+}
+
+struct PostIO { const u32 *pair_x, *pair_y, *seq_len; u64 *cand; const u32 *cand_cnt; u32 *res, *nnz; float *ea; u32 *flags; u32 count; const u32 *sel = nullptr; u32 nsel = 0; };
 
 static void post_info_set(mpcgpu_ctx *c, u32 kernel, u32 threads, u32 grid, u64 pairs) { c->pi_kernel = kernel; c->pi_threads = threads; c->pi_grid = grid; c->pi_pairs = pairs; }
 
@@ -418,15 +490,15 @@
 		int pocc = 0;
 		if (hipOccupancyMaxActiveBlocksPerMultiprocessor(&pocc, (const void *)post_rows_kernel, 64, smem) != hipSuccess || pocc < 1) pocc = 1;
 		pocc = std::max(1, std::min(pocc, (int)((152 * 1024) / smem)));
-		grid = (u32)std::min<u64>(io.count, (u64)c->prop.multiProcessorCount * (u32)pocc);
+		grid = (u32)std::max<u64>(std::min<u64>(io.sel ? io.nsel : io.count, (u64)c->prop.multiProcessorCount * (u32)pocc), 1);
 		if (trace_on()) { fprintf(stderr, "[mpcgpu] post rows: list of %u candidates in LDS, lds=%zu B blocks/CU=%d grid=%u\n", pr.sort_cap, smem, pocc, grid); fflush(stderr); }
 	}
 	HIPCHK(c, scratch.ensure(g.capc > pr.sort_cap ? (u64)grid * pr.sort_stride * 8 : 8));
 	pr.sort_scratch = scratch.as<u64>();
 	pr.res = io.res; pr.res_stride = g.res_stride();
 	pr.nnz = io.nnz; pr.ea = io.ea; pr.flags = io.flags;
-	pr.count = io.count; pr.long_min = g.long_min;
-	post_info_set(c, 0, 64, grid, io.count);
+	pr.count = io.sel ? io.nsel : io.count; pr.long_min = g.long_min; pr.sel = io.sel;
+	post_info_set(c, 0, 64, grid, pr.count);
 	TimedSpan sp;
 	if (timed && span_begin(c, 1, &sp)) return 1;
 	MPC_LAUNCH(post_rows_kernel, grid, 64, smem, c->stream, pr);
@@ -488,9 +560,10 @@
 	return timed ? span_end(c, &sp) : 0;
 }
 
-static int launch_post_batch(mpcgpu_ctx *c, const StageAGeom &g, bool post_rows, bool post_wide, u32 sort_cap, u64 B)
-{
-	const PostIO io = {c->d_bx.as<u32>(), c->d_by.as<u32>(), c->d_seq_len.as<u32>(), c->d_cand.as<u64>(), c->d_cand_cnt.as<u32>(), c->d_res.as<u32>(), c->d_nnz.as<u32>(), c->d_ea.as<float>(), c->d_flags.as<u32>(), (u32)B};
+static int launch_post_batch(mpcgpu_ctx *c, const StageAGeom &g, bool post_rows, bool post_wide, u32 sort_cap, u64 B, const std::vector<u32> *rest)
+{
+	PostIO io = {c->d_bx.as<u32>(), c->d_by.as<u32>(), c->d_seq_len.as<u32>(), c->d_cand.as<u64>(), c->d_cand_cnt.as<u32>(), c->d_res.as<u32>(), c->d_nnz.as<u32>(), c->d_ea.as<float>(), c->d_flags.as<u32>(), (u32)B};
+	if (rest) { io.sel = c->d_rest.as<u32>(); io.nsel = (u32)rest->size(); }
 	if (post_rows) {
 		if (launch_post_rows(c, g, io, sort_cap, (u32)std::max(env_int("MPCGPU_POST_BATCH", 64), 1), 0, c->d_sort_scratch, true)) return 1;
 	} else if (post_wide) {
@@ -598,6 +671,7 @@
 	const ScratchBudget budget = scratch_budget();
 	ChainPlan chain;
 	if (chain_plan(c, g, budget.planes, chain)) return 1;
+	c->sa_fused = 0; c->sa_fuse_bins = 0;
 	const char *post_mode = getenv("MPCGPU_POST");
 	const u32 sort_cap = (u32)std::max(env_int("MPCGPU_POST_SORT_CAP", 1024), 2);
 	const bool post_sort = post_mode && !strcmp(post_mode, "sort");
@@ -605,6 +679,7 @@
 	const bool fits = post_rows_fits(g.LXmax, g.LYmax, sort_cap);
 	const bool post_rows = wide_env != 1 && !post_sort && fits;
 	const bool post_wide = wide_env == 1 || (wide_env < 0 && kPostWideDefault && !post_sort && !fits);
+	if (fuse_plan(c, g, np, budget.batch, post_rows, sort_cap, chain)) return 1;
 	const bool host_trace = trace_host();
 	auto now = []() { return std::chrono::duration<double>(std::chrono::steady_clock::now().time_since_epoch()).count(); };
 	double lap_t[6] = {0, 0, 0, 0, 0, 0}, t_prev = host_trace ? now() : 0.0;
@@ -618,7 +693,7 @@
 	lap(0);
 	while (done < np) {
 		const u64 B = cur.B;
-		if (launch_post_batch(c, g, post_rows, post_wide, sort_cap, B)) return 1;
+		if (launch_post_batch(c, g, post_rows, post_wide, sort_cap, B, chain.fuse_any ? &cur.rest : nullptr)) return 1;
 		lap(1);
 		nxt.valid = false;
 		if (done + B < np && (prepare_batch(c, g, chain, budget.batch, np, px, py, done + B, nxt) || launch_fb_batch(c, g, chain, budget.planes, nxt, true))) return 1;
@@ -643,11 +718,17 @@
 		c->sa_b0 = done; c->sa_B = B; c->sa_capc = g.capc; c->sa_post_rows = post_rows; c->sa_long_min = g.long_min;
 		done += B;
 		for (u32 c2 : cur.chain_cnt) if (c2 >= 2) { c->sa_chains += 1; c->sa_chained += c2; }
+		c->sa_fused += cur.fused;
+		for (u32 H = 1; H <= MPC_HMAX; ++H) if (chain.fuse[H] && cur.ccount[H]) c->sa_fuse_bins |= 1u << H;
 		if (cur.coop_pairs) { c->sa_coop_pairs += cur.coop_pairs; c->sa_coop_waves = cur.coop_waves; }
 		std::swap(cur, nxt);
 		if (cur.valid) {
 			std::swap(c->d_bx, c->d_bx_n); std::swap(c->d_by, c->d_by_n); std::swap(c->d_order, c->d_order_n);
 			std::swap(c->d_chain_first, c->d_chain_first_n); std::swap(c->d_chain_cnt, c->d_chain_cnt_n);
+			if (chain.fuse_any) {
+				std::swap(c->d_rest, c->d_rest_n); std::swap(c->d_res, c->d_res_n);
+				std::swap(c->d_nnz, c->d_nnz_n); std::swap(c->d_ea, c->d_ea_n); std::swap(c->d_flags, c->d_flags_n);
+			}
 		}
 		lap(4);
 	}
```

Result: faster. 358,200, median of 6 (+3.6%).
